# sile/libflate

Hardware: AMD Instinct MI355X
Metric: gzip encode+decode throughput on 256 MiB synthetic text per GPU (uncompressed bytes through the round trip) (higher is better)
Workload: dtype u8; 1 GPU; cfg2: gzip::Encoder (DefaultLz77Encoder, default options, mtime=0) + gzip::Decoder on TEXT(268435456 B) per GPU, write schedule S8K (8192-byte writes); bytes_per_gpu=268435456, schedule=S8K, compressed_bytes=129579521, parallelism=1 rank

## Files before the change

include/lfx.h:

```cpp
#ifndef LFX_H
#define LFX_H
#include <stddef.h>
#include <stdint.h>

#ifdef __cplusplus
extern "C" {
#endif

#define LFX_VERSION 0x000100

enum { LFX_DEFLATE = 0, LFX_ZLIB = 1, LFX_GZIP = 2 };

enum {
    LFX_OK = 0,
    LFX_E_INVALID_DATA = 1,
    LFX_E_UNEXPECTED_EOF = 2,
    LFX_E_IO = 3,
    LFX_E_OOM = 4,
    LFX_E_DEVICE = 5,
    LFX_E_ARG = 6,
    LFX_E_NOSPACE = 7,
    LFX_E_UNSUPPORTED = 8,
    LFX_E_WOULD_BLOCK = 9
};
// ... 104 lines not shown
int lfx_index_read_device(lfx_ctx *c, const lfx_index *idx, const void *d_in, uint64_t in_base, uint64_t n,
                          uint32_t count, const uint64_t *off, const uint64_t *len, void *d_out,
                          const uint64_t *out_off, uint64_t *out_len_r, int32_t *status);
int lfx_index_span(const lfx_index *idx, uint64_t off, uint64_t len, uint64_t *in_lo, uint64_t *in_hi);
int lfx_index_get_info(const lfx_index *idx, lfx_index_info *info);
int lfx_index_get_point(const lfx_index *idx, uint32_t i, lfx_index_point *p);
int lfx_index_export(lfx_ctx *c, const lfx_index *idx, void *buf, uint64_t cap, uint64_t *len);
lfx_index *lfx_index_import(lfx_ctx *c, const void *buf, uint64_t len, int *status);
int lfx_index_check(const void *buf, uint64_t len, lfx_index_info *info);
void lfx_index_free(lfx_index *idx);

typedef struct lfx_shard_info {
    uint64_t total_bits;
    uint64_t n_bytes;
    uint32_t crc32;
    uint32_t adler32;
} lfx_shard_info;
int lfx_encode_shard_prepare(lfx_ctx *c, int format, const lfx_encode_opts *o,
                             const lfx_schedule *s, const void *d_in, uint64_t n, int is_first,
                             int is_last, lfx_shard_info *info);
int lfx_encode_shard_emit(lfx_ctx *c, uint64_t start_bit, uint32_t combined_check,
                          uint64_t total_n, void *d_out, uint64_t cap, uint64_t *out_len);
int lfx_encode_shard_prezero(lfx_ctx *c, void *d_out, uint64_t cap);
int lfx_decode_shard_device(lfx_ctx *c, const void *d_in, uint64_t n, uint64_t start_bit,
                            uint64_t total_bits, int is_last, void *d_out, uint64_t cap,
                            uint64_t *out_len);
typedef struct lfx_blk_tuple {
    uint64_t start_bit, end_bit;
    uint64_t n_out;
    uint64_t data_bit;
    uint32_t n_codes, nlanes;
    uint8_t btype, bfinal, status , _pad;
    uint16_t rank;
    uint16_t _pad2;
    uint32_t slot;
    uint32_t _pad3;
} lfx_blk_tuple;
int lfx_decode_range_scan(lfx_ctx *c, const void *d_part, uint64_t n_part, uint64_t lo_byte, uint64_t hi_byte,
                          uint64_t first_bit, uint64_t final_from_bit, uint32_t rank, lfx_blk_tuple *tuples, uint32_t cap,
                          uint32_t *count);
int lfx_decode_chain(const lfx_blk_tuple *all, uint32_t n_all, uint64_t first_bit, uint32_t *chain, uint32_t cap,
                     uint32_t *n_chain, uint64_t *total_out);
int lfx_decode_range_emit(lfx_ctx *c, const void *d_part, uint64_t n_part, uint64_t lo_byte, const lfx_blk_tuple *all,
                          const uint32_t *chain, uint32_t n_chain, uint32_t rank, void *d_out, uint64_t cap,
                          uint64_t *out_len, uint64_t *out_base, uint32_t *state);
int lfx_decode_range_map(lfx_ctx *c, void *d_map);
int lfx_decode_range_finish(lfx_ctx *c, const void *d_maps, uint32_t rank, uint32_t *crc32, uint32_t *adler32);
int lfx_shard_place_device(lfx_ctx *c, void *d_member, uint64_t cap, const void *d_part, uint64_t part_len,
                           uint64_t start_bit, int is_first);
typedef struct lfx_comm {
    void *user;
    uint32_t rank, world;
    int (*allgather)(void *user, const void *send, void *recv, uint64_t bytes);
    int (*isend)(void *user, const void *d_buf, uint64_t bytes, uint32_t to_rank);
    int (*irecv)(void *user, void *d_buf, uint64_t bytes, uint32_t from_rank);
    int (*wait)(void *user);
    int (*start)(void *user);
} lfx_comm;
int lfx_comm_rccl(void *nccl_comm, void *hip_stream, uint32_t rank, uint32_t world, lfx_comm *out);
void lfx_comm_rccl_free(lfx_comm *cm);

typedef struct lfx_sharded_enc lfx_sharded_enc;
typedef struct lfx_sharded_part {
    uint64_t start_bit;
    uint64_t end_bit;
    uint64_t part_len;
    uint64_t member_len;
    uint64_t total_n;
    uint32_t check;
    uint32_t _pad;
} lfx_sharded_part;
int lfx_sharded_encode_begin(lfx_ctx *c, const lfx_comm *cm, int format, const lfx_encode_opts *o, const lfx_schedule *s,
                             const void *d_in, uint64_t n, void *d_part, uint64_t part_cap, void *d_member ,
                             uint64_t member_cap, void *d_staging , uint64_t staging_cap, lfx_sharded_enc **state,
                             lfx_sharded_part *out);
int lfx_sharded_encode_finish(lfx_ctx *c, const lfx_comm *cm, lfx_sharded_enc *state, uint64_t *member_len );

typedef struct lfx_sharded_slice {
    uint64_t out_len, out_base;
    uint64_t total_out;
    uint32_t crc32, adler32;
} lfx_sharded_slice;
void lfx_sharded_byte_range(uint64_t first_byte, uint64_t member_len, uint32_t rank, uint32_t world, uint64_t *lo_byte,
                            uint64_t *hi_byte, uint64_t *hold_hi);
int lfx_sharded_decode(lfx_ctx *c, const lfx_comm *cm, const void *d_part, uint64_t n_part, uint64_t lo_byte, uint64_t hi_byte,
                       uint64_t first_bit, uint64_t member_len, void *d_out, uint64_t cap, lfx_sharded_slice *out);
int lfx_sharded_layout(const lfx_comm *cm, const lfx_shard_info *mine, uint64_t header_len, int format,
                       uint64_t *start_bits , uint32_t *check, uint64_t *total_n);
int lfx_sharded_gather_tuples(const lfx_comm *cm, const lfx_blk_tuple *mine, uint32_t count, int status, lfx_blk_tuple **all,
                              uint32_t *n_all, uint32_t *failed_rank);
int lfx_sharded_fold(const lfx_comm *cm, int status, uint32_t state, uint64_t len, uint32_t crc32, uint32_t adler32,
                     uint32_t *any_state, uint32_t *crc_all, uint32_t *adler_all, uint64_t *total, uint32_t *failed_rank);
void lfx_sharded_free(void *p);
uint32_t lfx_crc32_combine(uint32_t crc1, uint32_t crc2, uint64_t len2);
uint32_t lfx_adler32_combine(uint32_t ad1, uint32_t ad2, uint64_t len2);
uint64_t lfx_container_header_len(int format, const lfx_encode_opts *o);

typedef int64_t (*lfx_write_cb)(void *user, const uint8_t *p, size_t n);
typedef int (*lfx_flush_cb)(void *user);
typedef int64_t (*lfx_read_cb)(void *user, uint8_t *p, size_t cap);

typedef struct lfx_encoder lfx_encoder;
lfx_encoder *lfx_encoder_new(lfx_ctx *c, int format, const lfx_encode_opts *o, lfx_write_cb w,
                             lfx_flush_cb f, void *user, int *status);
int64_t lfx_encoder_write(lfx_encoder *e, const uint8_t *p, size_t n);
int lfx_encoder_write_codes(lfx_encoder *e, const uint32_t *codes, size_t n_codes, const uint8_t *raw, size_t n_raw,
                            int end_block);
int lfx_encoder_flush(lfx_encoder *e);
int lfx_encoder_finish(lfx_encoder *e);
const char *lfx_encoder_last_error(const lfx_encoder *e);
void lfx_encoder_free(lfx_encoder *e);

typedef struct lfx_decoder lfx_decoder;
#define LFX_DEC_NONBLOCKING 2u
lfx_decoder *lfx_decoder_new(lfx_ctx *c, int format, uint32_t flags, lfx_read_cb r, void *user,
                             int *status);
int64_t lfx_decoder_read(lfx_decoder *d, uint8_t *out, size_t cap);
int lfx_decoder_unread(lfx_decoder *d, const uint8_t **p, size_t *n);
uint64_t lfx_decoder_consumed(const lfx_decoder *d);
uint64_t lfx_decoder_buffered(const lfx_decoder *d);
int lfx_decoder_surplus(lfx_decoder *d, const uint8_t **p, size_t *n);
typedef struct lfx_header {
    int32_t format;
    uint32_t mtime;
    uint8_t xfl, os, is_text, is_verified, has_extra;
    uint8_t _pad[3];
    const uint8_t *extra;
    uint32_t extra_len;
    const char *filename;
    const char *comment;
    uint32_t zlib_window_size;
    uint32_t zlib_level;
} lfx_header;
int lfx_decoder_header(lfx_decoder *d, lfx_header *h);
const char *lfx_decoder_last_error(const lfx_decoder *d);
void lfx_decoder_free(lfx_decoder *d);

typedef void (*lfx_sink_cb)(void *user, const uint32_t *codes, size_t n);
typedef struct lfx_lz77 lfx_lz77;
lfx_lz77 *lfx_lz77_new(lfx_ctx *c, uint32_t window_size, uint32_t max_length, int *status);
int lfx_lz77_encode(lfx_lz77 *z, const uint8_t *buf, size_t len, lfx_sink_cb sink, void *user);
int lfx_lz77_flush(lfx_lz77 *z, lfx_sink_cb sink, void *user);
uint32_t lfx_lz77_window_size(const lfx_lz77 *z);
int lfx_lz77_compression_level(const lfx_lz77 *z);
void lfx_lz77_free(lfx_lz77 *z);

typedef struct lfx_timing {
    float total_ms;
    float phase_ms[16];
    char phase_name[16][24];
    int n_phases;
} lfx_timing;
uint64_t lfx_ctx_match_fallbacks(const lfx_ctx *c);
int lfx_ctx_last_timing(lfx_ctx *c, lfx_timing *t);
void lfx_ctx_enable_timing(lfx_ctx *c, int on);
uint32_t lfx_version(void);

#ifdef __cplusplus
}
#endif
#endif
```

libflate_amd/_ffi.py:

```python
import ctypes as C
import os

_HERE = os.path.dirname(os.path.abspath(__file__))
SO_PATH = os.environ.get("LFX_SO") or os.path.join(_HERE, "liblfx.so")

DEFLATE, ZLIB, GZIP = 0, 1, 2
OK, E_INVALID_DATA, E_UNEXPECTED_EOF, E_IO, E_OOM, E_DEVICE, E_ARG, E_NOSPACE, E_UNSUPPORTED, E_WOULD_BLOCK = range(10)
LZ77_DEFAULT, LZ77_NOCOMPRESSION = 0, 1
FLUSH_NONE, FLUSH_SYNC = 0, 2
SCHED_SINGLE, SCHED_FIXED, SCHED_LIST = 0, 1, 2
SCHED_FLUSH = (1 << 64) - 1
DEC_MULTI = 1
DEC_NONBLOCKING = 2
MEMBERS_BGZF = 1
BGZF_MEMBER_SIZE = 65280

EXPORTS = [
    "lfx_encode_opts_default", "lfx_ctx_new", "lfx_ctx_free", "lfx_ctx_last_error", "lfx_ctx_set_stream",
    "lfx_device_count", "lfx_encode_bound", "lfx_encode_device", "lfx_encode_batch_device", "lfx_encode_host", "lfx_decode_device",
    "lfx_decode_host", "lfx_decode_batch_device", "lfx_encode_shard_prepare", "lfx_encode_shard_emit", "lfx_encode_shard_prezero", "lfx_decode_shard_device", "lfx_shard_place_device", "lfx_decode_range_scan", "lfx_decode_chain", "lfx_decode_range_emit", "lfx_decode_range_map", "lfx_decode_range_finish",
    "lfx_crc32_combine", "lfx_adler32_combine", "lfx_container_header_len", "lfx_encoder_new",
    "lfx_encoder_write", "lfx_encoder_write_codes", "lfx_encoder_flush", "lfx_encoder_finish", "lfx_encoder_last_error",
    "lfx_encoder_free", "lfx_decoder_new", "lfx_decoder_read", "lfx_decoder_unread",
    "lfx_decoder_consumed", "lfx_decoder_buffered", "lfx_decoder_surplus", "lfx_decoder_header", "lfx_decoder_last_error", "lfx_decoder_free", "lfx_lz77_new",
    "lfx_lz77_encode", "lfx_lz77_flush", "lfx_lz77_window_size", "lfx_lz77_compression_level",
    "lfx_lz77_free", "lfx_ctx_last_timing", "lfx_ctx_enable_timing", "lfx_version",
    "lfx_comm_rccl", "lfx_comm_rccl_free", "lfx_sharded_encode_begin", "lfx_sharded_encode_finish", "lfx_sharded_byte_range",
    "lfx_sharded_decode", "lfx_sharded_layout", "lfx_sharded_gather_tuples", "lfx_sharded_fold", "lfx_sharded_free",
    "lfx_host_alloc", "lfx_host_free", "lfx_ctx_match_fallbacks", "lfx_decode_members_device", "lfx_decode_members_host",
    "lfx_decode_index_device", "lfx_index_read_device", "lfx_index_span", "lfx_index_get_info", "lfx_index_get_point",
    "lfx_index_export", "lfx_index_import", "lfx_index_check", "lfx_index_free", "lfx_encode_index_device",
    "lfx_encode_members_bound", "lfx_encode_members_device", "lfx_encode_members_host", "lfx_members_gzi",
]


class EncodeOpts(C.Structure):
    _fields_ = [
        ("block_size", C.c_uint64), ("dynamic_huffman", C.c_int32), ("no_compression", C.c_int32),
        ("lz77_kind", C.c_int32), ("window_size", C.c_uint32), ("max_length", C.c_uint32),
        ("zlib_flush_mode", C.c_int32), ("mtime", C.c_uint32), ("os", C.c_uint8), ("is_text", C.c_uint8),
        ("hcrc", C.c_uint8), ("lz77_level", C.c_uint8), ("extra", C.c_char_p), ("extra_len", C.c_uint32),
        ("filename", C.c_char_p), ("comment", C.c_char_p),
    ]


class Schedule(C.Structure):
    _fields_ = [("kind", C.c_int32), ("fixed_write", C.c_uint64), ("writes", C.POINTER(C.c_uint64)),
                ("n_writes", C.c_size_t)]


class BlkTuple(C.Structure):
    _fields_ = [("start_bit", C.c_uint64), ("end_bit", C.c_uint64), ("n_out", C.c_uint64), ("data_bit", C.c_uint64),
                ("n_codes", C.c_uint32), ("nlanes", C.c_uint32), ("btype", C.c_uint8), ("bfinal", C.c_uint8),
                ("status", C.c_uint8), ("_pad", C.c_uint8), ("rank", C.c_uint16), ("_pad2", C.c_uint16),
                ("slot", C.c_uint32), ("_pad3", C.c_uint32)]


class Member(C.Structure):
    _fields_ = [("in_off", C.c_uint64), ("in_len", C.c_uint64), ("out_off", C.c_uint64), ("out_len", C.c_uint64)]


class IndexPoint(C.Structure):
    _fields_ = [("in_bit", C.c_uint64), ("hdr_bit", C.c_uint64), ("out_off", C.c_uint64), ("member", C.c_uint32),
                ("win_len", C.c_uint32), ("in_crc", C.c_uint32), ("btype", C.c_uint8), ("_pad", C.c_uint8 * 3)]


class IndexInfo(C.Structure):
    _fields_ = [("in_len", C.c_uint64), ("out_len", C.c_uint64), ("spacing", C.c_uint64), ("max_gap", C.c_uint64),
                ("export_bytes", C.c_uint64), ("format", C.c_uint32), ("flags", C.c_uint32), ("n_points", C.c_uint32),
                ("n_members", C.c_uint32)]


class ShardInfo(C.Structure):
    _fields_ = [("total_bits", C.c_uint64), ("n_bytes", C.c_uint64), ("crc32", C.c_uint32),
                ("adler32", C.c_uint32)]


COMM_ALLGATHER = C.CFUNCTYPE(C.c_int, C.c_void_p, C.c_void_p, C.c_void_p, C.c_uint64)
COMM_P2P = C.CFUNCTYPE(C.c_int, C.c_void_p, C.c_void_p, C.c_uint64, C.c_uint32)
COMM_WAIT = C.CFUNCTYPE(C.c_int, C.c_void_p)


class Comm(C.Structure):
    _fields_ = [("user", C.c_void_p), ("rank", C.c_uint32), ("world", C.c_uint32), ("allgather", COMM_ALLGATHER),
                ("isend", COMM_P2P), ("irecv", COMM_P2P), ("wait", COMM_WAIT), ("start", COMM_WAIT)]


class ShardedPart(C.Structure):
    _fields_ = [("start_bit", C.c_uint64), ("end_bit", C.c_uint64), ("part_len", C.c_uint64), ("member_len", C.c_uint64), ("total_n", C.c_uint64),
                ("check", C.c_uint32), ("_pad", C.c_uint32)]


class ShardedSlice(C.Structure):
    _fields_ = [("out_len", C.c_uint64), ("out_base", C.c_uint64), ("total_out", C.c_uint64), ("crc32", C.c_uint32),
                ("adler32", C.c_uint32)]


class Header(C.Structure):
    _fields_ = [("format", C.c_int32), ("mtime", C.c_uint32), ("xfl", C.c_uint8), ("os", C.c_uint8),
                ("is_text", C.c_uint8), ("is_verified", C.c_uint8), ("has_extra", C.c_uint8), ("_pad", C.c_uint8 * 3),
                ("extra", C.POINTER(C.c_uint8)), ("extra_len", C.c_uint32), ("filename", C.c_char_p),
                ("comment", C.c_char_p), ("zlib_window_size", C.c_uint32), ("zlib_level", C.c_uint32)]


class Timing(C.Structure):
    _fields_ = [("total_ms", C.c_float), ("phase_ms", C.c_float * 16), ("phase_name", (C.c_char * 24) * 16),
                ("n_phases", C.c_int)]


WRITE_CB = C.CFUNCTYPE(C.c_int64, C.c_void_p, C.POINTER(C.c_uint8), C.c_size_t)
FLUSH_CB = C.CFUNCTYPE(C.c_int, C.c_void_p)
READ_CB = C.CFUNCTYPE(C.c_int64, C.c_void_p, C.POINTER(C.c_uint8), C.c_size_t)
SINK_CB = C.CFUNCTYPE(None, C.c_void_p, C.POINTER(C.c_uint32), C.c_size_t)


class LfxError(Exception):
    def __init__(self, status, message=""):
        super().__init__("lfx status %d: %s" % (status, message))
        self.status = status
        self.message = message


class DeviceError(LfxError):
    pass


_lib = None


def lib():
    global _lib
    if _lib is not None:
        return _lib
    if not os.path.exists(SO_PATH):
        raise ImportError(
            "libflate_amd: native library %s is missing — run `python -c 'import __graft_entry__ as g; "
            "g.build()'` (hipcc, gfx950). There is no CPU fallback." % SO_PATH)
    try:
        import torch
    except ImportError:
        pass
    L = C.CDLL(SO_PATH)
    u64, u32, vp, i32 = C.c_uint64, C.c_uint32, C.c_void_p, C.c_int
    L.lfx_encode_opts_default.argtypes = [C.POINTER(EncodeOpts)]
    L.lfx_ctx_new.restype = vp
    L.lfx_ctx_new.argtypes = [i32, C.POINTER(i32)]
    L.lfx_ctx_free.argtypes = [vp]
    L.lfx_ctx_last_error.restype = C.c_char_p
    L.lfx_ctx_last_error.argtypes = [vp]
    L.lfx_ctx_set_stream.argtypes = [vp, vp]
    L.lfx_encode_bound.restype = u64
    L.lfx_encode_bound.argtypes = [u64, C.POINTER(EncodeOpts), C.POINTER(Schedule)]
    L.lfx_encode_device.argtypes = [vp, i32, C.POINTER(EncodeOpts), C.POINTER(Schedule), vp, u64, vp, u64,
                                    C.POINTER(u64)]
    L.lfx_encode_host.argtypes = [vp, i32, C.POINTER(EncodeOpts), C.POINTER(Schedule), vp, u64, vp,
                                  u64, C.POINTER(u64)]
    L.lfx_host_alloc.restype = vp
    L.lfx_host_alloc.argtypes = [C.c_size_t]
    L.lfx_host_free.argtypes = [vp]
    L.lfx_ctx_match_fallbacks.restype = u64
    L.lfx_ctx_match_fallbacks.argtypes = [vp]
    L.lfx_decode_device.argtypes = [vp, i32, u32, vp, u64, vp, u64, C.POINTER(u64), C.POINTER(u64)]
    L.lfx_decode_host.argtypes = [vp, i32, u32, vp, u64, vp, u64, C.POINTER(u64), C.POINTER(u64)]
    L.lfx_decode_batch_device.argtypes = [vp, i32, u32, vp, vp, vp, vp, vp, vp, vp, vp]
    L.lfx_decode_members_device.argtypes = [vp, vp, u64, vp, u64, C.POINTER(u64), C.POINTER(u64), C.POINTER(Member), u32,
                                            C.POINTER(u32)]
    L.lfx_decode_members_host.argtypes = [vp, vp, u64, vp, u64, C.POINTER(u64), C.POINTER(u64), C.POINTER(Member), u32,
                                          C.POINTER(u32)]
    L.lfx_encode_members_bound.restype = u64
    L.lfx_encode_members_bound.argtypes = [u64, u64, u32, C.POINTER(EncodeOpts), C.POINTER(Schedule)]
    for f in (L.lfx_encode_members_device, L.lfx_encode_members_host):
        f.argtypes = [vp, C.POINTER(EncodeOpts), C.POINTER(Schedule), u64, u32, vp, u64, vp, u64, C.POINTER(u64),
                      C.POINTER(Member), u32, C.POINTER(u32)]
    L.lfx_members_gzi.argtypes = [C.POINTER(Member), u32, vp, u64, C.POINTER(u64)]
    L.lfx_decode_index_device.argtypes = [vp, i32, u32, vp, u64, vp, u64, C.POINTER(u64), C.POINTER(u64), u64, C.POINTER(vp)]
    L.lfx_encode_index_device.argtypes = [vp, i32, C.POINTER(EncodeOpts), C.POINTER(Schedule), vp, u64, vp, u64, C.POINTER(u64), u64,
                                          C.POINTER(vp)]
    L.lfx_index_read_device.argtypes = [vp, vp, vp, u64, u64, u32, vp, vp, vp, vp, vp, vp]
    L.lfx_index_span.argtypes = [vp, u64, u64, C.POINTER(u64), C.POINTER(u64)]
    L.lfx_index_get_info.argtypes = [vp, C.POINTER(IndexInfo)]
    L.lfx_index_get_point.argtypes = [vp, u32, C.POINTER(IndexPoint)]
    L.lfx_index_export.argtypes = [vp, vp, vp, u64, C.POINTER(u64)]
    L.lfx_index_import.argtypes = [vp, vp, u64, C.POINTER(i32)]
    L.lfx_index_import.restype = vp
    L.lfx_index_check.argtypes = [vp, u64, C.POINTER(IndexInfo)]
    L.lfx_index_free.argtypes = [vp]
    L.lfx_index_free.restype = None
    L.lfx_encode_batch_device.argtypes = [vp, i32, C.POINTER(EncodeOpts), C.POINTER(Schedule), u32, vp, vp, vp, vp, vp, vp, vp, vp]
    L.lfx_encode_shard_prepare.argtypes = [vp, i32, C.POINTER(EncodeOpts), C.POINTER(Schedule), vp, u64, i32,
                                           i32, C.POINTER(ShardInfo)]
    L.lfx_encode_shard_emit.argtypes = [vp, u64, u32, u64, vp, u64, C.POINTER(u64)]
    L.lfx_encode_shard_prezero.argtypes = [vp, vp, u64]
    L.lfx_decode_shard_device.argtypes = [vp, vp, u64, u64, u64, i32, vp, u64, C.POINTER(u64)]
    L.lfx_shard_place_device.argtypes = [vp, vp, u64, vp, u64, u64, i32]
    L.lfx_decode_range_scan.argtypes = [vp, vp, u64, u64, u64, u64, u64, u32, C.POINTER(BlkTuple), u32, C.POINTER(u32)]
    L.lfx_decode_chain.argtypes = [C.POINTER(BlkTuple), u32, u64, C.POINTER(u32), u32, C.POINTER(u32), C.POINTER(u64)]
    L.lfx_decode_range_emit.argtypes = [vp, vp, u64, u64, C.POINTER(BlkTuple), C.POINTER(u32), u32, u32, vp, u64,
                                        C.POINTER(u64), C.POINTER(u64), C.POINTER(u32)]
    L.lfx_decode_range_map.argtypes = [vp, vp]
    L.lfx_decode_range_finish.argtypes = [vp, vp, u32, C.POINTER(u32), C.POINTER(u32)]
    L.lfx_crc32_combine.restype = u32
    L.lfx_crc32_combine.argtypes = [u32, u32, u64]
    L.lfx_adler32_combine.restype = u32
    L.lfx_adler32_combine.argtypes = [u32, u32, u64]
    L.lfx_container_header_len.restype = u64
    L.lfx_container_header_len.argtypes = [i32, C.POINTER(EncodeOpts)]
    L.lfx_encoder_new.restype = vp
    L.lfx_encoder_new.argtypes = [vp, i32, C.POINTER(EncodeOpts), WRITE_CB, FLUSH_CB, vp, C.POINTER(i32)]
    L.lfx_encoder_write.restype = C.c_int64
    L.lfx_encoder_write.argtypes = [vp, C.c_char_p, C.c_size_t]
    L.lfx_encoder_write_codes.argtypes = [vp, C.POINTER(u32), C.c_size_t, C.c_char_p, C.c_size_t, i32]
    L.lfx_encoder_flush.argtypes = [vp]
    L.lfx_encoder_finish.argtypes = [vp]
    L.lfx_encoder_last_error.restype = C.c_char_p
    L.lfx_encoder_last_error.argtypes = [vp]
    L.lfx_encoder_free.argtypes = [vp]
    L.lfx_decoder_new.restype = vp
    L.lfx_decoder_new.argtypes = [vp, i32, u32, READ_CB, vp, C.POINTER(i32)]
    L.lfx_decoder_read.restype = C.c_int64
    L.lfx_decoder_read.argtypes = [vp, vp, C.c_size_t]
    L.lfx_decoder_unread.argtypes = [vp, C.POINTER(C.POINTER(C.c_uint8)), C.POINTER(C.c_size_t)]
    L.lfx_decoder_consumed.restype = u64
    L.lfx_decoder_consumed.argtypes = [vp]
    L.lfx_decoder_buffered.restype = u64
    L.lfx_decoder_buffered.argtypes = [vp]
    L.lfx_decoder_surplus.argtypes = [vp, C.POINTER(C.POINTER(C.c_uint8)), C.POINTER(C.c_size_t)]
    L.lfx_decoder_header.argtypes = [vp, C.POINTER(Header)]
    L.lfx_decoder_last_error.restype = C.c_char_p
    L.lfx_decoder_last_error.argtypes = [vp]
    L.lfx_decoder_free.argtypes = [vp]
    L.lfx_lz77_new.restype = vp
    L.lfx_lz77_new.argtypes = [vp, u32, u32, C.POINTER(i32)]
    L.lfx_lz77_encode.argtypes = [vp, C.c_char_p, C.c_size_t, SINK_CB, vp]
    L.lfx_lz77_flush.argtypes = [vp, SINK_CB, vp]
    L.lfx_lz77_window_size.restype = u32
    L.lfx_lz77_window_size.argtypes = [vp]
    L.lfx_lz77_compression_level.argtypes = [vp]
    L.lfx_lz77_free.argtypes = [vp]
    L.lfx_ctx_last_timing.argtypes = [vp, C.POINTER(Timing)]
    L.lfx_ctx_enable_timing.argtypes = [vp, i32]
    L.lfx_version.restype = u32
    L.lfx_comm_rccl.argtypes = [vp, vp, u32, u32, C.POINTER(Comm)]
    L.lfx_comm_rccl_free.argtypes = [C.POINTER(Comm)]
    L.lfx_comm_rccl_free.restype = None
    L.lfx_sharded_encode_begin.argtypes = [vp, C.POINTER(Comm), i32, C.POINTER(EncodeOpts), C.POINTER(Schedule), vp, u64, vp, u64,
                                           vp, u64, vp, u64, C.POINTER(vp), C.POINTER(ShardedPart)]
    L.lfx_sharded_encode_finish.argtypes = [vp, C.POINTER(Comm), vp, C.POINTER(u64)]
    L.lfx_sharded_byte_range.argtypes = [u64, u64, u32, u32, C.POINTER(u64), C.POINTER(u64), C.POINTER(u64)]
    L.lfx_sharded_byte_range.restype = None
    L.lfx_sharded_decode.argtypes = [vp, C.POINTER(Comm), vp, u64, u64, u64, u64, u64, vp, u64, C.POINTER(ShardedSlice)]
    L.lfx_sharded_layout.argtypes = [C.POINTER(Comm), C.POINTER(ShardInfo), u64, i32, C.POINTER(u64), C.POINTER(u32), C.POINTER(u64)]
    L.lfx_sharded_gather_tuples.argtypes = [C.POINTER(Comm), C.POINTER(BlkTuple), u32, i32, C.POINTER(C.POINTER(BlkTuple)),
                                            C.POINTER(u32), C.POINTER(u32)]
    L.lfx_sharded_fold.argtypes = [C.POINTER(Comm), i32, u32, u64, u32, u32, C.POINTER(u32), C.POINTER(u32), C.POINTER(u32),
                                   C.POINTER(u64), C.POINTER(u32)]
    L.lfx_sharded_free.argtypes = [vp]
    L.lfx_sharded_free.restype = None
    L.lfx_debug_huff_block.argtypes = [vp, u32, vp, vp, vp, C.POINTER(u32), C.POINTER(u64)]
    L.lfx_debug_plan.argtypes = [i32, C.POINTER(EncodeOpts), C.POINTER(Schedule), u64, vp, C.c_size_t,
                                 C.POINTER(C.c_size_t), vp, C.c_size_t, C.POINTER(C.c_size_t)]
    L.lfx_debug_plan_incremental.argtypes = [i32, C.POINTER(EncodeOpts), C.POINTER(Schedule), u64, u32, vp, C.c_size_t,
                                             C.POINTER(C.c_size_t), vp, C.c_size_t, C.POINTER(C.c_size_t)]
    L.lfx_debug_symbols.argtypes = [u32, u32, vp]
    _lib = L
    return L


def make_opts(**kw):
    o = EncodeOpts()
    lib().lfx_encode_opts_default(C.byref(o))
    keep = []
    for k, v in kw.items():
        if k == "extra":
            v = bytes(v)
            keep.append(v)
            o.extra, o.extra_len = v, len(v)
        elif k in ("filename", "comment"):
            v = bytes(v)
            keep.append(v)
            setattr(o, k, v)
        else:
            setattr(o, k, v)
    o._keep = keep
    return o


def members_to_gzi(members):
    members = list(members)
    table = (Member * max(len(members), 1))()
    for i, m in enumerate(members):
        table[i].in_off, table[i].in_len, table[i].out_off, table[i].out_len = m
    need = C.c_uint64(0)
    lib().lfx_members_gzi(table, len(members), None, 0, C.byref(need))
    buf = C.create_string_buffer(need.value)
    rc = lib().lfx_members_gzi(table, len(members), buf, need.value, C.byref(need))
    if rc:
        raise LfxError(rc, "lfx_members_gzi")
    return buf.raw[:need.value]


def make_schedule(write_size=0, writes=None):
    s = Schedule()
    if writes is not None:
        arr = (C.c_uint64 * len(writes))(*[SCHED_FLUSH if w is None else int(w) for w in writes])
        s.kind, s.writes, s.n_writes = SCHED_LIST, arr, len(writes)
        s._keep = arr
    elif write_size:
        s.kind, s.fixed_write = SCHED_FIXED, write_size
    else:
        s.kind = SCHED_SINGLE
    return s
```

libflate_amd/context.py:

```python
import ctypes as C

from . import _ffi


class Context:
    def __init__(self, device=0):
        st = C.c_int(0)
        self._h = _ffi.lib().lfx_ctx_new(device, C.byref(st))
        if not self._h:
            raise _ffi.DeviceError(st.value, "no usable MI355X device %d (there is no CPU fallback)" % device)
        self.device = device
        self._users = 0
        self._closing = False

    def _retain(self):
        self._users += 1

    def _release(self):
        self._users -= 1
        if self._users <= 0 and self._closing:
            self._free_now()

    def _free_now(self):
        if self._h:
            _ffi.lib().lfx_ctx_free(self._h)
            self._h = None

    def close(self):
        self._closing = True
        if self._users <= 0:
            self._free_now()

    def __del__(self):
        try:
            self.close()
        except Exception:
            pass

    @property
    def handle(self):
        return self._h

    def last_error(self):
        return (_ffi.lib().lfx_ctx_last_error(self._h) or b"").decode("utf-8", "replace")

    def set_stream(self, hip_stream_ptr):
        _ffi.lib().lfx_ctx_set_stream(self._h, hip_stream_ptr)

    def enable_timing(self, on=True):
        _ffi.lib().lfx_ctx_enable_timing(self._h, int(on) if on is not True and on is not False and 2 <= int(on) <= 6 else (1 if on else 0))

    def last_timing(self):
        t = _ffi.Timing()
        if _ffi.lib().lfx_ctx_last_timing(self._h, C.byref(t)) != 0:
            return None
        return {"total_ms": t.total_ms,
                "phases": [(bytes(t.phase_name[i]).split(b"\0")[0].decode(), t.phase_ms[i])
                           for i in range(t.n_phases)]}

    def match_fallbacks(self):
        return int(_ffi.lib().lfx_ctx_match_fallbacks(self._h))

    def encode_host_ptr(self, fmt, in_ptr, n, out_ptr, cap, opts=None, schedule=None):
        out_len = C.c_uint64(0)
        rc = _ffi.lib().lfx_encode_host(self._h, fmt, C.byref(opts) if opts is not None else None,
                                        C.byref(schedule) if schedule is not None else None, in_ptr, n, out_ptr, cap, C.byref(out_len))
        if rc:
            raise (_ffi.DeviceError if rc == _ffi.E_DEVICE else _ffi.LfxError)(rc, self.last_error())
        return out_len.value

    def decode_host_ptr(self, fmt, in_ptr, n, out_ptr, cap, flags=0):
        out_len, consumed = C.c_uint64(0), C.c_uint64(0)
        rc = _ffi.lib().lfx_decode_host(self._h, fmt, flags, in_ptr, n, out_ptr, cap, C.byref(out_len), C.byref(consumed))
        if rc in (_ffi.E_DEVICE, _ffi.E_OOM, _ffi.E_ARG):
            raise (_ffi.DeviceError if rc == _ffi.E_DEVICE else _ffi.LfxError)(rc, self.last_error())
        return rc, out_len.value, consumed.value, self.last_error() if rc else ""

    def encode_device(self, fmt, d_in, n, d_out, cap, opts=None, schedule=None):
        out_len = C.c_uint64(0)
        rc = _ffi.lib().lfx_encode_device(self._h, fmt, C.byref(opts) if opts is not None else None,
                                          C.byref(schedule) if schedule is not None else None,
                                          d_in, n, d_out, cap, C.byref(out_len))
        if rc:
            raise (_ffi.DeviceError if rc == _ffi.E_DEVICE else _ffi.LfxError)(rc, self.last_error())
        return out_len.value

    def encode_index_device(self, fmt, d_in, n, d_out, cap, opts=None, schedule=None, spacing=1 << 20):
        out_len, h = C.c_uint64(0), C.c_void_p(None)
        rc = _ffi.lib().lfx_encode_index_device(self._h, fmt, C.byref(opts) if opts is not None else None,
                                                C.byref(schedule) if schedule is not None else None,
                                                d_in, n, d_out, cap, C.byref(out_len), spacing, C.byref(h))
        if rc:
            raise (_ffi.DeviceError if rc == _ffi.E_DEVICE else _ffi.LfxError)(rc, self.last_error())
        return out_len.value, h.value

    def decode_device(self, fmt, d_in, n, d_out, cap, flags=0):
        out_len, consumed = C.c_uint64(0), C.c_uint64(0)
        rc = _ffi.lib().lfx_decode_device(self._h, fmt, flags, d_in, n, d_out, cap, C.byref(out_len),
                                          C.byref(consumed))
        if rc in (_ffi.E_DEVICE, _ffi.E_OOM, _ffi.E_ARG):
            raise (_ffi.DeviceError if rc == _ffi.E_DEVICE else _ffi.LfxError)(rc, self.last_error())
        return rc, out_len.value, consumed.value, self.last_error() if rc else ""

    def decode_members_device(self, d_in, n, d_out, cap, max_members=None):
        return self._members(_ffi.lib().lfx_decode_members_device, d_in, n, d_out, cap, max_members)

    def decode_index_device(self, fmt, d_in, n, d_out, cap, spacing=1 << 20, flags=0):
        out_len, consumed, h = C.c_uint64(0), C.c_uint64(0), C.c_void_p(None)
        rc = _ffi.lib().lfx_decode_index_device(self._h, fmt, flags, d_in, n, d_out, cap, C.byref(out_len), C.byref(consumed),
                                                spacing, C.byref(h))
        if rc in (_ffi.E_DEVICE, _ffi.E_OOM, _ffi.E_ARG):
            raise (_ffi.DeviceError if rc == _ffi.E_DEVICE else _ffi.LfxError)(rc, self.last_error())
        return rc, out_len.value, consumed.value, h.value, self.last_error() if rc else ""

    def index_read_device(self, index_handle, d_in, in_base, n, offs, lens, d_out, out_offs):
        k = len(offs)
        a = lambda v: (C.c_uint64 * max(k, 1))(*v)
        o, ln, oo = a(offs), a(lens), a(out_offs)
        out_len, st = (C.c_uint64 * max(k, 1))(), (C.c_int32 * max(k, 1))()
        rc = _ffi.lib().lfx_index_read_device(self._h, index_handle, d_in, in_base, n, k, o, ln, d_out, oo, out_len, st)
        if rc in (_ffi.E_DEVICE, _ffi.E_OOM) or (rc == _ffi.E_ARG and not any(st[i] == _ffi.E_ARG for i in range(k))):
            raise (_ffi.DeviceError if rc == _ffi.E_DEVICE else _ffi.LfxError)(rc, self.last_error())
        return rc, list(out_len[:k]), list(st[:k]), self.last_error() if rc else ""

    def _members(self, fn, src, n, dst, cap, max_members):
        if max_members is None:
            max_members = n // 20 + 1
        table = (_ffi.Member * max(int(max_members), 1))()
        out_len, consumed, count = C.c_uint64(0), C.c_uint64(0), C.c_uint32(0)
        rc = fn(self._h, src, n, dst, cap, C.byref(out_len), C.byref(consumed), table, int(max_members), C.byref(count))
        if rc in (_ffi.E_DEVICE, _ffi.E_OOM, _ffi.E_ARG):
            raise (_ffi.DeviceError if rc == _ffi.E_DEVICE else _ffi.LfxError)(rc, self.last_error())
        members = [(m.in_off, m.in_len, m.out_off, m.out_len) for m in table[:min(count.value, int(max_members))]]
        return rc, out_len.value, consumed.value, members, self.last_error() if rc else ""

    def decode_members_host(self, data, cap=None, max_members=None):
        data = bytes(data)
        grow = cap is None
        cap = cap if cap is not None else max(1 << 16, len(data) * 16)
        while True:
            out = C.create_string_buffer(cap)
            rc, ol, used, members, msg = self._members(_ffi.lib().lfx_decode_members_host, data, len(data), out, cap, max_members)
            if grow and rc == _ffi.E_NOSPACE and cap < len(data) * 1040 + (1 << 20):
                cap *= 8
                continue
            return rc, out.raw[:ol], used, members, msg

    def _encode_members(self, fn, src, n, dst, cap, member_size, flags, opts, schedule, max_members):
        count = 0 if (flags & _ffi.MEMBERS_BGZF and n == 0) else max(1, -(-n // member_size)) if member_size else 0
        if max_members is None:
            max_members = count
        table = (_ffi.Member * max(int(max_members), 1))()
        out_len, got = C.c_uint64(0), C.c_uint32(0)
        rc = fn(self._h, C.byref(opts) if opts is not None else None, C.byref(schedule) if schedule is not None else None,
                member_size, flags, src, n, dst, cap, C.byref(out_len), table, int(max_members), C.byref(got))
        if rc in (_ffi.E_DEVICE, _ffi.E_OOM, _ffi.E_ARG, _ffi.E_UNSUPPORTED):
            raise (_ffi.DeviceError if rc == _ffi.E_DEVICE else _ffi.LfxError)(rc, self.last_error())
        members = [(m.in_off, m.in_len, m.out_off, m.out_len) for m in table[:min(got.value, int(max_members))]]
        return rc, out_len.value, got.value, members, self.last_error() if rc else ""

    def encode_members_device(self, d_in, n, d_out, cap, member_size=1 << 20, flags=0, opts=None, schedule=None, max_members=None):
        return self._encode_members(_ffi.lib().lfx_encode_members_device, d_in, n, d_out, cap, member_size, flags, opts, schedule,
                                    max_members)

    def encode_members_host(self, data, member_size=1 << 20, flags=0, opts=None, schedule=None, cap=None, max_members=None):
        data = bytes(data)
        if cap is None:
            cap = _ffi.lib().lfx_encode_members_bound(len(data), member_size, flags, C.byref(opts) if opts is not None else None,
                                                      C.byref(schedule) if schedule is not None else None)
        out = C.create_string_buffer(max(cap, 1))
        rc, ol, count, members, msg = self._encode_members(_ffi.lib().lfx_encode_members_host, data, len(data), out, cap, member_size,
                                                           flags, opts, schedule, max_members)
        return rc, out.raw[:ol], count, members, msg

    def encode_host(self, fmt, data, opts=None, schedule=None):
        data = bytes(data)
        bound = _ffi.lib().lfx_encode_bound(len(data), C.byref(opts) if opts is not None else None,
                                            C.byref(schedule) if schedule is not None else None)
        if bound == 0:
            raise _ffi.LfxError(_ffi.E_ARG, "option outside the reference's domain")
        out = C.create_string_buffer(bound)
        out_len = C.c_uint64(0)
        rc = _ffi.lib().lfx_encode_host(self._h, fmt, C.byref(opts) if opts is not None else None,
                                        C.byref(schedule) if schedule is not None else None,
                                        data, len(data), out, bound, C.byref(out_len))
        if rc:
            raise (_ffi.DeviceError if rc == _ffi.E_DEVICE else _ffi.LfxError)(rc, self.last_error())
        return out.raw[:out_len.value]

    def decode_host(self, fmt, data, cap=None, flags=0):
        data = bytes(data)
        cap = cap if cap is not None else max(1 << 16, len(data) * 16)
        while True:
            out = C.create_string_buffer(cap)
            out_len, consumed = C.c_uint64(0), C.c_uint64(0)
            rc = _ffi.lib().lfx_decode_host(self._h, fmt, flags, data, len(data), out, cap,
                                            C.byref(out_len), C.byref(consumed))
            if rc in (_ffi.E_DEVICE, _ffi.E_OOM, _ffi.E_ARG):
                raise (_ffi.DeviceError if rc == _ffi.E_DEVICE else _ffi.LfxError)(rc, self.last_error())
            if rc == _ffi.E_NOSPACE and cap < len(data) * 1040 + (1 << 20):
                cap *= 8
                continue
            return rc, out.raw[:out_len.value], consumed.value, self.last_error() if rc else ""


_default = {}


def default_context(device=0):
    if device not in _default:
        _default[device] = Context(device)
    return _default[device]
```

libflate_amd/csrc/lfx_api.cpp:

```cpp
#include "../../include/lfx.h"
#include "../../include/lfx_testhooks.h"

#include <hip/hip_runtime.h>

#include <algorithm>
#include <cstddef>
#include <cstdio>
#include <cstdlib>
#include <cstring>
#include <mutex>
#include <string>
#include <vector>

#include "lfx_ctx.h"
#include "lfx_device.h"
#include "lfx_huff.h"
#include "lfx_index.h"
#include "lfx_plan.h"
#include "lfx_abi_guard.h"

using namespace lfx;

static uint32_t host_crc32(const uint8_t *p, size_t n) {
    static uint32_t tab[256];
// ... 58 lines not shown
    return d;
}
static int check_opts(const lfx_encode_opts &o) {
    if (o.block_size == 0) return LFX_E_ARG;
    if (o.max_length < 3) return LFX_E_ARG;
    return LFX_OK;
}
static PlanOpts plan_opts(int format, const lfx_encode_opts &o) {
    PlanOpts p;
    p.block_size = o.block_size;
    p.dynamic_huffman = o.dynamic_huffman != 0;
    p.no_compression = o.no_compression != 0;
    p.lz77_kind = o.lz77_kind;
    p.window_size = o.window_size;
    p.max_length = o.max_length;
    p.zlib_sync = format == LFX_ZLIB && o.zlib_flush_mode == LFX_FLUSH_SYNC;
    return p;
}

static void gzip_header(const lfx_encode_opts &o, bool with_hcrc, std::vector<uint8_t> &b) {
    uint8_t flg = (uint8_t)((o.is_text ? 1 : 0) | (with_hcrc ? 2 : 0) | (o.extra ? 4 : 0) |
                            (o.filename ? 8 : 0) | (o.comment ? 16 : 0));
    const uint8_t xfl = o.lz77_level == 1 + LFX_LEVEL_FAST ? 4 : o.lz77_level == 1 + LFX_LEVEL_BEST ? 2 : 0;
    const uint8_t h[10] = {31, 139, 8, flg, (uint8_t)o.mtime, (uint8_t)(o.mtime >> 8),
                           (uint8_t)(o.mtime >> 16), (uint8_t)(o.mtime >> 24), xfl, o.os};
    b.insert(b.end(), h, h + 10);
    if (o.extra) {
        b.push_back((uint8_t)o.extra_len);
        b.push_back((uint8_t)(o.extra_len >> 8));
        b.insert(b.end(), o.extra, o.extra + o.extra_len);
    }
    if (o.filename) b.insert(b.end(), o.filename, o.filename + strlen(o.filename) + 1);
    if (o.comment) b.insert(b.end(), o.comment, o.comment + strlen(o.comment) + 1);
    if (with_hcrc) {
        std::vector<uint8_t> t;
        gzip_header(o, false, t);
        uint32_t c = host_crc32(t.data(), t.size());
        b.push_back((uint8_t)c);
        b.push_back((uint8_t)(c >> 8));
    }
}
static int container_header(int format, const lfx_encode_opts &o, std::vector<uint8_t> &b) {
    if (format == LFX_GZIP) {
        if (o.extra && o.extra_len > 0xFFFF) return LFX_E_INVALID_DATA;
        gzip_header(o, o.hcrc != 0, b);
    } else if (format == LFX_ZLIB) {
        uint32_t ws = o.window_size;
        uint8_t cinfo = ws > 16384 ? 7 : ws > 8192 ? 6 : ws > 4096 ? 5 : ws > 2048 ? 4 : ws > 1024 ? 3
                        : ws > 512 ? 2 : ws > 256 ? 1 : 0;
        uint8_t level = (o.no_compression || o.lz77_kind == LFX_LZ77_NOCOMPRESSION) ? 0 : 2;
        if (o.lz77_level && !o.no_compression) level = (uint8_t)((o.lz77_level - 1) & 3);
        uint8_t cmf = (uint8_t)((cinfo << 4) | 8), flg = (uint8_t)(level << 6);
        uint32_t check = ((uint32_t)cmf << 8) + flg;
        if (check % 31 != 0) flg = (uint8_t)(flg + (31 - check % 31));
        b.push_back(cmf);
        b.push_back(flg);
    } else if (format != LFX_DEFLATE) {
        return LFX_E_ARG;
    }
    return LFX_OK;
}
extern "C" uint64_t lfx_container_header_len(int format, const lfx_encode_opts *o) {
    std::vector<uint8_t> b;
    lfx_encode_opts d = norm_opts(o);
    container_header(format, d, b);
    return b.size();
}

static void apply_schedule(Planner &pl, const lfx_schedule *s, uint64_t n) {
    if (!s || s->kind == LFX_SCHED_SINGLE) {
        pl.write(n);
    } else if (s->kind == LFX_SCHED_FIXED) {
        uint64_t w = s->fixed_write ? s->fixed_write : n;
        if (w) {
            pl.write_repeat(w, n / w);
            if (n % w) pl.write(n % w);
        }
    } else {
        uint64_t used = 0;
        for (size_t i = 0; i < s->n_writes; i++) {
            if (s->writes[i] == LFX_SCHED_FLUSH) { pl.flush(); continue; }
            uint64_t w = std::min(s->writes[i], n - used);
            pl.write(w);
            used += w;
        }
        if (used < n) pl.write(n - used);
    }
}

extern "C" uint64_t lfx_encode_bound(uint64_t n, const lfx_encode_opts *o, const lfx_schedule *s) {
    lfx_encode_opts d = norm_opts(o);
    if (check_opts(d)) return 0;
    Planner pl(plan_opts(LFX_ZLIB, d));
    apply_schedule(pl, s, n);
    Plan &p = pl.finish();
    uint64_t hdr = 64 + (d.extra ? d.extra_len + 2 : 0) + (d.filename ? strlen(d.filename) + 1 : 0) +
                   (d.comment ? strlen(d.comment) + 1 : 0);
    return n + n / 4 + 1024 * (uint64_t)p.blocks.size() + hdr + 64;
}

namespace lfx {

#define HIP_TRY(expr)                                                                 \
    do {                                                                              \
        hipError_t e_ = (expr);                                                       \
        if (e_ != hipSuccess) {                                                       \
            c->set_error(std::string(#expr) + ": " + hipGetErrorString(e_));          \
            return LFX_E_DEVICE;                                                      \
        }                                                                             \
    } while (0)

int DevBuf::reserve(size_t bytes) {
    if (bytes <= cap) return 0;
    if (p) (void)hipFree(p);
    p = nullptr;
    cap = 0;
    gen++;
    size_t want = bytes + bytes / 8 + 4096;
    if (hipMalloc(&p, want) != hipSuccess) {
        if (hipMalloc(&p, bytes) != hipSuccess) { p = nullptr; return LFX_E_OOM; }
        want = bytes;
    }
    cap = want;
    return 0;
}
void DevBuf::release() {
    if (p) (void)hipFree(p);
    p = nullptr;
    cap = 0;
}

void Diag::read() {
    auto on = [](const char *k) { return getenv(k) != nullptr; };
    debug = on("LFX_DEBUG");
    match_v1 = on("LFX_MATCH_V1");
    match_v5 = on("LFX_MATCH_V5");
    if (const char *mp = getenv("LFX_MATCH_PARTS")) match_parts = atoi(mp);
    if (const char *rc7 = getenv("LFX_R7_CAP")) r7_cap = atoi(rc7);
    no_serial = on("LFX_NO_SERIAL");
    batch_serial = on("LFX_BATCH_SERIAL");
    no_markers = on("LFX_NO_MARKERS");
    no_pieces = on("LFX_NO_PIECES");
    no_final_cand = on("LFX_NO_FINAL_CAND");
    window_chain = on("LFX_WINDOW_CHAIN");
    if (const char *fs = getenv("LFX_FREE_SHIFT")) free_shift = atoi(fs);
    if (const char *pm = getenv("LFX_POCR_MAX")) pocr_max = atoi(pm);
    if (const char *eb = getenv("LFX_ENC_BATCH_MB")) enc_batch_mb = atoi(eb);
    two_pass = on("LFX_TWO_PASS");
    hist_separate = on("LFX_HIST_SEPARATE");
    find2_exp = getenv("LFX_FIND2_EXP") ? atoi(getenv("LFX_FIND2_EXP")) : 0;
    no_pin_slots = on("LFX_NO_PIN_SLOTS");
    no_small_scan = on("LFX_NO_SMALL_SCAN");
    store_tight = on("LFX_STORE_TIGHT");
}

void Ctx::phase(const char *name) {
    if (!timing_on) return;
    if (timing_on >= 2 && timing_on <= 5) {
        static const char *const pair[4][2] = {{"lz77_resolve", "lz77_walk"}, {"find2", "blk_scan"}, {"upload", "lz77_cand"}, {"blk_emit", "lz77_copy"}};
        const char *const *pr = pair[timing_on - 2];
        if (strcmp(name, pr[0]) != 0 && strcmp(name, pr[1]) != 0) return;
    }
    if (n_ev >= 17) return;
    if (!ev[n_ev]) (void)hipEventCreate(&ev[n_ev]);
    (void)hipEventRecord(ev[n_ev], stream);
    snprintf(ev_name[n_ev], sizeof ev_name[n_ev], "%s", name);
    n_ev++;
}

}

extern "C" int lfx_device_count(void) {
    int n = 0;
    if (hipGetDeviceCount(&n) != hipSuccess) return 0;
    return n;
}

extern "C" lfx_ctx *lfx_ctx_new(int device, int *status) try {
    int st = LFX_OK;
    int n = 0;
    if (hipGetDeviceCount(&n) != hipSuccess || n <= 0 || device < 0 || device >= n) {
        if (status) *status = LFX_E_DEVICE;
        return nullptr;
    }
    Ctx *c = new Ctx();
    c->device = device;
    if (hipSetDevice(device) != hipSuccess || hipStreamCreate(&c->own_stream) != hipSuccess) {
        delete c;
        if (status) *status = LFX_E_DEVICE;
        return nullptr;
    }
    c->stream = c->own_stream;
    c->diag.read();
    (void)hipDeviceGetAttribute(&c->n_cu, hipDeviceAttributeMultiprocessorCount, device);
    if (hipStreamCreateWithFlags(&c->side_stream, hipStreamNonBlocking) != hipSuccess ||
        hipEventCreateWithFlags(&c->ev_fork, hipEventDisableTiming) != hipSuccess ||
        hipEventCreateWithFlags(&c->ev_join, hipEventDisableTiming) != hipSuccess ||
        hipEventCreateWithFlags(&c->ev_zero, hipEventDisableTiming) != hipSuccess ||
        hipEventCreateWithFlags(&c->ev_res, hipEventDisableTiming) != hipSuccess ||
        hipEventCreateWithFlags(&c->ev_part[0], hipEventDisableTiming) != hipSuccess ||
        hipEventCreateWithFlags(&c->ev_part[1], hipEventDisableTiming) != hipSuccess ||
        hipEventCreateWithFlags(&c->ev_part[2], hipEventDisableTiming) != hipSuccess ||
        hipEventCreateWithFlags(&c->ev_part[3], hipEventDisableTiming) != hipSuccess) {
        (void)hipStreamDestroy(c->own_stream);
        delete c;
        if (status) *status = LFX_E_DEVICE;
        return nullptr;
    }
    if (hipHostMalloc((void **)&c->h_res, 4096 + Ctx::PIN_ARENA, hipHostMallocDefault) != hipSuccess) {
        (void)hipStreamDestroy(c->own_stream);
        delete c;
        if (status) *status = LFX_E_OOM;
        return nullptr;
    }
    if (status) *status = st;
    return reinterpret_cast<lfx_ctx *>(c);
} LFX_ABI_CATCH_NEW
extern "C" void lfx_ctx_free(lfx_ctx *cc) {
    if (!cc) return;
    Ctx *c = reinterpret_cast<Ctx *>(cc);
    (void)hipSetDevice(c->device);
    (void)hipStreamSynchronize(c->stream);
    for (DevBuf *b : c->all_bufs()) b->release();
    for (DevBuf &b : c->dev_pool) b.release();
    c->dev_pool.clear();
    c->pin_pool.clear();
    for (auto &e : c->ev) if (e) (void)hipEventDestroy(e);
    if (c->h_res) (void)hipHostFree(c->h_res);
    c->hostio.release();
    if (c->ev_fork) (void)hipEventDestroy(c->ev_fork);
    if (c->ev_join) (void)hipEventDestroy(c->ev_join);
    if (c->ev_zero) (void)hipEventDestroy(c->ev_zero);
    if (c->ev_res) (void)hipEventDestroy(c->ev_res);
    for (hipEvent_t e : c->ev_part) if (e) (void)hipEventDestroy(e);
    if (c->side_stream) (void)hipStreamDestroy(c->side_stream);
    if (c->own_stream) (void)hipStreamDestroy(c->own_stream);
    delete c;
}
extern "C" const char *lfx_ctx_last_error(const lfx_ctx *cc) {
    return cc ? reinterpret_cast<const Ctx *>(cc)->err.c_str() : "no context";
}
extern "C" void lfx_ctx_set_stream(lfx_ctx *cc, void *s) {
    Ctx *c = reinterpret_cast<Ctx *>(cc);
    c->stream = s ? (hipStream_t)s : c->own_stream;
}
extern "C" uint64_t lfx_ctx_match_fallbacks(const lfx_ctx *cc) {
    return cc ? reinterpret_cast<const Ctx *>(cc)->match_fallbacks : 0;
}
extern "C" void lfx_ctx_enable_timing(lfx_ctx *cc, int on) { reinterpret_cast<Ctx *>(cc)->timing_on = on >= 2 && on <= 6 ? on : on != 0; }
extern "C" int lfx_ctx_last_timing(lfx_ctx *cc, lfx_timing *t) try {
    Ctx *c = reinterpret_cast<Ctx *>(cc);
    std::lock_guard<std::recursive_mutex> lock(c->mu);
    memset(t, 0, sizeof *t);
    if (c->n_ev < 2) return LFX_E_ARG;
    (void)hipEventSynchronize(c->ev[c->n_ev - 1]);
    (void)hipEventElapsedTime(&t->total_ms, c->ev[0], c->ev[c->n_ev - 1]);
    t->n_phases = c->n_ev - 1;
    for (int i = 0; i + 1 < c->n_ev && i < 16; i++) {
        (void)hipEventElapsedTime(&t->phase_ms[i], c->ev[i], c->ev[i + 1]);
        snprintf(t->phase_name[i], sizeof t->phase_name[i], "%s", c->ev_name[i + 1]);
    }
    return LFX_OK;
} LFX_ABI_CATCH

namespace lfx {

int encode_prepare(Ctx *c, const Plan &plan, const PlanOpts &po, const uint8_t *d_in, uint64_t n,
                   int ck_mode, const HostCodes *hc) {
    const bool want_checksum = ck_mode != 0;
    (void)hipSetDevice(c->device);
    hipStream_t st = c->stream;
    c->n_ev = 0;
    c->phase("start");
    for (const ChunkDesc &ch : plan.chunks)
        if (ch.len >= (1ull << 32) - 4) {
            c->set_error("an LZ77 chunk of 4 GiB or more is outside the reference's domain (u32 positions, default.rs:78)");
            return LFX_E_ARG;
        }
    const uint32_t nchunks = (uint32_t)plan.chunks.size(), nblocks = (uint32_t)plan.blocks.size();
    const bool match_v1 = c->force_match_v1 || c->diag.match_v1;
    if (c->force_match_v1 && !hc) c->match_fallbacks++;
    std::vector<SegDesc> segs;
    if (!hc) {
        uint64_t seg_len = SEG_POSITIONS;
        for (;;) {
            uint64_t cnt = 0;
            for (const ChunkDesc &ch : plan.chunks)
                if (!(ch.flags & CH_LITERALS) && ch.len > 3) cnt += div_up(ch.len - 3, seg_len);
            if (cnt >= 512 || seg_len <= 32768) break;
            seg_len /= 2;
        }
        for (uint32_t ci = 0; ci < nchunks; ci++) {
            const ChunkDesc &ch = plan.chunks[ci];
            if (ch.flags & CH_LITERALS) continue;
            for (uint64_t s = 0; s + 3 < ch.len; s += seg_len)
                segs.push_back(SegDesc{ci, (uint32_t)s, (uint32_t)std::min<uint64_t>(seg_len, ch.len - s), 0});
        }
    }
    uint64_t lnk_units = 0;
    for (SegDesc &sg : segs) {
        if (lnk_units > 0xFFFFFFFFull) { c->set_error("input too large for the link scratch"); return LFX_E_ARG; }
        sg.lnk_base = (uint32_t)lnk_units;
        lnk_units += div_up((uint64_t)sg.len + std::min<uint64_t>(sg.start, MAX_WINDOW) + 4, 64);
        lnk_units = (lnk_units + 1) & ~1ull;
    }
    std::vector<ParseWg> pwgs;
    for (uint32_t ci = 0; ci < nchunks && !hc; ci++) {
        const ChunkDesc &ch = plan.chunks[ci];
        if (ch.flags & CH_LITERALS) continue;
        for (uint32_t s = 0; s < ch.n_seg; s += PARSE_WG_SEGS) pwgs.push_back(ParseWg{ci, s});
    }
    if (pwgs.size() > 8) {
        const size_t nl = pwgs.size(), per = (nl + 7) / 8;
        std::vector<ParseWg> phys(per * 8);
        for (size_t i = 0; i < phys.size(); i++) {
            const size_t l = (i % 8) * per + i / 8;
            phys[i] = (i / 8 < per && l < nl && l / per == i % 8) ? pwgs[l] : ParseWg{0xFFFFFFFFu, 0u};
        }
        pwgs.swap(phys);
    }
    c->cur_nchunks = nchunks;
    c->cur_nblocks = nblocks;
    c->cur_ntiles = plan.n_tiles;
    c->cur_n = n;
    c->cur_in = d_in;
    int rc;
    if ((rc = c->d_chunks.reserve(sizeof(ChunkDesc) * std::max<size_t>(nchunks, 1)))) return rc;
    if ((rc = c->d_blocks.reserve(sizeof(BlockDesc) * std::max<size_t>(nblocks, 1)))) return rc;
    if ((rc = c->d_segs.reserve(sizeof(SegDesc) * std::max<size_t>(segs.size(), 1)))) return rc;
    if ((rc = c->d_pwgs.reserve(sizeof(ParseWg) * std::max<size_t>(pwgs.size(), 1)))) return rc;
    if (!hc && (rc = c->d_cd.reserve(2 * n + 64))) return rc;
    if (!hc && !match_v1 && (rc = c->d_glnk.reserve(264 * std::max<uint64_t>(lnk_units, 1)))) return rc;
    if (!hc && !match_v1 && (rc = c->d_ucount.reserve(4 * std::max<size_t>(segs.size(), 1)))) return rc;
    if (!hc && match_v1 && (rc = c->d_md.reserve(4 * std::max<uint64_t>(n, 1)))) return rc;
    if ((rc = c->d_codes.reserve(4 * std::max<uint64_t>(plan.n_codes_cap, 1)))) return rc;
    if ((rc = c->d_ncodes.reserve(4 * std::max<size_t>(nchunks, 1)))) return rc;
    if ((rc = c->d_vis.reserve(8 * std::max<uint64_t>(plan.n_vis, 1)))) return rc;
    if ((rc = c->d_segtmp.reserve(24ull * std::max<uint32_t>(plan.n_segs, 1)))) return rc;
    if (!hc && (rc = c->d_stage.reserve(4ull * (n + 64)))) return rc;
    if ((rc = c->d_chunkmap.reserve(4ull * (plan.n_tiles + plan.n_segs + 2)))) return rc;
    if ((rc = c->d_hist.reserve(4ull * 320 * std::max<size_t>(nblocks, 1)))) return rc;
    if ((rc = c->d_bc.reserve(sizeof(BlockCodes) * std::max<size_t>(nblocks, 1)))) return rc;
    if ((rc = c->d_block_start.reserve(8 * std::max<size_t>(nblocks, 1)))) return rc;
    if ((rc = c->d_tile_bits.reserve(4 * std::max<uint64_t>(plan.n_tiles, 1)))) return rc;
    if ((rc = c->d_tile_start.reserve(8 * std::max<uint64_t>(plan.n_tiles, 1)))) return rc;
    const uint64_t nspans = ck_nspans(n);
    if ((rc = c->d_ck.reserve(12 * nspans))) return rc;
    if ((rc = c->d_res.reserve(256))) return rc;
    if ((rc = c->d_small.reserve(70000))) return rc;

    auto upload = [&](int slot, DevBuf &b, const void *src, size_t bytes) -> hipError_t {
        std::vector<uint8_t> &sh = c->up_shadow[slot];
        const uint64_t tag = (uint64_t)(uintptr_t)b.p ^ ((uint64_t)b.gen << 48) ^ (1ull << 63);
        if (c->up_dev[slot] == tag && sh.size() == bytes && (bytes == 0 || memcmp(sh.data(), src, bytes) == 0)) return hipSuccess;
        sh.assign((const uint8_t *)src, (const uint8_t *)src + bytes);
        c->up_dev[slot] = tag;
        return bytes ? hipMemcpyAsync(b.p, sh.data(), bytes, hipMemcpyHostToDevice, st) : hipSuccess;
    };
    HIP_TRY(upload(0, c->d_chunks, plan.chunks.data(), sizeof(ChunkDesc) * nchunks));
    HIP_TRY(upload(1, c->d_blocks, plan.blocks.data(), sizeof(BlockDesc) * nblocks));
    HIP_TRY(upload(2, c->d_segs, segs.data(), sizeof(SegDesc) * segs.size()));
    HIP_TRY(upload(3, c->d_pwgs, pwgs.data(), sizeof(ParseWg) * pwgs.size()));
    const bool ucount_here = !hc && !match_v1 && !c->diag.match_v5;
    const ZeroSpan z_hist{(uint32_t *)c->d_hist.p, (uint32_t)(320 * std::max<size_t>(nblocks, 1))}, z_res{(uint32_t *)c->d_res.p, 64u},
        z_ucount{ucount_here ? (uint32_t *)c->d_ucount.p : nullptr, ucount_here ? (uint32_t)std::max<size_t>(segs.size(), 1) : 0u};
    c->phase("upload");
    uint32_t *tile_map = (uint32_t *)c->d_chunkmap.p, *seg_map = tile_map + plan.n_tiles;
    c->cur_tile_map = tile_map;
    if (int e_ = launch_chunk_maps(st, (const ChunkDesc *)c->d_chunks.p, nchunks, plan.n_tiles, plan.n_segs, tile_map, seg_map, z_hist,
                                   z_res, z_ucount)) {
        c->set_error(hipGetErrorString((hipError_t)e_));
        return LFX_E_DEVICE;
    }

#define LAUNCH_TRY(call)                                                              \
    do {                                                                              \
        int e_ = (call);                                                              \
        if (e_) {                                                                     \
            c->set_error(std::string(#call) + ": " + hipGetErrorString((hipError_t)e_)); \
            return LFX_E_DEVICE;                                                      \
        }                                                                             \
    } while (0)

    uint64_t *mdbg = nullptr;
    if (c->diag.debug) mdbg = (uint64_t *)((uint8_t *)c->d_small.p + 32768);
    bool fused_hist = false;
    bool forked = false;
    uint32_t emit_per = 0, emit_parts = 0;
    if (hc) {
        if (hc->n_codes) HIP_TRY(hipMemcpyAsync(c->d_codes.p, hc->codes, 4ull * hc->n_codes, hipMemcpyHostToDevice, st));
        if (nchunks) HIP_TRY(hipMemcpyAsync(c->d_ncodes.p, hc->chunk_codes, 4ull * nchunks, hipMemcpyHostToDevice, st));
        c->phase("codes_upload");
    } else {
    uint32_t *d_match_flags = (uint32_t *)((uint8_t *)c->d_res.p + offsetof(EncodeResult, match_flags));
    uint16_t *d_cd = (uint16_t *)c->d_cd.p;
    if (match_v1) {
        LAUNCH_TRY(launch_match(st, d_in, n, (const ChunkDesc *)c->d_chunks.p, (const SegDesc *)c->d_segs.p,
                                (uint32_t)segs.size(), po.window_size, po.max_length, (uint32_t *)c->d_md.p, mdbg));
        LAUNCH_TRY(launch_md_to_cd(st, (const uint32_t *)c->d_md.p, n, d_cd));
    } else {
        if (!c->diag.match_v5) {
            const uint32_t ns = (uint32_t)segs.size();
            const uint32_t ncu = (uint32_t)std::max(c->n_cu, 1);
            const uint32_t want_parts = (uint32_t)std::max(c->diag.match_parts, 1);
            const uint32_t parts = ns >= 2 * ncu ? std::min<uint32_t>(std::min<uint32_t>(4, want_parts), ns / ncu) : 1;
            const SegDesc *dsegs = (const SegDesc *)c->d_segs.p;
            uint32_t *d_glnk = (uint32_t *)c->d_glnk.p;
            uint64_t *d_umask = (uint64_t *)((uint8_t *)c->d_glnk.p + 256 * std::max<uint64_t>(lnk_units, 1));
            uint32_t *d_ucount = (uint32_t *)c->d_ucount.p;
            for (uint32_t k = 0; k < parts; k++) {
                const uint32_t s0 = (uint32_t)((uint64_t)ns * k / parts), s1 = (uint32_t)((uint64_t)ns * (k + 1) / parts);
                LAUNCH_TRY(launch_match7(st, d_in, n, (const ChunkDesc *)c->d_chunks.p, dsegs + s0, s1 - s0, po.window_size, d_cd,
                                         d_glnk, d_umask, d_match_flags, k == 0 ? mdbg : nullptr));
                if (parts == 1 && c->timing_fine()) c->phase("lz77_cand");
                hipStream_t rs = parts > 1 ? c->side_stream : st;
                if (parts > 1) {
                    HIP_TRY(hipEventRecord(c->ev_part[k], st));
                    HIP_TRY(hipStreamWaitEvent(rs, c->ev_part[k], 0));
                }
                LAUNCH_TRY(launch_resolve7(rs, (const ChunkDesc *)c->d_chunks.p, dsegs + s0, s1 - s0, po.window_size, d_cd,
                                           d_glnk, d_umask, (uint32_t *)c->d_stage.p, d_ucount + s0, (uint32_t)std::max(c->diag.r7_cap, 0)));
            }
            if (parts > 1) {
                HIP_TRY(hipEventRecord(c->ev_res, c->side_stream));
                HIP_TRY(hipStreamWaitEvent(st, c->ev_res, 0));
            }
        }
        else
            LAUNCH_TRY(launch_match5(st, d_in, n, (const ChunkDesc *)c->d_chunks.p, (const SegDesc *)c->d_segs.p,
                                     (uint32_t)segs.size(), po.window_size, d_cd, (uint16_t *)c->d_glnk.p, d_match_flags, mdbg));
    }
    if (mdbg) {
        uint64_t hv[256];
        (void)hipMemcpy(hv, mdbg, sizeof hv, hipMemcpyDeviceToHost);
        const bool v5 = !match_v1 && c->diag.match_v5, v7 = !match_v1 && !c->diag.match_v5;
        if (v7) {
            for (int w = 0; w < 16; w++)
                fprintf(stderr, "[lfx] match7 wave%d: work=%llu barrier-wait=%llu tiles=%llu\n", w, (unsigned long long)hv[w * 8],
                        (unsigned long long)hv[w * 8 + 1], (unsigned long long)hv[w * 8 + 5]);
        } else {
            for (int w = 0; w < 16; w++)
                fprintf(stderr, "[lfx] match%s wave%d: %s=%llu %s=%llu wait=%llu tiles=%llu\n", match_v1 ? "1" : "5", w,
                        match_v1 ? "load" : "phaseA", (unsigned long long)hv[w * 8], match_v1 ? "work" : "phaseB",
                        (unsigned long long)hv[w * 8 + 1], (unsigned long long)hv[w * 8 + 2], (unsigned long long)hv[w * 8 + 5]);
        }
        if (v5) {
            uint64_t handed = 0;
            for (int w = 1; w < 16; w++) handed += hv[128 + w * 8 + 5];
            fprintf(stderr, "[lfx] match5 workgroup 0: %llu walks handed over to wave 0 of %llu positions; wave 0 waited %llu cycles for their loads\n",
                    (unsigned long long)handed, (unsigned long long)hv[5] * 960ull, (unsigned long long)hv[6]);
            for (int w = 1; w < 16; w++)
                fprintf(stderr, "[lfx] match5 wave%d loop trips: sum=%u max=%u tiles>4=%u tiles>8=%u\n", w, (unsigned)hv[w * 8 + 3],
                        (unsigned)(hv[w * 8 + 3] >> 32), (unsigned)hv[w * 8 + 4], (unsigned)(hv[w * 8 + 4] >> 32));
        }
    }
    c->phase(c->timing_fine() ? "lz77_resolve" : "lz77_match");
    if (c->diag.debug && getenv("LFX_DUMP_SEG")) {
        const uint32_t sg = (uint32_t)atoi(getenv("LFX_DUMP_SEG"));
        for (int stage_no = 1; stage_no <= 3 && sg < plan.n_segs; stage_no++) {
            LAUNCH_TRY(launch_parse(st, d_in, n, (const ChunkDesc *)c->d_chunks.p, nchunks, plan.n_segs, (const ParseWg *)c->d_pwgs.p,
                                    (uint32_t)pwgs.size(), d_cd, po.max_length, (uint64_t *)c->d_vis.p, (uint32_t *)c->d_segtmp.p,
                                    (uint32_t *)c->d_codes.p, (uint32_t *)c->d_ncodes.p, (uint32_t *)c->d_stage.p, seg_map, stage_no % 3));
            (void)hipStreamSynchronize(st);
            uint64_t v[4];
            uint32_t t[6];
            uint16_t cdv[64];
            (void)hipMemcpy(v, (uint64_t *)c->d_vis.p + (uint64_t)sg * 64, sizeof v, hipMemcpyDeviceToHost);
            for (int q = 0; q < 6; q++) (void)hipMemcpy(&t[q], (uint32_t *)c->d_segtmp.p + (size_t)q * plan.n_segs + sg, 4, hipMemcpyDeviceToHost);
            (void)hipMemcpy(cdv, d_cd + (uint64_t)sg * PARSE_SEG, sizeof cdv, hipMemcpyDeviceToHost);
            fprintf(stderr, "[lfx] seg %u stage %d: vis %016llx %016llx %016llx %016llx exit=%u count=%u off=%u exit2=%u mpos=%u kspec=%u\n", sg,
                    stage_no, (unsigned long long)v[0], (unsigned long long)v[1], (unsigned long long)v[2], (unsigned long long)v[3], t[0],
                    t[1], t[2], t[3], t[4], t[5]);
            if (stage_no == 1) { fprintf(stderr, "[lfx]  cd:"); for (int q = 0; q < 64; q++) fprintf(stderr, " %u", cdv[q]); fprintf(stderr, "\n"); }
        }
    }
    {
        const uint32_t target = PARSE_EMIT_WG_PER_CU * (uint32_t)std::max(c->n_cu, 1);
        uint32_t per = (uint32_t)div_up(std::max<uint32_t>(plan.n_segs, 1), target);
        per = (per + PARSE_EMIT_WAVES - 1) / PARSE_EMIT_WAVES * PARSE_EMIT_WAVES;
        uint32_t max_segs = 0;
        uint64_t useful = 0;
        for (uint32_t ci = 0; ci < nchunks; ci++) {
            max_segs = std::max(max_segs, plan.chunks[ci].n_seg);
            useful += div_up(plan.chunks[ci].n_seg, per);
        }
        const uint64_t parts = div_up(max_segs, per);
        fused_hist = !c->diag.hist_separate && parts <= 65535 && (uint64_t)nchunks * parts <= 4 * useful + 4096;
        emit_per = per;
        emit_parts = (uint32_t)parts;
    }
    for (int part = c->timing_fine() ? 1 : 0; part <= (c->timing_fine() ? 2 : 0); part++) {
        LAUNCH_TRY(launch_parse(st, d_in, n, (const ChunkDesc *)c->d_chunks.p, nchunks, plan.n_segs, (const ParseWg *)c->d_pwgs.p,
                                (uint32_t)pwgs.size(), d_cd, po.max_length, (uint64_t *)c->d_vis.p, (uint32_t *)c->d_segtmp.p,
                                (uint32_t *)c->d_codes.p, (uint32_t *)c->d_ncodes.p, (uint32_t *)c->d_stage.p, seg_map, part == 1 ? 1 : 0,
                                mdbg ? mdbg + 256 : nullptr, fused_hist ? (uint32_t *)c->d_hist.p : nullptr, emit_per, emit_parts,
                                want_checksum ? c->ev_fork : nullptr, d_match_flags, part == 2 ? 1 : 0));
        if (part == 1) c->phase("lz77_walk");
    }
    if (want_checksum) {
        uint32_t *ck = (uint32_t *)c->d_ck.p;
        HIP_TRY(hipStreamWaitEvent(c->side_stream, c->ev_fork, 0));
        LAUNCH_TRY(launch_checksum_part(c->side_stream, d_in, n, ck, ck + nspans, ck + 2 * nspans, (EncodeResult *)c->d_res.p, ck_mode, 0, 2));
        forked = true;
    }
    if (mdbg) {
        uint64_t hv[32];
        (void)hipMemcpy(hv, mdbg + 256, sizeof hv, hipMemcpyDeviceToHost);
        for (int w = 0; w < 4; w++)
            fprintf(stderr, "[lfx] walk wave%d: fill=%llu spec=%llu resolve+chain=%llu emit=%llu cycles\n", w, (unsigned long long)hv[w * 8],
                    (unsigned long long)hv[w * 8 + 1], (unsigned long long)hv[w * 8 + 2], (unsigned long long)hv[w * 8 + 3]);
    }
    c->phase(c->timing_fine() ? "lz77_chain" : "lz77_parse");
    }
    if (want_checksum) {
        uint32_t *ck = (uint32_t *)c->d_ck.p;
        HIP_TRY(hipEventRecord(c->ev_fork, st));
        HIP_TRY(hipStreamWaitEvent(c->side_stream, c->ev_fork, 0));
        if (forked) LAUNCH_TRY(launch_checksum_part(c->side_stream, d_in, n, ck, ck + nspans, ck + 2 * nspans, (EncodeResult *)c->d_res.p, ck_mode, 1, 2));
        else LAUNCH_TRY(launch_checksum(c->side_stream, d_in, n, ck, ck + nspans, ck + 2 * nspans, (EncodeResult *)c->d_res.p, ck_mode));
        HIP_TRY(hipEventRecord(c->ev_join, c->side_stream));
    }
    uint32_t split = nchunks && nchunks < 1024 ? std::min<uint32_t>(1024, 2048 / nchunks + 1) : 1;
    if (!fused_hist)
        LAUNCH_TRY(launch_histogram(st, (const ChunkDesc *)c->d_chunks.p, nchunks, split, (const uint32_t *)c->d_codes.p,
                                    (const uint32_t *)c->d_ncodes.p, (uint32_t *)c->d_hist.p));
    c->phase("histogram");
    LAUNCH_TRY(launch_huffman(st, (const BlockDesc *)c->d_blocks.p, nblocks, (const uint32_t *)c->d_hist.p,
                              (BlockCodes *)c->d_bc.p, mdbg ? mdbg + 512 : nullptr));
    c->phase("huffman");
    if (mdbg) {
        uint64_t hv[24];
        (void)hipMemcpy(hv, mdbg + 512, sizeof hv, hipMemcpyDeviceToHost);
        static const char *nm[10] = {"lit: rank sort", "lit: depth", "lit: package-merge", "lit: widths", "lit: codes", "dist tree", "run lengths",
                                     "code-length tree", "header bits", "body size"};
        fprintf(stderr, "[lfx] huffman block 0 (cycles):");
        for (int k = 0; k < 10; k++) fprintf(stderr, " %s=%llu", nm[k], (unsigned long long)(hv[k + 1] - hv[k]));
        fprintf(stderr, "\n");
    }
    if (want_checksum) {
        HIP_TRY(hipStreamWaitEvent(st, c->ev_join, 0));
        c->phase("checksum");
    }
    return LFX_OK;
}

int encode_emit(Ctx *c, int format, bool with_trailer, uint32_t trailer_check, bool use_device_check, uint64_t total_n,
                const uint8_t *prefix, uint32_t prefix_len, uint64_t start_bit, uint8_t *d_out, uint64_t cap,
                EncodeResult *host_res, EncodeResult *async_slot = nullptr);
int encode_emit(Ctx *c, int format, bool with_trailer, uint32_t trailer_check, bool use_device_check,
                uint64_t total_n, const uint8_t *prefix, uint32_t prefix_len, uint64_t start_bit,
                uint8_t *d_out, uint64_t cap, EncodeResult *host_res, EncodeResult *async_slot) {
    (void)hipSetDevice(c->device);
    hipStream_t st = c->stream;
    if (((uintptr_t)d_out & 3) != 0) { c->set_error("output buffer must be 4-byte aligned"); return LFX_E_ARG; }
    const uint64_t trailer = with_trailer ? (format == LFX_GZIP ? 8 : format == LFX_ZLIB ? 4 : 0) : 0;
    if (cap < prefix_len + trailer + 8) { c->set_error("output capacity too small"); return LFX_E_NOSPACE; }
    const uint64_t cap_words = cap / 4;
    const uint64_t cap_bits = (cap_words * 4 - trailer) * 8;
    if (c->prezero_ptr == d_out && c->prezero_bytes == cap_words * 4) {
        HIP_TRY(hipStreamWaitEvent(st, c->ev_zero, 0));
    } else {
        HIP_TRY(hipMemsetAsync(d_out, 0, cap_words * 4, st));
    }
    c->prezero_ptr = nullptr;
    c->phase("memset_out");
    EncodeResult *dres = (EncodeResult *)c->d_res.p;
    LAUNCH_TRY(launch_offsets(st, (const BlockDesc *)c->d_blocks.p, c->cur_nblocks, (const BlockCodes *)c->d_bc.p,
                              start_bit, cap_bits, (uint64_t *)c->d_block_start.p, dres));
    LAUNCH_TRY(launch_pack(st, c->cur_in, c->cur_n, (const ChunkDesc *)c->d_chunks.p, c->cur_nchunks,
                           (const BlockDesc *)c->d_blocks.p, c->cur_nblocks, c->cur_ntiles,
                           (const uint32_t *)c->d_codes.p, (const uint32_t *)c->d_ncodes.p,
                           (const BlockCodes *)c->d_bc.p, (const uint64_t *)c->d_block_start.p,
                           (uint32_t *)c->d_tile_bits.p, (uint64_t *)c->d_tile_start.p, dres, 0,
                           (uint32_t *)d_out, c->cur_tile_map));
    c->phase("pack");
    if (prefix_len) {
        int rcp = c->d_hdr.reserve(prefix_len);
        if (rcp) return rcp;
        HIP_TRY(hipMemcpyAsync(c->d_hdr.p, prefix, prefix_len, hipMemcpyHostToDevice, st));
        LAUNCH_TRY(launch_put_bytes(st, (const uint8_t *)c->d_hdr.p, prefix_len, 0, (uint32_t *)d_out));
    }
    if (!use_device_check) {
        HIP_TRY(hipMemcpyAsync((uint8_t *)dres + offsetof(EncodeResult, crc32), &trailer_check, 4, hipMemcpyHostToDevice, st));
        HIP_TRY(hipMemcpyAsync((uint8_t *)dres + offsetof(EncodeResult, adler32), &trailer_check, 4, hipMemcpyHostToDevice, st));
    }
    LAUNCH_TRY(launch_trailer(st, with_trailer ? format : LFX_DEFLATE, (uint32_t)total_n, 0, dres, (uint32_t *)d_out));
    HIP_TRY(hipMemcpyAsync(async_slot ? (void *)async_slot : c->h_res, dres, sizeof(EncodeResult), hipMemcpyDeviceToHost, st));
    c->phase("frame");
    if (async_slot) return LFX_OK;
    HIP_TRY(hipStreamSynchronize(st));
    *host_res = *(EncodeResult *)c->h_res;
    if (host_res->status != 0) { c->set_error("output capacity too small"); return LFX_E_NOSPACE; }
    return LFX_OK;
}

}

static bool match_violation(Ctx *c, const EncodeResult &res) {
    if (!(res.match_flags & 1) || c->force_match_v1) return false;
    c->force_match_v1 = true;
    return true;
}

extern "C" int lfx_encode_device(lfx_ctx *cc, int format, const lfx_encode_opts *o, const lfx_schedule *s,
                                 const void *d_in, uint64_t n, void *d_out, uint64_t cap, uint64_t *out_len) try {
    if (!cc) return LFX_E_DEVICE;
    Ctx *c = reinterpret_cast<Ctx *>(cc);
    std::lock_guard<std::recursive_mutex> lock(c->mu);
    lfx_encode_opts d = norm_opts(o);
    int rc = check_opts(d);
    if (rc) { c->set_error("option outside the reference's domain"); return rc; }
    std::vector<uint8_t> hdr;
    if ((rc = container_header(format, d, hdr))) { c->set_error("bad container options"); return rc; }
    PlanOpts po = plan_opts(format, d);
    Planner pl(po);
    apply_schedule(pl, s, n);
    Plan &plan = pl.finish();
    EncodeResult res{};
    c->prezero_ptr = nullptr;
    if (((uintptr_t)d_out & 3) == 0 && cap >= 16) {
        (void)hipSetDevice(c->device);
        const uint64_t bytes = cap / 4 * 4;
        if (hipEventRecord(c->ev_fork, c->stream) == hipSuccess && hipStreamWaitEvent(c->side_stream, c->ev_fork, 0) == hipSuccess &&
            hipMemsetAsync(d_out, 0, bytes, c->side_stream) == hipSuccess && hipEventRecord(c->ev_zero, c->side_stream) == hipSuccess) {
            c->prezero_ptr = d_out;
            c->prezero_bytes = bytes;
        }
    }
    for (;;) {
        if ((rc = encode_prepare(c, plan, po, (const uint8_t *)d_in, n, format == LFX_GZIP ? 1 : format == LFX_ZLIB ? 2 : 0))) {
            if (c->prezero_ptr) (void)hipEventSynchronize(c->ev_zero);
            c->prezero_ptr = nullptr;
            return rc;
        }
        rc = encode_emit(c, format, true, 0, true, n, hdr.data(), (uint32_t)hdr.size(), 8 * (uint64_t)hdr.size(),
                         (uint8_t *)d_out, cap, &res);
        if (match_violation(c, res)) continue;
        break;
    }
    if (c->prezero_ptr) (void)hipEventSynchronize(c->ev_zero);
    c->prezero_ptr = nullptr;
    if (rc) return rc;
    if (out_len) *out_len = res.out_bytes;
    if (c->idx_enc) return idx_encode_cand(c, plan);
    return LFX_OK;
} LFX_ABI_CATCH

extern "C" int lfx_encode_batch_device(lfx_ctx *cc, int format, const lfx_encode_opts *o, const lfx_schedule *s, uint32_t count,
                                       const void *d_in, const uint64_t *in_off, const uint64_t *in_len, void *d_out,
                                       const uint64_t *out_off, const uint64_t *out_cap, uint64_t *out_len, int32_t *status) try {
    if (!cc) return LFX_E_DEVICE;
    Ctx *c = reinterpret_cast<Ctx *>(cc);
    std::lock_guard<std::recursive_mutex> lock(c->mu);
    if (format < 0 || format > 2 || (count && (!in_off || !in_len || !out_off || !out_cap))) return LFX_E_ARG;
    lfx_encode_opts d = norm_opts(o);
    int rc = check_opts(d);
    if (rc) { c->set_error("option outside the reference's domain"); return rc; }
    std::vector<uint8_t> hdr;
    if ((rc = container_header(format, d, hdr))) { c->set_error("bad container options"); return rc; }
    if (!count) return LFX_OK;
    (void)hipSetDevice(c->device);
    hipStream_t st = c->stream;
    const PlanOpts po = plan_opts(format, d);
    const uint32_t trailer = format == LFX_GZIP ? 8 : format == LFX_ZLIB ? 4 : 0;
    Plan plan;
    std::vector<BatchStream> streams(count);
    uint64_t in_extent = 0, out_lo = ~0ull, out_hi = 0;
    for (uint32_t i = 0; i < count; i++) {
        if (out_off[i] & 3) { c->set_error("output offsets must be 4-byte aligned"); return LFX_E_ARG; }
        Planner pl(po);
        apply_schedule(pl, s, in_len[i]);
        Plan &p = pl.finish();
        const uint32_t c0 = (uint32_t)plan.chunks.size(), b0 = (uint32_t)plan.blocks.size();
        for (ChunkDesc ch : p.chunks) {
            ch.in_off += in_off[i]; ch.code_off += plan.n_codes_cap; ch.block += b0; ch.tile_base += plan.n_tiles;
            ch.vis_base += plan.n_vis; ch.seg_base += plan.n_segs;
            plan.chunks.push_back(ch);
        }
        for (BlockDesc b : p.blocks) { b.in_off += in_off[i]; b.first_chunk += c0; plan.blocks.push_back(b); }
        plan.n_codes_cap += p.n_codes_cap; plan.n_tiles += p.n_tiles; plan.n_vis += p.n_vis; plan.n_segs += p.n_segs;
        streams[i] = BatchStream{in_off[i], in_len[i], out_off[i], out_cap[i], b0, (uint32_t)p.blocks.size()};
        in_extent = std::max(in_extent, in_off[i] + in_len[i]);
        out_lo = std::min(out_lo, out_off[i]);
        out_hi = std::max(out_hi, out_off[i] + out_cap[i]);
    }
    {
        std::vector<uint32_t> order(count);
        for (uint32_t i = 0; i < count; i++) order[i] = i;
        std::sort(order.begin(), order.end(), [&](uint32_t a, uint32_t b) { return out_off[a] < out_off[b]; });
        for (uint32_t k = 0; k + 1 < count; k++)
            if (out_off[order[k]] + out_cap[order[k]] > out_off[order[k + 1]]) {
                c->set_error("the output ranges of two streams overlap");
                return LFX_E_ARG;
            }
    }
    const uint32_t nblocks = (uint32_t)plan.blocks.size();
    const size_t sz_streams = sizeof(BatchStream) * count;
    DevBuf &sb = c->d_dec_streams;
    if ((rc = sb.reserve(sz_streams + (4 + 4 + 8 + 4 + 8) * (size_t)count + hdr.size() + 64))) return rc;
    BatchStream *d_streams = (BatchStream *)sb.p;
    uint64_t *d_end = (uint64_t *)((uint8_t *)sb.p + sz_streams);
    uint64_t *d_len = d_end + count;
    uint32_t *d_crc = (uint32_t *)(d_len + count), *d_adler = d_crc + count;
    int32_t *d_status = (int32_t *)(d_adler + count);
    uint8_t *d_hdr = (uint8_t *)(d_status + count);
    std::vector<uint64_t> h_len(count);
    std::vector<int32_t> h_status(count);
    EncodeResult res{};
    for (;;) {
        if ((rc = encode_prepare(c, plan, po, (const uint8_t *)d_in, in_extent, 0))) return rc;
        HIP_TRY(hipMemcpyAsync(d_streams, streams.data(), sz_streams, hipMemcpyHostToDevice, st));
        if (!hdr.empty()) HIP_TRY(hipMemcpyAsync(d_hdr, hdr.data(), hdr.size(), hipMemcpyHostToDevice, st));
        if (trailer)
            LAUNCH_TRY(launch_checksum_ranges(st, (const uint8_t *)d_in, count, (const uint64_t *)d_streams, sizeof(BatchStream) / 8,
                                              (const uint64_t *)d_streams + 1, sizeof(BatchStream) / 8, d_crc, d_adler));
        c->phase("checksum");
        HIP_TRY(hipMemsetAsync((uint8_t *)d_out + out_lo, 0, out_hi - out_lo, st));
        EncodeResult *dres = (EncodeResult *)c->d_res.p;
        LAUNCH_TRY(launch_offsets_batch(st, d_streams, count, (const BlockDesc *)c->d_blocks.p, (const BlockCodes *)c->d_bc.p,
                                        (uint32_t)hdr.size(), trailer, (uint64_t *)c->d_block_start.p, d_end, d_status, dres));
        LAUNCH_TRY(launch_pack(st, (const uint8_t *)d_in, in_extent, (const ChunkDesc *)c->d_chunks.p, c->cur_nchunks,
                               (const BlockDesc *)c->d_blocks.p, nblocks, c->cur_ntiles, (const uint32_t *)c->d_codes.p,
                               (const uint32_t *)c->d_ncodes.p, (const BlockCodes *)c->d_bc.p, (const uint64_t *)c->d_block_start.p,
                               (uint32_t *)c->d_tile_bits.p, (uint64_t *)c->d_tile_start.p, dres, 0, (uint32_t *)d_out, c->cur_tile_map));
        c->phase("pack");
        LAUNCH_TRY(launch_frame_batch(st, format, d_streams, count, d_hdr, (uint32_t)hdr.size(), d_end, d_crc, d_adler, dres,
                                      (uint32_t *)d_out, d_len));
        HIP_TRY(hipMemcpyAsync(c->h_res, dres, sizeof(EncodeResult), hipMemcpyDeviceToHost, st));
        HIP_TRY(hipMemcpyAsync(h_len.data(), d_len, 8ull * count, hipMemcpyDeviceToHost, st));
        HIP_TRY(hipMemcpyAsync(h_status.data(), d_status, 4ull * count, hipMemcpyDeviceToHost, st));
        c->phase("frame");
        HIP_TRY(hipStreamSynchronize(st));
        res = *(EncodeResult *)c->h_res;
        if (match_violation(c, res)) continue;
        break;
    }
    for (uint32_t i = 0; i < count; i++) {
        if (status) status[i] = res.status ? h_status[i] : LFX_OK;
        if (out_len) out_len[i] = res.status ? 0 : h_len[i];
    }
    if (res.status) {
        c->set_error("output capacity of a stream too small (status[] says which): the call is void, the output span holds no stream");
        return LFX_E_NOSPACE;
    }
    return LFX_OK;
} LFX_ABI_CATCH

extern "C" int lfx_encode_host(lfx_ctx *cc, int format, const lfx_encode_opts *o, const lfx_schedule *s,
                               const void *in, uint64_t n, void *out, uint64_t cap, uint64_t *out_len) try {
    if (!cc) return LFX_E_DEVICE;
    Ctx *c = reinterpret_cast<Ctx *>(cc);
    std::lock_guard<std::recursive_mutex> lock(c->mu);
    (void)hipSetDevice(c->device);
    uint64_t bound = lfx_encode_bound(n, o, s);
    if (bound == 0) { c->set_error("option outside the reference's domain"); return LFX_E_ARG; }
    int rc;
    if ((rc = c->d_io_in.reserve(std::max<uint64_t>(n, 4)))) return rc;
    if ((rc = c->d_io_out.reserve(bound))) return rc;
    if ((rc = host_to_device(c, c->d_io_in.p, in, n, c->stream))) { c->set_error("host to device copy failed"); return rc; }
    uint64_t len = 0;
    rc = lfx_encode_device(cc, format, o, s, c->d_io_in.p, n, c->d_io_out.p, bound & ~3ull, &len);
    if (rc) { (void)hipStreamSynchronize(c->stream); return rc; }
    if (len > cap) { c->set_error("output capacity too small"); return LFX_E_NOSPACE; }
    if ((rc = device_to_host(c, out, c->d_io_out.p, len, c->stream))) { c->set_error("device to host copy failed"); return rc; }
    if (out_len) *out_len = len;
    return LFX_OK;
} LFX_ABI_CATCH

static const uint8_t BGZF_EXTRA[6] = {0x42, 0x43, 0x02, 0x00, 0x00, 0x00};
static const uint32_t BGZF_MAX_MEMBER = 65536, BGZF_EOF_LEN = 28;
static const uint64_t BGZF_MAX_SLICE = 65505;
static int members_check(uint64_t member_size, uint32_t flags, const lfx_encode_opts *o, const lfx_schedule *s, lfx_encode_opts *d,
                         const char **why) {
    *d = norm_opts(o);
    if (flags & ~(uint32_t)LFX_MEMBERS_BGZF) { *why = "flags: unknown bit"; return LFX_E_ARG; }
    if (member_size == 0) { *why = "member_size: must not be 0"; return LFX_E_ARG; }
    if (check_opts(*d)) { *why = "block_size / max_length: outside the reference's domain"; return LFX_E_ARG; }
    if (!(flags & LFX_MEMBERS_BGZF)) return LFX_OK;
    if (member_size > BGZF_MAX_SLICE) { *why = "member_size: a BGZF member holds at most 65505 bytes"; return LFX_E_ARG; }
    if (d->extra) { *why = "extra: BGZF carries its own BC subfield"; return LFX_E_ARG; }
    if (d->filename) { *why = "filename: a BGZF header is 18 bytes"; return LFX_E_ARG; }
    if (d->comment) { *why = "comment: a BGZF header is 18 bytes"; return LFX_E_ARG; }
    if (d->hcrc) { *why = "hcrc: a BGZF header is 18 bytes"; return LFX_E_ARG; }
    if (s && s->kind != LFX_SCHED_SINGLE) { *why = "schedule: BGZF needs LFX_SCHED_SINGLE"; return LFX_E_ARG; }
    if (d->block_size <= member_size && member_size + 36 > BGZF_MAX_MEMBER) {
        *why = "block_size: with block_size <= member_size a BGZF member holds at most 65500 bytes";
        return LFX_E_ARG;
    }
    d->extra = BGZF_EXTRA;
    d->extra_len = sizeof BGZF_EXTRA;
    return LFX_OK;
}
struct MemberSlices { uint64_t full, last; bool have_last; uint64_t count() const { return full + (have_last ? 1 : 0); } };
static MemberSlices member_slices(uint64_t n, uint64_t member_size, uint32_t flags) {
    MemberSlices m{n / member_size, n % member_size, n % member_size != 0};
    if (n == 0 && !(flags & LFX_MEMBERS_BGZF)) m.have_last = true;
    return m;
}

extern "C" uint64_t lfx_encode_members_bound(uint64_t n, uint64_t member_size, uint32_t flags, const lfx_encode_opts *o,
                                             const lfx_schedule *s) try {
    lfx_encode_opts d;
    const char *why = nullptr;
    if (members_check(member_size, flags, o, s, &d, &why)) return 0;
    const bool bgzf = (flags & LFX_MEMBERS_BGZF) != 0;
    const MemberSlices ms = member_slices(n, member_size, flags);
    auto term = [&](uint64_t len) { const uint64_t b = lfx_encode_bound(len, o, s); return bgzf ? std::min<uint64_t>(b, BGZF_MAX_MEMBER) : b; };
    return (ms.full ? ms.full * term(member_size) : 0) + (ms.have_last ? term(ms.last) : 0) + (bgzf ? BGZF_EOF_LEN : 0);
} catch (...) { return 0; }

extern "C" int lfx_encode_members_device(lfx_ctx *cc, const lfx_encode_opts *o, const lfx_schedule *s, uint64_t member_size,
                                         uint32_t flags, const void *d_in, uint64_t n, void *d_out, uint64_t cap, uint64_t *out_len,
                                         lfx_member *members, uint32_t max_members, uint32_t *n_members) try {
    if (!cc) return LFX_E_DEVICE;
    Ctx *c = reinterpret_cast<Ctx *>(cc);
    std::lock_guard<std::recursive_mutex> lock(c->mu);
    if (out_len) *out_len = 0;
    if (n_members) *n_members = 0;
    lfx_encode_opts d;
    const char *why = nullptr;
    int rc = members_check(member_size, flags, o, s, &d, &why);
    if (rc) { c->set_error(why); return rc; }
    if (((uintptr_t)d_out & 3) != 0) { c->set_error("output buffer must be 4-byte aligned"); return LFX_E_ARG; }
    const bool bgzf = (flags & LFX_MEMBERS_BGZF) != 0;
    std::vector<uint8_t> hdr;
    if ((rc = container_header(LFX_GZIP, d, hdr))) { c->set_error("extra: longer than 65535 bytes"); return rc; }
    const MemberSlices ms = member_slices(n, member_size, flags);
    if (ms.count() >= 0xFFFFFFFFull) { c->set_error("member_size: more than 2^32 - 2 members"); return LFX_E_ARG; }
    const uint32_t count = (uint32_t)ms.count();
    (void)hipSetDevice(c->device);
    hipStream_t st = c->stream;
    if (!count) {
        static const uint8_t eof[BGZF_EOF_LEN] = {0x1f, 0x8b, 0x08, 0x04, 0, 0, 0, 0, 0, 0xff, 0x06, 0, 0x42, 0x43,
                                                  0x02, 0,    0x1b, 0,    3, 0, 0, 0, 0, 0,    0,    0, 0,    0};
        if (cap < BGZF_EOF_LEN) { c->set_error("output capacity too small"); return LFX_E_NOSPACE; }
        HIP_TRY(hipMemcpyAsync(d_out, eof, BGZF_EOF_LEN, hipMemcpyHostToDevice, st));
        HIP_TRY(hipStreamSynchronize(st));
        if (out_len) *out_len = BGZF_EOF_LEN;
        return LFX_OK;
    }
    const PlanOpts po = plan_opts(LFX_GZIP, d);
    Plan pfull, plast;
    if (ms.full) { Planner pl(po); apply_schedule(pl, s, member_size); pfull = std::move(pl.finish()); }
    if (ms.have_last) { Planner pl(po); apply_schedule(pl, s, ms.last); plast = std::move(pl.finish()); }
    if (bgzf) {
        PlanOpts ps = po;
        ps.no_compression = true;
        for (int k = 0; k < 2; k++) {
            if (k == 0 ? !ms.full : !ms.have_last) continue;
            const Plan &pc = k == 0 ? pfull : plast;
            Planner pl(ps);
            apply_schedule(pl, s, k == 0 ? member_size : ms.last);
            const Plan &pr = pl.finish();
            bool same = pr.blocks.size() == pc.blocks.size();
            for (size_t b = 0; same && b < pr.blocks.size(); b++)
                same = pr.blocks[b].in_off == pc.blocks[b].in_off && pr.blocks[b].in_len == pc.blocks[b].in_len &&
                       pr.blocks[b].final == pc.blocks[b].final && pr.blocks[b].align_after == pc.blocks[b].align_after;
            if (!same) { c->set_error("block_size: the stored form of a member has other blocks than the compressed form"); return LFX_E_UNSUPPORTED; }
        }
    }
    if ((uint64_t)ms.full * pfull.chunks.size() + plast.chunks.size() > 0xFFFFFFF0ull ||
        (uint64_t)ms.full * pfull.blocks.size() + plast.blocks.size() > 0xFFFFFFF0ull ||
        (uint64_t)ms.full * pfull.n_segs + plast.n_segs > 0xFFFFFFF0ull) {
        c->set_error("member_size: too many blocks for one call");
        return LFX_E_ARG;
    }
    Plan plan;
    plan.chunks.reserve(ms.full * pfull.chunks.size() + plast.chunks.size());
    plan.blocks.reserve(ms.full * pfull.blocks.size() + plast.blocks.size());
    auto append = [&](const Plan &p, uint64_t in_off) {
        const uint32_t c0 = (uint32_t)plan.chunks.size(), b0 = (uint32_t)plan.blocks.size();
        for (ChunkDesc ch : p.chunks) {
            ch.in_off += in_off; ch.code_off += plan.n_codes_cap; ch.block += b0; ch.tile_base += plan.n_tiles;
            ch.vis_base += plan.n_vis; ch.seg_base += plan.n_segs;
            plan.chunks.push_back(ch);
        }
        for (BlockDesc b : p.blocks) { b.in_off += in_off; b.first_chunk += c0; plan.blocks.push_back(b); }
        plan.n_codes_cap += p.n_codes_cap; plan.n_tiles += p.n_tiles; plan.n_vis += p.n_vis; plan.n_segs += p.n_segs;
    };
    for (uint64_t m = 0; m < ms.full; m++) append(pfull, m * member_size);
    if (ms.have_last) append(plast, ms.full * member_size);
    MembersGeom g{};
    g.n = n; g.member_size = member_size; g.count = count;
    g.bpm = (uint32_t)(ms.full ? pfull.blocks.size() : plast.blocks.size());
    g.bpm_last = (uint32_t)(ms.have_last ? plast.blocks.size() : pfull.blocks.size());
    g.hdr_len = (uint32_t)hdr.size(); g.bgzf = bgzf ? 1u : 0u;
    const uint32_t nblocks = (uint32_t)plan.blocks.size();
    const uint32_t nwg = (count + 255) / 256;
    const size_t cnt = std::max<uint32_t>(count, 1);
    DevBuf &sb = c->d_dec_streams;
    if ((rc = sb.reserve((sizeof(lfx_member) + 8 + 8 + 4 + 4) * cnt + 8 * (size_t)std::max<uint32_t>(nwg, 1) + hdr.size() + 64))) return rc;
    lfx_member *d_members = (lfx_member *)sb.p;
    uint64_t *d_local = (uint64_t *)(d_members + cnt), *d_mlen = d_local + cnt, *d_wg = d_mlen + cnt;
    uint32_t *d_crc = (uint32_t *)(d_wg + std::max<uint32_t>(nwg, 1)), *d_adler = d_crc + cnt;
    uint8_t *d_hdr = (uint8_t *)(d_adler + cnt);
    const uint64_t bound = lfx_encode_members_bound(n, member_size, flags, o, s);
    const uint64_t fill = std::min(cap, bound);
    bool prezero = fill && hipEventRecord(c->ev_fork, st) == hipSuccess && hipStreamWaitEvent(c->side_stream, c->ev_fork, 0) == hipSuccess &&
                   hipMemsetAsync(d_out, 0, fill, c->side_stream) == hipSuccess && hipEventRecord(c->ev_zero, c->side_stream) == hipSuccess;
    c->prezero_ptr = nullptr;
    EncodeResult res{};
    const uint32_t n_rec = members ? std::min(count, max_members) : 0;
    auto body = [&]() -> int {
        for (;;) {
            int rc2;
            if ((rc2 = encode_prepare(c, plan, po, (const uint8_t *)d_in, n, 0))) return rc2;
            HIP_TRY(hipMemcpyAsync(d_hdr, hdr.data(), hdr.size(), hipMemcpyHostToDevice, st));
            EncodeResult *dres = (EncodeResult *)c->d_res.p;
            LAUNCH_TRY(launch_members_layout(st, g, (BlockDesc *)c->d_blocks.p, (const BlockCodes *)c->d_bc.p, d_local, d_mlen, d_wg, cap,
                                             (uint64_t *)c->d_block_start.p, d_members, dres));
            if (bgzf) c->up_dev[1] = 0;
            c->phase("members_layout");
            LAUNCH_TRY(launch_checksum_ranges(st, (const uint8_t *)d_in, count, (const uint64_t *)d_members, sizeof(lfx_member) / 8,
                                              (const uint64_t *)d_members + 1, sizeof(lfx_member) / 8, d_crc, d_adler));
            c->phase("checksum");
            if (prezero) HIP_TRY(hipStreamWaitEvent(st, c->ev_zero, 0));
            else if (fill) HIP_TRY(hipMemsetAsync(d_out, 0, fill, st));
            prezero = false;
            LAUNCH_TRY(launch_pack(st, (const uint8_t *)d_in, n, (const ChunkDesc *)c->d_chunks.p, c->cur_nchunks,
                                   (const BlockDesc *)c->d_blocks.p, nblocks, c->cur_ntiles, (const uint32_t *)c->d_codes.p,
                                   (const uint32_t *)c->d_ncodes.p, (const BlockCodes *)c->d_bc.p, (const uint64_t *)c->d_block_start.p,
                                   (uint32_t *)c->d_tile_bits.p, (uint64_t *)c->d_tile_start.p, dres, 0, (uint32_t *)d_out, c->cur_tile_map));
            c->phase("pack");
            LAUNCH_TRY(launch_members_frame(st, g, d_hdr, d_members, d_crc, dres, (uint32_t *)d_out));
            HIP_TRY(hipMemcpyAsync(c->h_res, dres, sizeof(EncodeResult), hipMemcpyDeviceToHost, st));
            if (n_rec) HIP_TRY(hipMemcpyAsync(members, d_members, sizeof(lfx_member) * (size_t)n_rec, hipMemcpyDeviceToHost, st));
            c->phase("frame");
            HIP_TRY(hipStreamSynchronize(st));
            res = *(EncodeResult *)c->h_res;
            if (match_violation(c, res)) continue;
            return LFX_OK;
        }
    };
    rc = body();
    if (prezero) (void)hipEventSynchronize(c->ev_zero);
    if (rc) return rc;
    if (n_members) *n_members = count;
    if (res.status) { c->set_error("output capacity too small"); return LFX_E_NOSPACE; }
    if (out_len) *out_len = res.out_bytes;
    return LFX_OK;
} LFX_ABI_CATCH

extern "C" int lfx_encode_members_host(lfx_ctx *cc, const lfx_encode_opts *o, const lfx_schedule *s, uint64_t member_size,
                                       uint32_t flags, const void *in, uint64_t n, void *out, uint64_t cap, uint64_t *out_len,
                                       lfx_member *members, uint32_t max_members, uint32_t *n_members) try {
    if (!cc) return LFX_E_DEVICE;
    Ctx *c = reinterpret_cast<Ctx *>(cc);
    std::lock_guard<std::recursive_mutex> lock(c->mu);
    (void)hipSetDevice(c->device);
    if (out_len) *out_len = 0;
    if (n_members) *n_members = 0;
    lfx_encode_opts d;
    const char *why = nullptr;
    int rc = members_check(member_size, flags, o, s, &d, &why);
    if (rc) { c->set_error(why); return rc; }
    const uint64_t bound = lfx_encode_members_bound(n, member_size, flags, o, s);
    if ((rc = c->d_io_in.reserve(std::max<uint64_t>(n, 4)))) return rc;
    if ((rc = c->d_io_out.reserve(std::max<uint64_t>(bound, 4)))) return rc;
    if ((rc = host_to_device(c, c->d_io_in.p, in, n, c->stream))) { c->set_error("host to device copy failed"); return rc; }
    uint64_t len = 0;
    rc = lfx_encode_members_device(cc, o, s, member_size, flags, c->d_io_in.p, n, c->d_io_out.p, std::min(cap, bound), &len, members,
                                   max_members, n_members);
    if (rc) { (void)hipStreamSynchronize(c->stream); return rc; }
    if ((rc = device_to_host(c, out, c->d_io_out.p, len, c->stream))) { c->set_error("device to host copy failed"); return rc; }
    if (out_len) *out_len = len;
    return LFX_OK;
} LFX_ABI_CATCH

extern "C" int lfx_members_gzi(const lfx_member *members, uint32_t n_members, void *buf, uint64_t cap, uint64_t *len) {
    if (n_members && !members) return LFX_E_ARG;
    const uint64_t pairs = n_members ? n_members - 1 : 0, need = 8 + 16 * pairs;
    if (len) *len = need;
    if (cap < need || !buf) return cap < need ? LFX_E_NOSPACE : LFX_E_ARG;
    uint8_t *p = (uint8_t *)buf;
    auto put64 = [&](uint64_t v) { for (int i = 0; i < 8; i++) *p++ = (uint8_t)(v >> (8 * i)); };
    put64(pairs);
    for (uint32_t i = 1; i < n_members; i++) { put64(members[i].out_off); put64(members[i].in_off); }
    return LFX_OK;
}

extern "C" int lfx_encode_shard_prezero(lfx_ctx *cc, void *d_out, uint64_t cap) try {
    if (!cc) return LFX_E_DEVICE;
    Ctx *c = reinterpret_cast<Ctx *>(cc);
    std::lock_guard<std::recursive_mutex> lock(c->mu);
    if (c->prezero_ptr) (void)hipEventSynchronize(c->ev_zero);
    c->prezero_ptr = nullptr;
    if (!d_out || ((uintptr_t)d_out & 3) != 0 || cap < 16) return LFX_OK;
    (void)hipSetDevice(c->device);
    const uint64_t bytes = cap / 4 * 4;
    if (hipEventRecord(c->ev_fork, c->stream) == hipSuccess && hipStreamWaitEvent(c->side_stream, c->ev_fork, 0) == hipSuccess &&
        hipMemsetAsync(d_out, 0, bytes, c->side_stream) == hipSuccess && hipEventRecord(c->ev_zero, c->side_stream) == hipSuccess) {
        c->prezero_ptr = d_out;
        c->prezero_bytes = bytes;
    }
    return LFX_OK;
} LFX_ABI_CATCH

extern "C" int lfx_encode_shard_prepare(lfx_ctx *cc, int format, const lfx_encode_opts *o, const lfx_schedule *s,
                                        const void *d_in, uint64_t n, int is_first, int is_last,
                                        lfx_shard_info *info) try {
    if (!cc) return LFX_E_DEVICE;
    Ctx *c = reinterpret_cast<Ctx *>(cc);
    std::lock_guard<std::recursive_mutex> lock(c->mu);
    lfx_encode_opts d = norm_opts(o);
    int rc = check_opts(d);
    if (rc) return rc;
    if (d.no_compression) { c->set_error("sharded encode of stored blocks is not supported (their size depends on the bit phase)"); return LFX_E_UNSUPPORTED; }
    PlanOpts po = plan_opts(format, d);
    Planner pl(po);
    apply_schedule(pl, s, n);
    Plan *plan;
    if (is_last) {
        plan = &pl.finish();
    } else {
        plan = &pl.plan();
        Planner probe = pl;
        Plan &fin = probe.finish();
        if (fin.blocks.size() != plan->blocks.size() + 1 || fin.blocks.back().in_len != 0) {
            c->set_error("shard boundary is not a block boundary under this write schedule");
            return LFX_E_ARG;
        }
        plan->n_codes_cap = fin.n_codes_cap;
        plan->n_tiles = plan->chunks.empty() ? 0 : plan->chunks.back().tile_base + div_up(plan->chunks.back().len + 1, PACK_TILE);
    }
    c->shard_hdr.clear();
    if (is_first && (rc = container_header(format, d, c->shard_hdr))) return rc;
    c->shard_format = format;
    c->shard_last = is_last != 0;
    hipStream_t st = c->stream;
    EncodeResult r{};
    for (;;) {
        if ((rc = encode_prepare(c, *plan, po, (const uint8_t *)d_in, n, 3))) return rc;
        LAUNCH_TRY(launch_offsets(st, (const BlockDesc *)c->d_blocks.p, c->cur_nblocks, (const BlockCodes *)c->d_bc.p,
                                  0, ~0ull, (uint64_t *)c->d_block_start.p, (EncodeResult *)c->d_res.p));
        HIP_TRY(hipMemcpyAsync(c->h_res, c->d_res.p, sizeof(EncodeResult), hipMemcpyDeviceToHost, st));
        HIP_TRY(hipStreamSynchronize(st));
        r = *(EncodeResult *)c->h_res;
        if (match_violation(c, r)) continue;
        break;
    }
    info->total_bits = r.end_bit;
    info->n_bytes = n;
    info->crc32 = r.crc32;
    info->adler32 = r.adler32;
    return LFX_OK;
} LFX_ABI_CATCH

extern "C" int lfx_encode_shard_emit(lfx_ctx *cc, uint64_t start_bit, uint32_t combined_check, uint64_t total_n,
                                     void *d_out, uint64_t cap, uint64_t *out_len) try {
    if (!cc) return LFX_E_DEVICE;
    Ctx *c = reinterpret_cast<Ctx *>(cc);
    std::lock_guard<std::recursive_mutex> lock(c->mu);
    const uint64_t rel_start = c->shard_hdr.empty() ? (start_bit & 7) : start_bit;
    EncodeResult res;
    int rc = encode_emit(c, c->shard_format, c->shard_last, combined_check, false, total_n,
                         c->shard_hdr.data(), (uint32_t)c->shard_hdr.size(), rel_start, (uint8_t *)d_out, cap, &res);
    if (rc) return rc;
    if (out_len) *out_len = c->shard_last ? res.out_bytes : (res.end_bit + 7) / 8;
    return LFX_OK;
} LFX_ABI_CATCH

extern "C" int lfx_shard_place_device(lfx_ctx *cc, void *d_member, uint64_t cap, const void *d_part, uint64_t part_len,
                                      uint64_t start_bit, int is_first) try {
    if (!cc) return LFX_E_DEVICE;
    Ctx *c = reinterpret_cast<Ctx *>(cc);
    std::lock_guard<std::recursive_mutex> lock(c->mu);
    (void)hipSetDevice(c->device);
    const uint64_t at = is_first ? 0 : start_bit / 8;
    if (at + part_len > cap) { c->set_error("member buffer too small"); return LFX_E_NOSPACE; }
    if (part_len == 0) return LFX_OK;
    uint8_t *dst = (uint8_t *)d_member + at;
    const uint8_t *src = (const uint8_t *)d_part;
    const bool shared = !is_first && (start_bit & 7) != 0;
    if (shared) {
        LAUNCH_TRY(launch_or_byte(c->stream, dst, src));
        if (part_len > 1) HIP_TRY(hipMemcpyAsync(dst + 1, src + 1, part_len - 1, hipMemcpyDeviceToDevice, c->stream));
    } else {
        HIP_TRY(hipMemcpyAsync(dst, src, part_len, hipMemcpyDeviceToDevice, c->stream));
    }
    HIP_TRY(hipStreamSynchronize(c->stream));
    return LFX_OK;
} LFX_ABI_CATCH

struct lfx_encoder {
    Ctx *c;
    int format;
    lfx_encode_opts o;
    std::string filename, comment;
    std::vector<uint8_t> extra;
    PlanOpts po;
    lfx_write_cb w;
    lfx_flush_cb f;
    void *user;
    PinVec pending;
    PinVec h_out;
    PinVec inflight_buf, h_res;
    bool inflight = false, inflight_final = false;
    uint64_t inflight_n = 0, inflight_bound = 0;
    Plan inflight_plan;
    hipEvent_t ev_out = nullptr, ev_small = nullptr;
    Planner *pl = nullptr;
    uint64_t total_in = 0, encoded_in = 0;
    uint32_t crc = 0, adler = 1;
    uint8_t carry = 0;
    uint32_t carry_bits = 0;
    bool finished = false, failed = false;
    std::string err;
    DevBuf d_in, d_out;
    int mode = 0;
    struct CodeBlock { uint64_t n_codes; uint32_t type, final; };
    std::vector<uint32_t> codes;
    std::vector<CodeBlock> cblocks;
    uint64_t closed_codes = 0, open_codes = 0;
    bool final_closed = false;
};

static int enc_emit_bytes(lfx_encoder *e, const uint8_t *p, size_t n) {
    if (!n) return LFX_OK;
    int64_t r = e->w(e->user, p, n);
    if (r != (int64_t)n) { e->err = "write callback failed"; e->failed = true; return LFX_E_IO; }
    return LFX_OK;
}

struct EncCollected { uint64_t whole = 0; bool have = false; };

static int enc_launch(lfx_encoder *e, Plan &&plan, uint64_t n, bool final) {
    Ctx *c = e->c;
    int rc;
    if ((rc = e->d_in.reserve(std::max<uint64_t>(n, 4)))) return rc;
    const uint64_t bound = n + n / 4 + 1024 * (uint64_t)plan.blocks.size() + 128;
    if ((rc = e->d_out.reserve(bound))) return rc;
    if (e->h_res.size() < 256) e->h_res.resize(256);
    e->inflight_buf.assign(e->pending.begin() + (std::ptrdiff_t)n, e->pending.end());
    e->inflight_buf.swap(e->pending);
    if (n && hipMemcpyAsync(e->d_in.p, e->inflight_buf.data(), n, hipMemcpyHostToDevice, c->stream) != hipSuccess) return LFX_E_DEVICE;
    const uint8_t prefix[1] = {e->carry};
    if ((rc = encode_prepare(c, plan, e->po, (const uint8_t *)e->d_in.p, n, e->format == LFX_GZIP ? 1 : e->format == LFX_ZLIB ? 2 : 0))) { e->err = c->err; return rc; }
    rc = encode_emit(c, LFX_DEFLATE, false, 0, true, 0, prefix, e->carry_bits ? 1 : 0, e->carry_bits, (uint8_t *)e->d_out.p,
                     bound & ~3ull, nullptr, (EncodeResult *)e->h_res.data());
    if (rc) { e->err = c->err; return rc; }
    e->inflight = true;
    e->inflight_final = final;
    e->inflight_n = n;
    e->inflight_bound = bound;
    e->inflight_plan = std::move(plan);
    return LFX_OK;
}

static int enc_collect(lfx_encoder *e, EncCollected *out) {
    Ctx *c = e->c;
    out->have = false;
    if (!e->inflight) return LFX_OK;
    e->inflight = false;
    if (hipStreamSynchronize(c->stream) != hipSuccess) return LFX_E_DEVICE;
    EncodeResult res = *(const EncodeResult *)e->h_res.data();
    const uint64_t n = e->inflight_n;
    int rc = LFX_OK;
    if (match_violation(c, res)) {
        const uint8_t prefix[1] = {e->carry};
        if ((rc = encode_prepare(c, e->inflight_plan, e->po, (const uint8_t *)e->d_in.p, n, e->format == LFX_GZIP ? 1 : e->format == LFX_ZLIB ? 2 : 0))) { e->err = c->err; return rc; }
        rc = encode_emit(c, LFX_DEFLATE, false, 0, true, 0, prefix, e->carry_bits ? 1 : 0, e->carry_bits, (uint8_t *)e->d_out.p,
                         e->inflight_bound & ~3ull, &res);
        if (rc) { e->err = c->err; return rc; }
    }
    if (res.status != 0) { c->set_error("output capacity too small"); e->err = c->err; return LFX_E_NOSPACE; }
    if (e->format == LFX_GZIP) e->crc = e->encoded_in == 0 ? res.crc32 : lfx_crc32_combine(e->crc, res.crc32, n);
    if (e->format == LFX_ZLIB) e->adler = e->encoded_in == 0 ? res.adler32 : lfx_adler32_combine(e->adler, res.adler32, n);
    e->encoded_in += n;
    const uint64_t whole = e->inflight_final ? (res.end_bit + 7) / 8 : res.end_bit / 8;
    e->h_out.resize(whole + 1);
    uint8_t *slot = e->h_res.data() + 128;
    if (hipMemcpyAsync(slot, (const uint8_t *)e->d_out.p + whole, 1, hipMemcpyDeviceToHost, c->stream) != hipSuccess ||
        hipEventRecord(e->ev_small, c->stream) != hipSuccess ||
        (whole && hipMemcpyAsync(e->h_out.data(), e->d_out.p, whole, hipMemcpyDeviceToHost, c->stream) != hipSuccess) ||
        hipEventRecord(e->ev_out, c->stream) != hipSuccess || hipEventSynchronize(e->ev_small) != hipSuccess) return LFX_E_DEVICE;
    e->carry_bits = e->inflight_final ? 0 : (uint32_t)(res.end_bit & 7);
    e->carry = e->carry_bits ? *slot : 0;
    out->whole = whole;
    out->have = true;
    return LFX_OK;
}

static int enc_run(lfx_encoder *e, bool final, bool drain = true) {
    Ctx *c = e->c;
    std::lock_guard<std::recursive_mutex> lock(c->mu);
    (void)hipSetDevice(c->device);
    if (!e->ev_out && (hipEventCreateWithFlags(&e->ev_out, hipEventDisableTiming) != hipSuccess ||
                       hipEventCreateWithFlags(&e->ev_small, hipEventDisableTiming) != hipSuccess)) return LFX_E_DEVICE;
    if (final) e->pl->finish();
    const uint64_t n = final ? e->pending.size() : e->pl->closed_bytes();
    Plan plan = final ? std::move(e->pl->plan()) : e->pl->take_closed();
    int rc;
    EncCollected prev;
    if ((rc = enc_collect(e, &prev))) return rc;
    const bool launched = !plan.blocks.empty();
    if (launched && (rc = enc_launch(e, std::move(plan), n, final))) return rc;
    if (prev.have) {
        if (hipEventSynchronize(e->ev_out) != hipSuccess) return LFX_E_DEVICE;
        if ((rc = enc_emit_bytes(e, e->h_out.data(), prev.whole))) return rc;
    }
    if (drain && launched) {
        EncCollected cur;
        if ((rc = enc_collect(e, &cur))) return rc;
        if (cur.have) {
            if (hipEventSynchronize(e->ev_out) != hipSuccess) return LFX_E_DEVICE;
            if ((rc = enc_emit_bytes(e, e->h_out.data(), cur.whole))) return rc;
        }
    }
    return LFX_OK;
}

static int enc_run_codes(lfx_encoder *e) {
    Ctx *c = e->c;
    std::lock_guard<std::recursive_mutex> lock(c->mu);
    (void)hipSetDevice(c->device);
    if (e->cblocks.empty()) return LFX_OK;
    Plan plan;
    std::vector<uint32_t> chunk_codes;
    uint64_t code_cursor = 0, tile_cursor = 0;
    for (const lfx_encoder::CodeBlock &cb : e->cblocks) {
        BlockDesc b{};
        b.type = cb.type;
        b.final = cb.final;
        b.first_chunk = (uint32_t)plan.chunks.size();
        if (cb.type != BT_RAW) {
            ChunkDesc ch{};
            ch.len = cb.n_codes - 1;
            ch.code_off = code_cursor;
            ch.block = (uint32_t)plan.blocks.size();
            ch.flags = CH_LAST_IN_BLOCK;
            ch.tile_base = tile_cursor;
            code_cursor += cb.n_codes;
            tile_cursor += div_up(cb.n_codes, PACK_TILE);
            plan.chunks.push_back(ch);
            chunk_codes.push_back((uint32_t)cb.n_codes);
            b.n_chunks = 1;
        }
        plan.blocks.push_back(b);
    }
    if (e->final_closed) plan.blocks.back().align_after = 1;
    plan.n_codes_cap = code_cursor;
    plan.n_tiles = tile_cursor;
    const uint64_t n = e->pending.size();
    int rc;
    if ((rc = e->d_in.reserve(std::max<uint64_t>(n, 4)))) return rc;
    const uint64_t bound = 6 * code_cursor + 1024 * (uint64_t)plan.blocks.size() + 128;
    if ((rc = e->d_out.reserve(bound))) return rc;
    if (n && hipMemcpyAsync(e->d_in.p, e->pending.data(), n, hipMemcpyHostToDevice, c->stream) != hipSuccess) return LFX_E_DEVICE;
    EncodeResult res{};
    uint8_t prefix[1] = {e->carry};
    const HostCodes hc{e->codes.data(), code_cursor, chunk_codes.data()};
    if ((rc = encode_prepare(c, plan, e->po, (const uint8_t *)e->d_in.p, n, e->format == LFX_GZIP ? 1 : e->format == LFX_ZLIB ? 2 : 0, &hc))) { e->err = c->err; return rc; }
    rc = encode_emit(c, LFX_DEFLATE, false, 0, true, 0, prefix, e->carry_bits ? 1 : 0, e->carry_bits, (uint8_t *)e->d_out.p, bound & ~3ull, &res);
    if (rc) { e->err = c->err; return rc; }
    if (n) {
        if (e->format == LFX_GZIP) e->crc = e->encoded_in == 0 ? res.crc32 : lfx_crc32_combine(e->crc, res.crc32, n);
        if (e->format == LFX_ZLIB) e->adler = e->encoded_in == 0 ? res.adler32 : lfx_adler32_combine(e->adler, res.adler32, n);
        e->encoded_in += n;
    }
    const uint64_t whole = e->final_closed ? (res.end_bit + 7) / 8 : res.end_bit / 8;
    e->h_out.resize(whole + 1);
    if (hipMemcpyAsync(e->h_out.data(), e->d_out.p, whole + 1, hipMemcpyDeviceToHost, c->stream) != hipSuccess ||
        hipStreamSynchronize(c->stream) != hipSuccess) return LFX_E_DEVICE;
    e->carry_bits = e->final_closed ? 0 : (uint32_t)(res.end_bit & 7);
    e->carry = e->carry_bits ? e->h_out[whole] : 0;
    e->pending.clear();
    e->codes.erase(e->codes.begin(), e->codes.begin() + (std::ptrdiff_t)e->closed_codes);
    e->closed_codes = 0;
    e->cblocks.clear();
    return enc_emit_bytes(e, e->h_out.data(), whole);
}

static const uint64_t ENC_BATCH_CODES = 2ull << 20;
static const uint64_t ENC_BATCH_BYTES_DEFAULT = 8ull << 20;
static uint64_t enc_batch_bytes(const lfx_encoder *e) { return e->c->diag.enc_batch_mb > 0 ? (uint64_t)e->c->diag.enc_batch_mb << 20 : ENC_BATCH_BYTES_DEFAULT; }

extern "C" int lfx_encoder_write_codes(lfx_encoder *e, const uint32_t *codes, size_t n_codes, const uint8_t *raw, size_t n_raw,
                                       int end_block) try {
    if (!e || e->finished || e->final_closed || end_block < 0 || end_block > 2 || (n_codes && !codes) || (n_raw && !raw)) return LFX_E_ARG;
    if (e->failed) return LFX_E_IO;
    if (e->mode == 1 || e->po.no_compression) { e->err = "lfx_encoder_write_codes on an encoder that takes bytes"; return LFX_E_ARG; }
    for (size_t i = 0; i < n_codes; i++) {
        const uint32_t dist = codes[i] & 0xFFFFu, val = codes[i] >> 16;
        if (dist == 0 ? val > 255 : (val < 3 || val > MAX_LENGTH || dist > MAX_WINDOW)) { e->err = "code word outside Code's domain"; return LFX_E_ARG; }
    }
    e->mode = 2;
    e->codes.insert(e->codes.end(), codes, codes + n_codes);
    e->open_codes += n_codes;
    e->pending.insert(e->pending.end(), raw, raw + n_raw);
    e->total_in += n_raw;
    if (end_block) {
        e->codes.push_back(CODE_EOB);
        e->cblocks.push_back(lfx_encoder::CodeBlock{e->open_codes + 1, e->po.dynamic_huffman ? (uint32_t)BT_DYNAMIC : (uint32_t)BT_FIXED,
                                                    end_block == 2 ? 1u : 0u});
        e->closed_codes += e->open_codes + 1;
        e->open_codes = 0;
        if (end_block == 2) e->final_closed = true;
        else if (e->closed_codes >= ENC_BATCH_CODES || e->pending.size() >= enc_batch_bytes(e)) {
            int rc = enc_run_codes(e);
            if (rc) { e->failed = true; return rc; }
        }
    }
    return LFX_OK;
} LFX_ABI_CATCH

extern "C" void lfx_encoder_free(lfx_encoder *e);
extern "C" lfx_encoder *lfx_encoder_new(lfx_ctx *cc, int format, const lfx_encode_opts *o, lfx_write_cb w,
                                        lfx_flush_cb f, void *user, int *status) try {
    if (!cc || !w) { if (status) *status = cc ? LFX_E_ARG : LFX_E_DEVICE; return nullptr; }
    lfx_encode_opts d = norm_opts(o);
    int rc = check_opts(d);
// ... 253 lines not shown
```

libflate_amd/csrc/lfx_ctx.h:

```cpp
#pragma once
#include <hip/hip_runtime.h>

#include <mutex>
#include <string>
#include <vector>

#include "lfx_common.h"
#include "lfx_device.h"
#include <string.h>

#include "lfx_hostio.h"

namespace lfx {

struct DevBuf {
    void *p = nullptr;
    size_t cap = 0;
    uint32_t gen = 0;
    int reserve(size_t bytes);
    void release();
};

struct Diag {
    bool debug = false;
    bool match_v1 = false;
    bool match_v5 = false;
    int r7_cap = 0;
    int match_parts = 1;
    bool no_serial = false;
    bool batch_serial = false;
    bool no_markers = false;
    bool no_pieces = false;
    bool no_final_cand = false;
    bool window_chain = false;
    int free_shift = -1;
    bool no_small_scan = false;
    bool two_pass = false;
    bool no_pin_slots = false;
    int find2_exp = 0;
    bool hist_separate = false;
    bool store_tight = false;
    int enc_batch_mb = 0;
    int pocr_max = 100;
    void read();
};

struct RangeState {
    int state = -1;
    uint64_t total = 0, before = 0, max_len = 0;
    uint8_t *d_out = nullptr;
    uint32_t nsu = 0;
};

struct Ctx {
    int device = 0;
    RangeState range;
    std::vector<uint8_t> range_stored;
    std::vector<uint64_t> range_temp_off;
    std::vector<uint32_t> range_cap;
    Diag diag;
    int n_cu = 0;
    hipStream_t own_stream = nullptr, stream = nullptr;
    hipStream_t side_stream = nullptr;
    hipEvent_t ev_fork = nullptr, ev_join = nullptr, ev_zero = nullptr;
    hipEvent_t ev_part[4] = {}, ev_res = nullptr;
    const void *prezero_ptr = nullptr;
    uint64_t prezero_bytes = 0;
    std::recursive_mutex mu;
    std::string err;
    void set_error(const std::string &e) { err = e; }

    DevBuf d_chunks, d_blocks, d_segs, d_pwgs, d_cd, d_md, d_codes, d_ncodes, d_hist, d_bc, d_block_start, d_tile_bits,
        d_tile_start, d_ck, d_res, d_small, d_hdr, d_io_in, d_io_out, d_vis, d_segtmp, d_stage, d_chunkmap, d_glnk, d_ucount;
    std::vector<uint8_t> up_shadow[4];
    uint64_t up_dev[4] = {0, 0, 0, 0};
    DevBuf d_dec_streams, d_dec_state, d_dec_tmp, d_dec_cand, d_dec_blocks, d_dec_tabs, d_dec_sym, d_dec_win, d_dec_maps,
        d_dec_temp, d_dec_lanesx;
    DevBuf d_idx_tasks, d_idx_probe, d_idx_stage;
    DevBuf d_idx_enc;
    struct IdxCollect *idx = nullptr;
    struct IdxCollect *idx_enc = nullptr;
    std::vector<DevBuf *> all_bufs() {
        return {&d_chunks, &d_blocks, &d_segs, &d_pwgs, &d_cd, &d_md, &d_codes, &d_ncodes, &d_hist, &d_bc, &d_block_start,
                &d_tile_bits, &d_tile_start, &d_ck, &d_res, &d_small, &d_hdr, &d_io_in, &d_io_out, &d_vis, &d_segtmp, &d_stage, &d_chunkmap, &d_glnk, &d_ucount,
                &d_dec_streams, &d_dec_state, &d_dec_tmp, &d_dec_cand, &d_dec_blocks, &d_dec_tabs, &d_dec_sym, &d_dec_win, &d_dec_maps,
                &d_dec_temp, &d_dec_lanesx, &d_idx_tasks, &d_idx_probe, &d_idx_stage, &d_idx_enc};
    }
    void *h_res = nullptr;
    static constexpr size_t PIN_ARENA = 1u << 20;
    size_t pin_used = 0;
    struct PinDown { void *slot, *dst; size_t n; };
    std::vector<PinDown> pin_pending;
    void pin_reset() { pin_used = 0; pin_pending.clear(); }
    void *pin_take(size_t n) {
        const size_t at = (pin_used + 63) & ~(size_t)63;
        if (!h_res || diag.no_pin_slots || at + n > PIN_ARENA) return nullptr;
        pin_used = at + n;
        return (uint8_t *)h_res + 4096 + at;
    }
    hipError_t small_up(void *dev, const void *host, size_t n, hipStream_t st) {
        if (!n) return hipSuccess;
        void *slot = pin_take(n);
        if (!slot) return hipMemcpyAsync(dev, host, n, hipMemcpyHostToDevice, st);
        memcpy(slot, host, n);
        return hipMemcpyAsync(dev, slot, n, hipMemcpyHostToDevice, st);
    }
    hipError_t small_down(void *host, const void *dev, size_t n, hipStream_t st) {
        if (!n) return hipSuccess;
        void *slot = pin_take(n);
        if (!slot) return hipMemcpyAsync(host, dev, n, hipMemcpyDeviceToHost, st);
        pin_pending.push_back({slot, host, n});
        return hipMemcpyAsync(slot, dev, n, hipMemcpyDeviceToHost, st);
    }
    hipError_t small_sync(hipStream_t st) {
        const hipError_t e = hipStreamSynchronize(st);
        for (const PinDown &d : pin_pending) memcpy(d.dst, d.slot, d.n);
        pin_pending.clear();
        return e;
    }

    uint32_t cur_nchunks = 0, cur_nblocks = 0;
    uint64_t cur_ntiles = 0, cur_n = 0;
    const uint32_t *cur_tile_map = nullptr;
    const uint8_t *cur_in = nullptr;
    bool force_match_v1 = false;
    uint64_t match_fallbacks = 0;
    HostIo hostio;
    static constexpr size_t POOL_MAX = 8;
    std::vector<PinVec> pin_pool;
    std::vector<DevBuf> dev_pool;
    PinVec take_pin() {
        std::lock_guard<std::recursive_mutex> lock(mu);
        if (pin_pool.empty()) return PinVec();
        size_t best = 0;
        for (size_t i = 1; i < pin_pool.size(); i++)
            if (pin_pool[i].capacity() > pin_pool[best].capacity()) best = i;
        PinVec v = std::move(pin_pool[best]);
        pin_pool.erase(pin_pool.begin() + (std::ptrdiff_t)best);
        v.clear();
        return v;
    }
    void give_pin(PinVec &&v) {
        std::lock_guard<std::recursive_mutex> lock(mu);
        if (v.capacity() && pin_pool.size() < POOL_MAX) { v.clear(); pin_pool.push_back(std::move(v)); }
    }
    DevBuf take_dev() {
        std::lock_guard<std::recursive_mutex> lock(mu);
        if (dev_pool.empty()) return DevBuf();
        DevBuf b = dev_pool.back();
        dev_pool.pop_back();
        return b;
    }
    void give_dev(DevBuf &b) {
        std::lock_guard<std::recursive_mutex> lock(mu);
        if (b.p && dev_pool.size() < POOL_MAX) dev_pool.push_back(b);
        else b.release();
        b = DevBuf();
    }
    std::vector<uint8_t> shard_hdr;
    int shard_format = 0;
    bool shard_last = false;

    int timing_on = 0;
    bool timing_fine() const { return timing_on >= 2; }
    hipEvent_t ev[17] = {};
    char ev_name[17][24] = {};
    int n_ev = 0;
    void phase(const char *name);
};

struct HostCodes {
    const uint32_t *codes;
    uint64_t n_codes;
    const uint32_t *chunk_codes;
};
int encode_prepare(Ctx *c, const struct Plan &plan, const struct PlanOpts &po, const uint8_t *d_in,
                   uint64_t n, int ck_mode, const HostCodes *hc = nullptr);

}
```

libflate_amd/csrc/lfx_device.h:

```cpp
#pragma once
#include <hip/hip_runtime.h>
#include <stdint.h>

#include "../../include/lfx.h"
#include "lfx_common.h"

namespace lfx {

struct SegDesc {
    uint32_t chunk;
    uint32_t start;
    uint32_t len;
    uint32_t lnk_base;
};
constexpr uint32_t SEG_POSITIONS = 256 * 1024;

struct EncodeResult {
    uint64_t end_bit;
    uint64_t out_bytes;
    uint32_t status;
    uint32_t crc32;
    uint32_t adler32;
    uint32_t match_flags;
};

struct BatchStream {
    uint64_t in_off, in_len;
    uint64_t out_off, out_cap;
    uint32_t first_block, n_blocks;
};

struct ParseWg {
    uint32_t chunk;
    uint32_t seg0;
};

int launch_match(hipStream_t st, const uint8_t *in, uint64_t in_bytes, const ChunkDesc *chunks,
                 const SegDesc *segs, uint32_t nsegs, uint32_t window, uint32_t max_len, uint32_t *md,
                 uint64_t *dbg = nullptr);
int launch_match7(hipStream_t st, const uint8_t *in, uint64_t in_bytes, const ChunkDesc *chunks, const SegDesc *segs,
                  uint32_t nsegs, uint32_t window, uint16_t *cd, uint32_t *glnk ,
                  uint64_t *umask , uint32_t *flags, uint64_t *dbg = nullptr);
int launch_resolve7(hipStream_t st, const ChunkDesc *chunks, const SegDesc *segs, uint32_t nsegs, uint32_t window, uint16_t *cd,
                    const uint32_t *glnk, const uint64_t *umask, uint32_t *ulist ,
                    uint32_t *ucount ,
                    uint32_t hop_cap = 0 );
int launch_match5(hipStream_t st, const uint8_t *in, uint64_t in_bytes, const ChunkDesc *chunks, const SegDesc *segs,
                  uint32_t nsegs, uint32_t window, uint16_t *cd, uint16_t *glnk, uint32_t *flags, uint64_t *dbg = nullptr);
int launch_md_to_cd(hipStream_t st, const uint32_t *md, uint64_t n, uint16_t *cd);
int launch_parse(hipStream_t st, const uint8_t *in, uint64_t in_bytes, const ChunkDesc *chunks, uint32_t nchunks,
                 uint32_t nsegs, const ParseWg *wgs, uint32_t nwgs, const uint16_t *cd, uint32_t max_len, uint64_t *vis,
                 uint32_t *seg_tmp, uint32_t *codes, uint32_t *ncodes, uint32_t *stage ,
                 const uint32_t *seg_map, int stop_after = 0 ,
                 uint64_t *dbg = nullptr ,
                 uint32_t *hist = nullptr ,
                 uint32_t emit_per = 0 ,
                 uint32_t emit_parts = 0 ,
                 hipEvent_t ev_walked = nullptr ,
                 const uint32_t *mflags = nullptr ,
                 int start_at = 0 );
struct ZeroSpan { uint32_t *p; uint32_t n; };
int launch_chunk_maps(hipStream_t st, const ChunkDesc *chunks, uint32_t nchunks, uint64_t ntiles, uint32_t nsegs,
                      uint32_t *tile_map, uint32_t *seg_map, ZeroSpan z0 = ZeroSpan{nullptr, 0}, ZeroSpan z1 = ZeroSpan{nullptr, 0},
                      ZeroSpan z2 = ZeroSpan{nullptr, 0});
int launch_histogram(hipStream_t st, const ChunkDesc *chunks, uint32_t nchunks, uint32_t split,
                     const uint32_t *codes, const uint32_t *ncodes, uint32_t *hist);
int launch_huffman(hipStream_t st, const BlockDesc *blocks, uint32_t nblocks, const uint32_t *hist,
                   BlockCodes *bc, uint64_t *dbg = nullptr);
int launch_offsets(hipStream_t st, const BlockDesc *blocks, uint32_t nblocks, const BlockCodes *bc,
                   uint64_t start_bit, uint64_t cap_bits, uint64_t *block_start, EncodeResult *res);
int launch_offsets_batch(hipStream_t st, const BatchStream *streams, uint32_t count, const BlockDesc *blocks, const BlockCodes *bc,
                         uint32_t hdr_len, uint32_t trailer_len, uint64_t *block_start, uint64_t *stream_end, int32_t *status,
                         EncodeResult *res);
int launch_frame_batch(hipStream_t st, int format, const BatchStream *streams, uint32_t count, const uint8_t *hdr, uint32_t hdr_len,
                       const uint64_t *stream_end, const uint32_t *crc, const uint32_t *adler, const EncodeResult *res, uint32_t *out,
                       uint64_t *out_len);
struct MembersGeom {
    uint64_t n, member_size;
    uint32_t count;
    uint32_t bpm, bpm_last;
    uint32_t hdr_len;
    uint32_t bgzf;
};
int launch_members_layout(hipStream_t st, const MembersGeom &g, BlockDesc *blocks, const BlockCodes *bc, uint64_t *local_off,
                          uint64_t *mlen, uint64_t *wg_sum, uint64_t cap, uint64_t *block_start, lfx_member *members,
                          EncodeResult *res);
int launch_members_frame(hipStream_t st, const MembersGeom &g, const uint8_t *hdr, const lfx_member *members, const uint32_t *crc,
                         const EncodeResult *res, uint32_t *out);
int launch_pack(hipStream_t st, const uint8_t *in, uint64_t in_bytes, const ChunkDesc *chunks,
                uint32_t nchunks, const BlockDesc *blocks, uint32_t nblocks, uint64_t ntiles,
                const uint32_t *codes, const uint32_t *ncodes, const BlockCodes *bc,
                const uint64_t *block_start, uint32_t *tile_bits, uint64_t *tile_start,
                const EncodeResult *res, uint64_t out_base_bit, uint32_t *out, const uint32_t *tile_map);
inline uint32_t ck_span(uint64_t n) { return n <= (64ull << 20) ? 8192u : 65536u; }
inline uint64_t ck_nspans(uint64_t n) { return div_up(n ? n : 1, ck_span(n)); }
int launch_checksum(hipStream_t st, const uint8_t *in, uint64_t n, uint32_t *crc_part,
                    uint32_t *a_part, uint32_t *b_part, EncodeResult *res,
                    int mode = 3)   ;
int launch_checksum_part(hipStream_t st, const uint8_t *in, uint64_t n, uint32_t *crc_part, uint32_t *a_part, uint32_t *b_part,
                         EncodeResult *res, int mode, uint32_t part, uint32_t nparts);
int launch_checksum_ranges(hipStream_t st, const uint8_t *data, uint32_t count, const uint64_t *off,
                           uint32_t off_stride, const uint64_t *len, uint32_t len_stride, uint32_t *crc, uint32_t *adler);
int launch_or_byte(hipStream_t st, uint8_t *dst, const uint8_t *src);
int launch_put_bytes(hipStream_t st, const uint8_t *d_bytes, uint32_t n, uint64_t at_byte, uint32_t *out);
int launch_trailer(hipStream_t st, int format, uint32_t isize, uint64_t out_base_bit,
                   EncodeResult *res, uint32_t *out);

}
```

libflate_amd/csrc/lfx_encode_kernels.hip:

```cpp
#include <hip/hip_runtime.h>
#include <stdint.h>

#include "lfx_common.h"
#include "lfx_device.h"
#include "lfx_huff.h"

namespace lfx {

struct ByteSrc {
    gptr_u32 w;
    uint64_t shift;
    uint64_t nbytes;
    __device__ __forceinline__ uint32_t load4(uint64_t off) const {
        uint64_t a = off + shift;
        uint64_t idx = a >> 2;
        uint32_t sh = (uint32_t)a & 3;
        uint64_t last = (nbytes + shift + 3) >> 2;
        uint32_t w0 = idx < last ? w[idx] : 0;
        uint32_t w1 = (sh != 0 && idx + 1 < last) ? w[idx + 1] : 0;
        return __builtin_amdgcn_alignbyte(w1, w0, sh);
    }
    __device__ __forceinline__ uint32_t load1(uint64_t off) const {
        uint64_t a = off + shift;
        return (w[a >> 2] >> (((uint32_t)a & 3) * 8)) & 0xFF;
// ... 121 lines not shown
        }
        if (need > loaded_to) loaded_to = need;
        if (do_head && t_head + MTILE - swept_at > 16384) {
            for (uint32_t i = tid; i < (1u << HASH_BITS); i += MATCH_THREADS) {
                const uint32_t d = (t_head - head[i]) & 0xFFFFu;
                if (d == 0 || d > MAX_WINDOW) head[i] = (uint16_t)(t_head - HEAD_FAR);
            }
            swept_at = t_head;
        }
        const uint32_t fidx = (wave - 1) * 64 + lane;
        bool fin_valid = false;
        uint32_t fin_e = LK_DONE;
        if (wave > 0 && do_fin) {
            const uint32_t sk = st_k[(fin_idx % 3) * MTILE + fidx];
            if (sk != 0xFFFFFFFFu) {
                fin_valid = true;
                const uint32_t key = sk & 0xFFFFFFu, f = sk >> 24;
                const uint32_t w_p = ring_fwd(wring_off(t_fin), fidx, WRING), s_p = ring_fwd(t_fin % PRING, fidx, PRING);
                uint32_t d = f & 0x3F;
                bool same = (f & 0x40) != 0;
                if (d == 0) {
                    d = (t_fin + fidx - hvs[(fin_idx & 1) * MTILE + fidx]) & 0xFFFFu;
                    if (d > MAX_WINDOW) d = 0;
                    if (d) same = (win_at(win32, ring_back(w_p, d, WRING)) & 0xFFFFFFu) == key;
                }
                uint32_t e = LK_DONE | d;
                if (d && same) {
                    if (d > fidx) {
                        const uint32_t pq = prevd[ring_back(s_p, d, PRING)];
                        e = LK_DONE | (pq ? d + pq : 0);
                    } else e = fidx - d;
                }
                fin_e = e;
                lk[fidx] = e;
                cd[(fin_idx & 1) * MTILE + fidx] = (uint16_t)((d && same) ? d : 0);
            }
        }
        lds_barrier();
        const uint64_t c1 = dbg ? clock64() : 0;
        if (wave == 0) {
            if (do_head) {
                const uint32_t *stl = st_k + (head_idx % 3) * MTILE;
                uint16_t *hv_out = hvs + (head_idx & 1) * MTILE;
                uint32_t hvv[NSUB];
#pragma unroll
                for (uint32_t sub = 0; sub < NSUB; ++sub) {
                    const uint32_t sk = stl[sub * 64 + lane];
                    const uint32_t hh = hash3(sk & 0xFFFFFFu) & ((1u << HASH_BITS) - 1);
                    hvv[sub] = head[hh];
                    if (sk != 0xFFFFFFFFu && ((sk >> 24) & 0x80)) head[hh] = (uint16_t)(t_head + sub * 64 + lane);
                }
#pragma unroll
                for (uint32_t sub = 0; sub < NSUB; ++sub) hv_out[sub * 64 + lane] = (uint16_t)hvv[sub];
            }
        } else {
            if (do_fin) {
                uint32_t e = fin_e;
                while (__ballot(fin_valid && !(e & LK_DONE))) {
                    if (fin_valid && !(e & LK_DONE)) {
                        const uint32_t eq = lk[e];
                        if (eq & LK_DONE) {
                            const uint32_t dq = eq & ~LK_DONE;
                            e = LK_DONE | (dq ? (fidx - e) + dq : 0);
                        } else e = eq;
                        lk[fidx] = e;
                    }
                }
                if (fin_valid) {
                    const uint32_t dist = e & ~LK_DONE;
                    prevd[ring_fwd(t_fin % PRING, fidx, PRING)] = (uint16_t)(dist <= MAX_WINDOW ? dist : 0);
                }
            }
            if (it >= 0) {
            const uint32_t w_res = wring_off(t_res), s_res = t_res % PRING;
            const uint32_t pos = t_res + (wave - 1) * 64 + lane;
            const bool act = pos >= q0 && pos < q1;
            uint32_t dist = 0, l = 0, lim = 0, oa = 0, ob = 0, lit_byte = 0;
            bool found = false;
            if (act) {
                const uint32_t w_pos = ring_fwd(w_res, (wave - 1) * 64 + lane, WRING);
                const uint32_t s_pos = ring_fwd(s_res, (wave - 1) * 64 + lane, PRING);
                const uint32_t key = st_k[((uint32_t)it % 3) * MTILE + (wave - 1) * 64 + lane] & 0xFFFFFFu;
                const uint32_t known = cd[((uint32_t)it & 1) * MTILE + (wave - 1) * 64 + lane];
                lit_byte = key & 0xFFu;
                uint32_t d = prevd[s_pos];
                if (known) { dist = known; found = dist <= window; d = 0; }
                while (d != 0) {
                    dist += d;
                    if (dist > window || dist > pos) break;
                    if ((win_at(win32, ring_back(w_pos, dist, WRING)) & 0xFFFFFFu) == key) { found = true; break; }
                    d = prevd[ring_back(s_pos, dist, PRING)];
                }
                if (found) {
                    lim = n - (pos + 3);
                    if (lim > max_len - 3) lim = max_len - 3;
                    oa = ring_fwd(w_pos, 3, WRING); ob = ring_back(oa, dist, WRING);
                    while (l < lim && l < 16) {
                        const uint32_t x = win_at(win32, oa) ^ win_at(win32, ob);
                        if (x) { l += (uint32_t)__builtin_ctz(x) >> 3; break; }
                        l += 4;
                        oa += 4; if (oa >= WRING) oa -= WRING;
                        ob += 4; if (ob >= WRING) ob -= WRING;
                    }
                }
            }
            uint64_t lm = __ballot(found && l == 16 && l < lim);
            while (lm) {
                const uint32_t sl = (uint32_t)__builtin_ctzll(lm);
                lm &= lm - 1;
                const uint32_t boa = __builtin_amdgcn_readlane(oa, sl), bob = __builtin_amdgcn_readlane(ob, sl);
                const uint32_t blim = __builtin_amdgcn_readlane(lim, sl);
                const uint32_t off = 4 * lane;
                uint32_t x = 0;
                if (16 + off < blim) {
                    uint32_t a = boa + off, b = bob + off;
                    if (a >= WRING) a -= WRING;
                    if (b >= WRING) b -= WRING;
                    x = win_at(win32, a) ^ win_at(win32, b);
                }
                const uint64_t mis = __ballot(x != 0);
                uint32_t res = blim;
                if (mis) {
                    const uint32_t fl = (uint32_t)__builtin_ctzll(mis);
                    const uint32_t cand = 16 + off + ((uint32_t)__builtin_ctz(x | 0x80000000u) >> 3);
                    res = __builtin_amdgcn_readlane(cand, fl);
                }
                if (lane == sl) l = res;
            }
            if (act) {
                uint32_t out = lit_byte << 16;
                if (found) {
                    if (l > lim) l = lim;
                    out = ((3 + l) << 16) | dist;
                }
                md[ch.in_off + pos] = out;
            }
            }
            predigest(pre_idx);
        }
        const uint64_t c2 = dbg ? clock64() : 0;
        lds_barrier();
        const uint64_t c3 = dbg ? clock64() : 0;
        cy_load += c1 - c0; cy_work += c2 - c1; cy_wait += c3 - c2;
    }
    if (dbg && blockIdx.x == 0 && lane == 0) {
        uint64_t *d = dbg + wave * 8;
        d[0] = cy_load; d[1] = cy_work; d[2] = cy_wait; d[3] = 0; d[4] = 0; d[5] = ntiles;
    }
}

__global__ __launch_bounds__(256) void chunk_maps_kernel(const ChunkDesc *__restrict__ chunks, uint32_t nchunks,
                                                         uint64_t ntiles, uint32_t nsegs,
                                                         uint32_t *__restrict__ tile_map, uint32_t *__restrict__ seg_map,
                                                         ZeroSpan z0, ZeroSpan z1, ZeroSpan z2) {
    {
        const uint32_t nthreads = 256u * gridDim.x * gridDim.y, me = (blockIdx.y * gridDim.x + blockIdx.x) * 256u + threadIdx.x;
        for (uint32_t i = me; i < z0.n; i += nthreads) z0.p[i] = 0;
        for (uint32_t i = me; i < z1.n; i += nthreads) z1.p[i] = 0;
        for (uint32_t i = me; i < z2.n; i += nthreads) z2.p[i] = 0;
    }
    const uint32_t c = blockIdx.x;
    const ChunkDesc ch = chunks[c];
    const uint64_t t1 = c + 1 < nchunks ? chunks[c + 1].tile_base : ntiles;
    const uint32_t s1 = c + 1 < nchunks ? chunks[c + 1].seg_base : nsegs;
    for (uint64_t t = ch.tile_base + blockIdx.y * 256 + threadIdx.x; t < t1; t += 256ull * gridDim.y) tile_map[t] = c;
    for (uint32_t q = ch.seg_base + blockIdx.y * 256 + threadIdx.x; q < s1; q += 256u * gridDim.y) seg_map[q] = c;
}

constexpr int HIST_STRIDE = 320;

__global__ __launch_bounds__(256) void histogram_kernel(const ChunkDesc *__restrict__ chunks,
                                                        const uint32_t *__restrict__ codes,
                                                        const uint32_t *__restrict__ ncodes,
                                                        uint32_t *__restrict__ hist) {
    constexpr uint32_t HREP = 4;
    __shared__ uint32_t hh[HREP * HIST_STRIDE];
    uint32_t *h = hh + (threadIdx.x & (HREP - 1)) * HIST_STRIDE;
    const uint32_t c = blockIdx.x;
    const ChunkDesc ch = chunks[c];
    for (uint32_t i = threadIdx.x; i < HREP * HIST_STRIDE; i += 256) hh[i] = 0;
    __syncthreads();
    const uint32_t n = ncodes[c];
    const uint32_t per = (uint32_t)div_up(n, gridDim.y);
    const uint32_t lo = blockIdx.y * per, hi = min(n, lo + per);
    const uint32_t *p = codes + ch.code_off;
    constexpr uint32_t HLOADS = 16;
    for (uint32_t i0 = lo + threadIdx.x; i0 < hi; i0 += HLOADS * 256) {
        uint32_t v[HLOADS];
#pragma unroll
        for (uint32_t q = 0; q < HLOADS; ++q) v[q] = p[min(i0 + 256 * q, hi - 1)];
#pragma unroll
        for (uint32_t q = 0; q < HLOADS; ++q) {
            if (i0 + 256 * q >= hi) break;
            const uint32_t dist = v[q] & 0xFFFFu, val = v[q] >> 16;
            if (dist == 0) {
                atomicAdd(&h[val], 1u);
            } else {
                uint32_t eb, ex;
                atomicAdd(&h[len_symbol(val, eb, ex)], 1u);
                atomicAdd(&h[288 + dist_symbol(dist, eb, ex)], 1u);
            }
        }
    }
    __syncthreads();
    uint32_t *g = hist + (uint64_t)ch.block * HIST_STRIDE;
    for (uint32_t i = threadIdx.x; i < HIST_STRIDE; i += 256) {
        uint32_t v = 0;
#pragma unroll
        for (uint32_t r = 0; r < HREP; ++r) v += hh[r * HIST_STRIDE + i];
        if (v) atomicAdd(&g[i], v);
    }
}

constexpr int HUFF_THREADS = 320;
__global__ __launch_bounds__(HUFF_THREADS) void huffman_kernel(const BlockDesc *__restrict__ blocks,
                                                               const uint32_t *__restrict__ hist,
                                                               BlockCodes *__restrict__ bc, uint64_t *__restrict__ dbg) {
    __shared__ HuffScratch S;
    const uint32_t b = blockIdx.x;
    const uint32_t type = blocks[b].type;
    if (type == BT_RAW) return;
    huff_block_build(hist + (uint64_t)b * HIST_STRIDE, type, &bc[b], S, (int)threadIdx.x, HUFF_THREADS);
    if (dbg && b == 0 && threadIdx.x < 24) dbg[threadIdx.x] = S.stamp[threadIdx.x];
}

__global__ __launch_bounds__(256) void offsets_kernel(const BlockDesc *__restrict__ blocks, uint32_t nblocks,
                                                      const BlockCodes *__restrict__ bc, uint64_t start_bit,
                                                      uint64_t cap_bits, uint64_t *__restrict__ block_start,
                                                      EncodeResult *__restrict__ res) {
    __shared__ uint64_t s_bits[256];
    __shared__ uint32_t s_kind[256];
    __shared__ uint64_t s_bit;
    if (threadIdx.x == 0) s_bit = start_bit;
    for (uint32_t b0 = 0; b0 < nblocks; b0 += 256) {
        const uint32_t b = b0 + threadIdx.x;
        if (b < nblocks) {
            const BlockDesc bd = blocks[b];
            s_kind[threadIdx.x] = (bd.type == BT_RAW ? 1u : 0u) | (bd.align_after ? 2u : 0u);
            s_bits[threadIdx.x] = bd.type == BT_RAW ? 32 + 8 * bd.in_len : bc[b].body_bits;
        }
        const uint32_t cnt = min(256u, nblocks - b0);
        const uint32_t my_kind = b < nblocks ? s_kind[threadIdx.x] : 0u;
        const bool odd = b < nblocks && (my_kind & 1u || ((my_kind & 2u) && threadIdx.x + 1 != cnt));
        const int serial = __syncthreads_or(odd ? 1 : 0);
        if (!serial) {
            const uint32_t lane = threadIdx.x & 63, wave = threadIdx.x >> 6;
            uint64_t x = b < nblocks ? s_bits[threadIdx.x] : 0ull;
            const uint64_t mine = x;
            for (int o = 1; o < 64; o <<= 1) { const uint64_t y = __shfl_up(x, o); if ((int)lane >= o) x += y; }
            __shared__ uint64_t s_wsum[4];
            if (lane == 63) s_wsum[wave] = x;
            __syncthreads();
            uint64_t pre = s_bit;
            for (uint32_t w = 0; w < wave; ++w) pre += s_wsum[w];
            if (b < nblocks) block_start[b] = pre + x - mine;
            __syncthreads();
            if (threadIdx.x == cnt - 1) {
                uint64_t bit = pre + x;
                if (my_kind & 2u) bit = (bit + 7) & ~7ull;
                s_bit = bit;
            }
        } else if (threadIdx.x == 0) {
            uint64_t bit = s_bit;
            for (uint32_t k = 0; k < cnt; ++k) {
                block_start[b0 + k] = bit;
                if (s_kind[k] & 1) { bit += 3; bit = (bit + 7) & ~7ull; }
                bit += s_bits[k];
                if (s_kind[k] & 2) bit = (bit + 7) & ~7ull;
            }
            s_bit = bit;
        }
        __syncthreads();
    }
    if (threadIdx.x == 0) {
        res->end_bit = s_bit;
        res->status = s_bit > cap_bits ? 1u : 0u;
    }
}

__global__ __launch_bounds__(256) void offsets_batch_kernel(const BatchStream *__restrict__ streams, uint32_t count,
                                                            const BlockDesc *__restrict__ blocks, const BlockCodes *__restrict__ bc,
                                                            uint32_t hdr_len, uint32_t trailer_len, uint64_t *__restrict__ block_start,
                                                            uint64_t *__restrict__ stream_end, int32_t *__restrict__ status,
                                                            EncodeResult *__restrict__ res) {
    const uint32_t s = blockIdx.x * 256 + threadIdx.x;
    if (s >= count) return;
    const BatchStream bs = streams[s];
    uint64_t bit = (bs.out_off + hdr_len) * 8;
    for (uint32_t b = bs.first_block; b < bs.first_block + bs.n_blocks; ++b) {
        const BlockDesc bd = blocks[b];
        block_start[b] = bit;
        if (bd.type == BT_RAW) { bit += 3; bit = (bit + 7) & ~7ull; bit += 32 + 8 * bd.in_len; }
        else bit += bc[b].body_bits;
        if (bd.align_after) bit = (bit + 7) & ~7ull;
    }
    stream_end[s] = bit;
    const bool over = bs.out_cap < hdr_len + trailer_len || bit > (bs.out_off + bs.out_cap - trailer_len) * 8;
    status[s] = over ? 7 : 0;
    if (over) atomicOr(&res->status, 1u);
}
__global__ __launch_bounds__(256) void frame_batch_kernel(int format, const BatchStream *__restrict__ streams, uint32_t count,
                                                          const uint8_t *__restrict__ hdr, uint32_t hdr_len,
                                                          const uint64_t *__restrict__ stream_end, const uint32_t *__restrict__ crc,
                                                          const uint32_t *__restrict__ adler, const EncodeResult *__restrict__ res,
                                                          uint32_t *__restrict__ out, uint64_t *__restrict__ out_len) {
    const uint32_t s = blockIdx.x * 256 + threadIdx.x;
    if (s >= count || res->status != 0) return;
    const BatchStream bs = streams[s];
    auto put = [&](uint64_t ob, uint32_t byte) { atomicOr(&out[ob >> 2], byte << (8 * (ob & 3))); };
    for (uint32_t i = 0; i < hdr_len; ++i) put(bs.out_off + i, hdr[i]);
    const uint64_t at = stream_end[s] >> 3;
    uint32_t nt = 0;
    if (format == 2) {
        const uint32_t c = bs.in_len ? crc[s] : 0u, sz = (uint32_t)bs.in_len;
        for (uint32_t i = 0; i < 4; ++i) { put(at + i, (c >> (8 * i)) & 255u); put(at + 4 + i, (sz >> (8 * i)) & 255u); }
        nt = 8;
    } else if (format == 1) {
        const uint32_t a = bs.in_len ? adler[s] : 1u;
// ... 77 lines not shown
        __syncthreads();
        if (threadIdx.x == 0) tile_bits[gt] = red[0] + red[1] + red[2] + red[3];
    }
}

__global__ __launch_bounds__(1024) void tile_scan_kernel(const ChunkDesc *__restrict__ chunks,
                                                        const BlockDesc *__restrict__ blocks,
                                                        const BlockCodes *__restrict__ bc,
                                                        const uint64_t *__restrict__ block_start,
                                                        const uint32_t *__restrict__ tile_bits,
                                                        uint64_t total_tiles,
                                                        uint32_t nchunks,
                                                        uint64_t *__restrict__ tile_start) {
    __shared__ uint64_t wsum[16];
    __shared__ uint64_t carry;
    const uint32_t b = blockIdx.x;
    const BlockDesc bd = blocks[b];
    if (bd.type == BT_RAW || bd.n_chunks == 0) return;
    const uint64_t t0 = chunks[bd.first_chunk].tile_base;
    const uint32_t lastc = bd.first_chunk + bd.n_chunks;
    const uint64_t t1 = lastc < nchunks ? chunks[lastc].tile_base : total_tiles;
    if (threadIdx.x == 0) carry = block_start[b] + 3 + bc[b].hdr_bits;
    __syncthreads();
    const uint32_t lane = threadIdx.x & 63, wave = threadIdx.x >> 6;
    const uint32_t T = blockDim.x;
    for (uint64_t base = t0; base < t1; base += T) {
        const uint64_t i = base + threadIdx.x;
        const uint64_t v = i < t1 ? tile_bits[i] : 0;
        uint64_t x = v;
        for (int o = 1; o < 64; o <<= 1) {
            const uint64_t y = __shfl_up(x, o);
            if ((int)lane >= o) x += y;
        }
        if (lane == 63) wsum[wave] = x;
        __syncthreads();
        uint64_t pre = carry;
        for (uint32_t w = 0; w < wave; ++w) pre += wsum[w];
        if (i < t1) tile_start[i] = pre + x - v;
        __syncthreads();
        if (threadIdx.x == T - 1) carry = pre + x;
        __syncthreads();
    }
}

constexpr int STAGE_WORDS64 = (PACK_TILE * 48) / 64 + 4;

__global__ __launch_bounds__(PACK_THREADS) void pack_kernel(
    const ChunkDesc *__restrict__ chunks, uint32_t nchunks, const BlockDesc *__restrict__ blocks,
    const uint32_t *__restrict__ codes, const uint32_t *__restrict__ ncodes,
    const BlockCodes *__restrict__ bc, const uint64_t *__restrict__ tile_start,
    const EncodeResult *__restrict__ res, uint64_t out_base_bit, uint32_t *__restrict__ out,
    const uint32_t *__restrict__ tile_map, uint64_t ntiles) {
    __shared__ uint32_t lit[288], dst[32];
    __shared__ uint32_t wsum[PACK_THREADS / 64];
    __shared__ unsigned long long stage[STAGE_WORDS64];
    if (res->status != 0) return;
    const uint64_t g0 = (uint64_t)blockIdx.x * PACK_TPW;
    uint32_t cm[PACK_TPW];
    uint64_t ts[PACK_TPW];
#pragma unroll
    for (uint32_t q = 0; q < PACK_TPW; ++q) {
        cm[q] = tile_map[min(g0 + q, ntiles - 1)];
        ts[q] = tile_start[min(g0 + q, ntiles - 1)];
    }
    uint32_t cur_c = 0xFFFFFFFFu, cur_block = 0xFFFFFFFFu, n = 0;
    ChunkDesc ch{};
    bool raw = false;
    uint32_t cv[PACK_PER_THREAD], cvn[PACK_PER_THREAD];
    bool have_next = false;
    const uint32_t lane = threadIdx.x & 63, wave = threadIdx.x >> 6;
#pragma unroll
    for (uint32_t q = 0; q < PACK_TPW; ++q) {
        const uint64_t gt = g0 + q;
        if (gt >= ntiles) break;
        const uint32_t c = cm[q];
        if (c != cur_c) {
            cur_c = c;
            ch = chunks[c];
            n = ncodes[c];
            raw = blocks[ch.block].type == BT_RAW;
            have_next = false;
        }
        const uint32_t lo = (uint32_t)(gt - ch.tile_base) * PACK_TILE;
        if (lo >= n || raw) { have_next = false; continue; }
        const uint32_t hi = min(n, lo + PACK_TILE);
        const uint32_t *p = codes + ch.code_off;
        const uint32_t first = lo + threadIdx.x * PACK_PER_THREAD;
        if (have_next) {
#pragma unroll
            for (int k = 0; k < PACK_PER_THREAD; ++k) cv[k] = cvn[k];
        } else {
#pragma unroll
            for (int k = 0; k < PACK_PER_THREAD; ++k) cv[k] = p[min(first + k, hi - 1)];
        }
        have_next = q + 1 < PACK_TPW && gt + 1 < ntiles && cm[q + 1 < PACK_TPW ? q + 1 : q] == c;
        if (have_next) {
#pragma unroll
            for (int k = 0; k < PACK_PER_THREAD; ++k) cvn[k] = p[min(first + PACK_TILE + k, n - 1)];
        }
        __syncthreads();
        if (ch.block != cur_block) {
            cur_block = ch.block;
            const BlockCodes *B = &bc[ch.block];
            for (uint32_t i = threadIdx.x; i < 288; i += PACK_THREADS) lit[i] = B->lit[i];
            if (threadIdx.x < 32) dst[threadIdx.x] = B->dist[threadIdx.x];
        }
        for (uint32_t i = threadIdx.x; i < STAGE_WORDS64; i += PACK_THREADS) stage[i] = 0;
        __syncthreads();
        uint64_t cb[PACK_PER_THREAD];
        uint32_t cn[PACK_PER_THREAD];
        uint32_t mine = 0;
#pragma unroll
        for (int k = 0; k < PACK_PER_THREAD; ++k) {
            const uint32_t i = first + k;
            const uint32_t nb = code_bits(cv[k], lit, dst, cb[k]);
            cn[k] = i < hi ? nb : 0u;
            cb[k] = i < hi ? cb[k] : 0ull;
            mine += cn[k];
        }
        uint32_t x = mine;
        for (int o = 1; o < 64; o <<= 1) {
            const uint32_t y = __shfl_up(x, o);
            if ((int)lane >= o) x += y;
        }
        if (lane == 63) wsum[wave] = x;
        __syncthreads();
        uint32_t pre = 0;
        for (uint32_t w = 0; w < wave; ++w) pre += wsum[w];
        const uint32_t total = wsum[0] + wsum[1] + wsum[2] + wsum[3];
        const uint64_t start = ts[q] - out_base_bit;
        const uint32_t phase = (uint32_t)start & 31;
        uint32_t bit = phase + pre + x - mine;
#pragma unroll
        for (int k = 0; k < PACK_PER_THREAD; ++k) {
            if (cn[k]) {
                const uint32_t w = bit >> 6, sh = bit & 63;
                atomicOr(&stage[w], cb[k] << sh);
                if (sh + cn[k] > 64) atomicOr(&stage[w + 1], cb[k] >> (64 - sh));
                bit += cn[k];
            }
        }
        __syncthreads();
        const uint32_t nwords = (phase + total + 31) >> 5;
        const uint32_t *s32 = (const uint32_t *)stage;
        uint32_t *o = out + (start >> 5);
        for (uint32_t i = threadIdx.x; i < nwords; i += PACK_THREADS) {
            const uint32_t v = s32[i];
            if (i == 0 || i == nwords - 1) { if (v) atomicOr(&o[i], v); }
            else o[i] = v;
        }
    }
}

__global__ __launch_bounds__(256) void block_header_kernel(
    const uint8_t *__restrict__ in, uint64_t in_bytes, const BlockDesc *__restrict__ blocks,
    const BlockCodes *__restrict__ bc, const uint64_t *__restrict__ block_start,
    const EncodeResult *__restrict__ res, uint64_t out_base_bit, uint32_t *__restrict__ out) {
    if (res->status != 0) return;
    const uint32_t b = blockIdx.x;
    const BlockDesc bd = blocks[b];
    const uint64_t start = block_start[b] - out_base_bit;
    const uint32_t first3 = (bd.final & 1) | (bd.type << 1);
    if (threadIdx.x == 0) {
        const uint32_t sh = (uint32_t)start & 31;
        atomicOr(&out[start >> 5], first3 << sh);
        if (sh > 29) atomicOr(&out[(start >> 5) + 1], first3 >> (32 - sh));
    }
    if (bd.type == BT_DYNAMIC) {
        const BlockCodes *B = &bc[b];
        const uint64_t hb = start + 3;
        const uint32_t nw = (B->hdr_bits + 31) >> 5;
        const uint32_t sh = (uint32_t)hb & 31;
        for (uint32_t i = threadIdx.x; i < nw; i += 256) {
            const uint32_t v = B->hdr[i];
            if (v == 0) continue;
            atomicOr(&out[(hb >> 5) + i], v << sh);
            if (sh) atomicOr(&out[(hb >> 5) + i + 1], v >> (32 - sh));
        }
    } else if (bd.type == BT_RAW) {
        const uint64_t byte0 = ((start + 3 + 7) >> 3);
        const uint32_t len = (uint32_t)bd.in_len;
        const ByteSrc src = make_src(in + bd.in_off, in_bytes - bd.in_off);
        const uint64_t total = 4 + (uint64_t)len;
        const uint64_t wfirst = byte0 >> 2, wlast = (byte0 + total - 1) >> 2;
        for (uint64_t w = wfirst + threadIdx.x; w <= wlast; w += 256) {
            uint32_t v = 0;
            for (int k = 0; k < 4; ++k) {
                const uint64_t ob = w * 4 + k;
                if (ob < byte0 || ob >= byte0 + total) continue;
                const uint64_t r = ob - byte0;
                uint32_t byte;
                if (r == 0) byte = len & 0xFF;
                else if (r == 1) byte = (len >> 8) & 0xFF;
                else if (r == 2) byte = (~len) & 0xFF;
                else if (r == 3) byte = ((~len) >> 8) & 0xFF;
                else byte = src.load1(r - 4);
                v |= byte << (8 * k);
            }
            if (v) atomicOr(&out[w], v);
        }
    }
}

constexpr uint32_t CK_SPAN = 65536;
constexpr uint32_t CRC_POLY = 0xEDB88320u;

__device__ __forceinline__ uint32_t gf2_mulmod(uint32_t a, uint32_t b) {
    uint32_t p = 0;
    for (int i = 0; i < 32; ++i) {
        if (a & 0x80000000u) p ^= b;
        a <<= 1;
        b = (b >> 1) ^ (CRC_POLY & (0u - (b & 1)));
    }
    return p;
}
struct Xp8Table { uint32_t v[48]; };
constexpr uint32_t cx_mulmod(uint32_t a, uint32_t b) {
    uint32_t p = 0;
    for (int i = 0; i < 32; ++i) {
        if (a & 0x80000000u) p ^= b;
        a <<= 1;
        b = (b >> 1) ^ (0xEDB88320u & (0u - (b & 1)));
    }
    return p;
}
constexpr Xp8Table cx_xp8_table() {
    Xp8Table t{};
    uint32_t sq = 0x00800000u;
    for (int k = 0; k < 48; ++k) { t.v[k] = sq; sq = cx_mulmod(sq, sq); }
    return t;
}
__constant__ Xp8Table XP8 = cx_xp8_table();

struct AdvTable { uint32_t t[4][256]; };
constexpr uint32_t cx_xpow8n(uint64_t n) {
    uint32_t r = 0x80000000u, sq = 0x00800000u;
    while (n) { if (n & 1) r = cx_mulmod(r, sq); sq = cx_mulmod(sq, sq); n >>= 1; }
    return r;
}
constexpr AdvTable cx_adv_table() {
    AdvTable a{};
    const uint32_t adv = cx_xpow8n(4096 - 64);
    for (int k = 0; k < 4; ++k)
        for (uint32_t b = 0; b < 256; ++b) a.t[k][b] = cx_mulmod(b << (8 * k), adv);
    return a;
}
__constant__ AdvTable ADV = cx_adv_table();

__device__ __forceinline__ uint32_t gf2_xpow8n(uint64_t nbytes) {
    uint32_t r = 0x80000000u;
    bool first = true;
    for (uint32_t k = 0; nbytes; ++k, nbytes >>= 1)
        if (nbytes & 1) {
            const uint32_t f = XP8.v[k < 47 ? k : 47];
            r = first ? f : gf2_mulmod(r, f);
            first = false;
        }
    return r;
}

__device__ __forceinline__ void ck_tables(uint32_t (*tab)[256], uint32_t (*advt)[256]) {
    {
        uint32_t c = threadIdx.x;
        for (int k = 0; k < 8; ++k) c = (c >> 1) ^ (CRC_POLY & (0u - (c & 1)));
        tab[0][threadIdx.x] = c;
    }
    for (int k = 0; k < 4; ++k) advt[k][threadIdx.x] = ADV.t[k][threadIdx.x];
    __syncthreads();
    for (int t = 1; t < 4; ++t) {
        const uint32_t pv = tab[t - 1][threadIdx.x];
        tab[t][threadIdx.x] = (pv >> 8) ^ tab[0][pv & 0xFF];
        __syncthreads();
    }
}

struct CkPartial { uint32_t crc, a, b; };
template <int MODE = 3>
__device__ __forceinline__ CkPartial ck_span_partial(const uint8_t *p, uint32_t rlen, uint32_t lane,
                                                     const uint32_t (*tab)[256], const uint32_t (*advt)[256]) {
    constexpr bool CRC = (MODE & 1) != 0, ADL = (MODE & 2) != 0;
    const ByteSrc src = make_src(p, rlen);
    uint32_t crc = 0, stand = 0;
    uint32_t s1 = 0, s1_before = 0;
    uint64_t s2 = 0;
    const uint32_t first = 64 * lane;
    const uint32_t shb = (uint32_t)src.shift;
    const bool wide = shb == 0 && ((uint64_t)src.w & 15) == 0;
    auto load_piece = [&](uint32_t (&w)[16], uint32_t o) {
        if (wide) {
            const uint32_t last16 = (rlen - 1) >> 4;
            const uint4 *w16 = (const uint4 *)src.w;
#pragma unroll
            for (uint32_t q = 0; q < 4; ++q) {
                const uint32_t i = min((o >> 4) + q, last16);
                const uint4 v = w16[i];
                w[4 * q] = v.x; w[4 * q + 1] = v.y; w[4 * q + 2] = v.z; w[4 * q + 3] = v.w;
            }
        } else {
            const uint32_t lastd = (rlen + shb - 1) >> 2;
            const uint32_t i0 = (o + shb) >> 2;
            uint32_t raw[17];
#pragma unroll
            for (uint32_t q = 0; q < 17; ++q) raw[q] = src.w[min(i0 + q, lastd)];
#pragma unroll
            for (uint32_t q = 0; q < 16; ++q) w[q] = __builtin_amdgcn_alignbyte(raw[q + 1], raw[q], shb);
        }
// ... 63 lines not shown
                                                            uint32_t *__restrict__ a_part,
                                                            uint32_t *__restrict__ b_part, uint64_t region0) {
    __shared__ uint32_t tab[4][256];
    __shared__ uint32_t advt[4][256];
    ck_tables(tab, advt);
    const uint32_t lane = threadIdx.x & 63;
    const uint64_t region = region0 + (uint64_t)blockIdx.x * 4 + (threadIdx.x >> 6);
    const uint64_t r0 = region * span;
    if (r0 >= n) return;
    const uint32_t rlen = (uint32_t)min((uint64_t)span, n - r0);
    const CkPartial r = ck_span_partial<MODE>(in + r0, rlen, lane, tab, advt);
    if (lane == 0) { crc_part[region] = r.crc; a_part[region] = r.a; b_part[region] = r.b; }
}

__global__ __launch_bounds__(256) void checksum_ranges_kernel(const uint8_t *__restrict__ data, uint32_t count,
                                                              const uint64_t *__restrict__ off, uint32_t off_stride,
                                                              const uint64_t *__restrict__ len, uint32_t len_stride,
                                                              uint32_t *__restrict__ crc_out,
                                                              uint32_t *__restrict__ adler_out) {
    __shared__ uint32_t tab[4][256];
    __shared__ uint32_t advt[4][256];
    ck_tables(tab, advt);
    const uint32_t lane = threadIdx.x & 63;
    const uint32_t i = blockIdx.x * 4 + (threadIdx.x >> 6);
    if (i >= count) return;
    const uint8_t *p = data + off[(uint64_t)i * off_stride];
    const uint64_t n = len[(uint64_t)i * len_stride];
    uint32_t crc = 0, a = 0, b = 0;
    const uint32_t xs = gf2_xpow8n(CK_SPAN);
    for (uint64_t o = 0; o < n; o += CK_SPAN) {
        const uint32_t sl = (uint32_t)min((uint64_t)CK_SPAN, n - o);
        const CkPartial r = ck_span_partial(p + o, sl, lane, tab, advt);
        crc = gf2_mulmod(crc, sl == CK_SPAN ? xs : gf2_xpow8n(sl)) ^ r.crc;
        b = (uint32_t)((b + r.b + (sl % 65521u) * (uint64_t)a) % 65521u);
        a = (a + r.a) % 65521u;
    }
    if (lane == 0) {
        crc_out[i] = crc ^ gf2_mulmod(0xFFFFFFFFu, gf2_xpow8n(n)) ^ 0xFFFFFFFFu;
        const uint32_t A = (1u + a) % 65521u;
        const uint32_t B = (uint32_t)((n % 65521u + b) % 65521u);
        adler_out[i] = (B << 16) | A;
    }
}

__global__ __launch_bounds__(1024) void checksum_combine_kernel(const uint32_t *__restrict__ crc_part,
                                                                const uint32_t *__restrict__ a_part,
                                                                const uint32_t *__restrict__ b_part,
                                                                uint64_t n, uint32_t span,
                                                                EncodeResult *__restrict__ res) {
    __shared__ uint32_t s_crc[16], s_a[16], s_b[16];
    const uint64_t nspans = div_up(n, span);
    const uint64_t per = div_up(nspans ? nspans : 1, 1023);
    const uint32_t t = threadIdx.x;
    uint32_t crc = 0, a = 0, b = 0;
    if (t < 1023) {
        const uint64_t lo = (uint64_t)t * per, hi = min(nspans, lo + per);
        if (lo < hi) {
            uint64_t len = 0;
            const uint32_t xs = gf2_xpow8n(span);
            for (uint64_t s = lo; s < hi; ++s) {
                const uint64_t sl = min((uint64_t)span, n - s * span);
                const uint32_t sh = sl == span ? xs : gf2_xpow8n(sl);
                crc = gf2_mulmod(crc, sh) ^ crc_part[s];
                b = (uint32_t)((b + b_part[s] + (sl % 65521u) * (uint64_t)a) % 65521u);
                a = (a + a_part[s]) % 65521u;
                len += sl;
            }
            const uint64_t after = n - (lo * span + len);
            if (after) crc = gf2_mulmod(crc, gf2_xpow8n(after));
            b = (uint32_t)((b + (after % 65521u) * (uint64_t)a) % 65521u);
        }
    } else {
        crc = gf2_mulmod(0xFFFFFFFFu, gf2_xpow8n(n));
    }
    for (int o = 32; o > 0; o >>= 1) {
        crc ^= __shfl_xor(crc, o);
        a += __shfl_xor(a, o);
        b += __shfl_xor(b, o);
    }
    if ((t & 63) == 0) { s_crc[t >> 6] = crc; s_a[t >> 6] = a; s_b[t >> 6] = b; }
    __syncthreads();
    if (t == 0) {
        uint32_t c = 0;
        uint64_t A = 0, B = 0;
        for (int w = 0; w < 16; ++w) { c ^= s_crc[w]; A += s_a[w]; B += s_b[w]; }
        res->crc32 = c ^ 0xFFFFFFFFu;
        const uint32_t Af = (uint32_t)((1u + A) % 65521u);
        const uint32_t Bv = (uint32_t)((n % 65521u + B) % 65521u);
        res->adler32 = (Bv << 16) | Af;
    }
}

__global__ void put_bytes_kernel(const uint8_t *__restrict__ bytes, uint32_t n, uint64_t at_byte,
                                 uint32_t *__restrict__ out) {
    for (uint32_t i = threadIdx.x; i < n; i += blockDim.x) {
        const uint64_t ob = at_byte + i;
        atomicOr(&out[ob >> 2], (uint32_t)bytes[i] << (8 * (ob & 3)));
    }
}
__global__ void or_byte_kernel(uint8_t *__restrict__ dst, const uint8_t *__restrict__ src) {
    if (threadIdx.x == 0 && blockIdx.x == 0) dst[0] = (uint8_t)(dst[0] | src[0]);
}
int launch_or_byte(hipStream_t st, uint8_t *dst, const uint8_t *src) {
    hipLaunchKernelGGL(or_byte_kernel, dim3(1), dim3(64), 0, st, dst, src);
    const hipError_t e_ = hipGetLastError();
    return e_ != hipSuccess ? (int)e_ : 0;
}
__global__ void trailer_kernel(int format, uint32_t isize, uint64_t out_base_bit,
                               EncodeResult *__restrict__ res, uint32_t *__restrict__ out) {
    if (threadIdx.x != 0 || res->status != 0) return;
    const uint64_t at = (res->end_bit - out_base_bit + 7) >> 3;
    uint8_t t[8];
    uint32_t nt = 0;
    if (format == 2) {
        const uint32_t c = res->crc32;
        t[0] = c; t[1] = c >> 8; t[2] = c >> 16; t[3] = c >> 24;
        t[4] = isize; t[5] = isize >> 8; t[6] = isize >> 16; t[7] = isize >> 24;
        nt = 8;
    } else if (format == 1) {
        const uint32_t a = res->adler32;
        t[0] = a >> 24; t[1] = a >> 16; t[2] = a >> 8; t[3] = a;
        nt = 4;
    }
    for (uint32_t i = 0; i < nt; ++i) {
        const uint64_t ob = at + i;
        atomicOr(&out[ob >> 2], (uint32_t)t[i] << (8 * (ob & 3)));
    }
    res->out_bytes = at + nt;
}

#define LFX_LAUNCH_CHECK()                          \
    do {                                            \
        hipError_t e_ = hipGetLastError();          \
        if (e_ != hipSuccess) return (int)e_;       \
    } while (0)

int launch_match(hipStream_t st, const uint8_t *in, uint64_t in_bytes, const ChunkDesc *chunks,
                 const SegDesc *segs, uint32_t nsegs, uint32_t window, uint32_t max_len, uint32_t *md, uint64_t *dbg) {
    if (nsegs == 0) return 0;
    const size_t lds = MATCH_LDS;
    static bool attr_set[64] = {};
    int dev_ = 0;
    (void)hipGetDevice(&dev_);
    if (!attr_set[dev_ & 63]) {
        (void)hipFuncSetAttribute((const void *)lz77_match_kernel, hipFuncAttributeMaxDynamicSharedMemorySize, (int)lds);
        attr_set[dev_ & 63] = true;
    }
    hipLaunchKernelGGL(lz77_match_kernel, dim3(nsegs), dim3(MATCH_THREADS), lds, st, in, in_bytes,
                       chunks, segs, window, max_len, md, dbg);
    LFX_LAUNCH_CHECK();
    return 0;
}
int launch_chunk_maps(hipStream_t st, const ChunkDesc *chunks, uint32_t nchunks, uint64_t ntiles, uint32_t nsegs,
                      uint32_t *tile_map, uint32_t *seg_map, ZeroSpan z0, ZeroSpan z1, ZeroSpan z2) {
    if (nchunks == 0) {
        for (const ZeroSpan &z : {z0, z1, z2})
            if (z.n && hipMemsetAsync(z.p, 0, 4ull * z.n, st) != hipSuccess) return (int)hipGetLastError();
        return 0;
    }
    uint32_t split = nchunks >= 256 ? 1 : 256 / nchunks + 1;
    if (split > 64) split = 64;
    hipLaunchKernelGGL(chunk_maps_kernel, dim3(nchunks, split), dim3(256), 0, st, chunks, nchunks, ntiles, nsegs, tile_map, seg_map, z0, z1, z2);
    LFX_LAUNCH_CHECK();
    return 0;
}
int launch_histogram(hipStream_t st, const ChunkDesc *chunks, uint32_t nchunks, uint32_t split,
                     const uint32_t *codes, const uint32_t *ncodes, uint32_t *hist) {
    if (nchunks == 0) return 0;
    hipLaunchKernelGGL(histogram_kernel, dim3(nchunks, split), dim3(256), 0, st, chunks, codes, ncodes, hist);
    LFX_LAUNCH_CHECK();
    return 0;
}
int launch_huffman(hipStream_t st, const BlockDesc *blocks, uint32_t nblocks, const uint32_t *hist,
                   BlockCodes *bc, uint64_t *dbg) {
    if (nblocks == 0) return 0;
    hipLaunchKernelGGL(huffman_kernel, dim3(nblocks), dim3(HUFF_THREADS), 0, st, blocks, hist, bc, dbg);
    LFX_LAUNCH_CHECK();
    return 0;
}
int launch_offsets(hipStream_t st, const BlockDesc *blocks, uint32_t nblocks, const BlockCodes *bc,
                   uint64_t start_bit, uint64_t cap_bits, uint64_t *block_start, EncodeResult *res) {
    hipLaunchKernelGGL(offsets_kernel, dim3(1), dim3(256), 0, st, blocks, nblocks, bc, start_bit,
                       cap_bits, block_start, res);
    LFX_LAUNCH_CHECK();
    return 0;
}
int launch_offsets_batch(hipStream_t st, const BatchStream *streams, uint32_t count, const BlockDesc *blocks, const BlockCodes *bc,
                         uint32_t hdr_len, uint32_t trailer_len, uint64_t *block_start, uint64_t *stream_end, int32_t *status,
                         EncodeResult *res) {
    if (!count) return 0;
    hipLaunchKernelGGL(offsets_batch_kernel, dim3((count + 255) / 256), dim3(256), 0, st, streams, count, blocks, bc, hdr_len,
                       trailer_len, block_start, stream_end, status, res);
    LFX_LAUNCH_CHECK();
    return 0;
}
int launch_frame_batch(hipStream_t st, int format, const BatchStream *streams, uint32_t count, const uint8_t *hdr, uint32_t hdr_len,
                       const uint64_t *stream_end, const uint32_t *crc, const uint32_t *adler, const EncodeResult *res, uint32_t *out,
                       uint64_t *out_len) {
    if (!count) return 0;
    hipLaunchKernelGGL(frame_batch_kernel, dim3((count + 255) / 256), dim3(256), 0, st, format, streams, count, hdr, hdr_len,
                       stream_end, crc, adler, res, out, out_len);
    LFX_LAUNCH_CHECK();
    return 0;
}
int launch_pack(hipStream_t st, const uint8_t *in, uint64_t in_bytes, const ChunkDesc *chunks,
                uint32_t nchunks, const BlockDesc *blocks, uint32_t nblocks, uint64_t ntiles,
                const uint32_t *codes, const uint32_t *ncodes, const BlockCodes *bc,
                const uint64_t *block_start, uint32_t *tile_bits, uint64_t *tile_start,
                const EncodeResult *res, uint64_t out_base_bit, uint32_t *out, const uint32_t *tile_map) {
    if (ntiles) {
        const uint32_t ngroups = (uint32_t)div_up(ntiles, PACK_TPW);
        hipLaunchKernelGGL(tile_bits_kernel, dim3(ngroups), dim3(PACK_THREADS), 0, st, chunks,
                           nchunks, blocks, codes, ncodes, bc, tile_bits, tile_map, ntiles);
        LFX_LAUNCH_CHECK();
        hipLaunchKernelGGL(tile_scan_kernel, dim3(nblocks), dim3(ntiles / (nblocks ? nblocks : 1) > 2048 ? 1024 : 256), 0, st, chunks, blocks, bc,
                           block_start, tile_bits, ntiles, nchunks, tile_start);
        LFX_LAUNCH_CHECK();
        hipLaunchKernelGGL(pack_kernel, dim3(ngroups), dim3(PACK_THREADS), 0, st, chunks,
                           nchunks, blocks, codes, ncodes, bc, tile_start, res, out_base_bit, out, tile_map, ntiles);
        LFX_LAUNCH_CHECK();
    }
    if (nblocks) {
        hipLaunchKernelGGL(block_header_kernel, dim3(nblocks), dim3(256), 0, st, in, in_bytes, blocks,
                           bc, block_start, res, out_base_bit, out);
        LFX_LAUNCH_CHECK();
    }
    return 0;
}
int launch_checksum_part(hipStream_t st, const uint8_t *in, uint64_t n, uint32_t *crc_part, uint32_t *a_part, uint32_t *b_part,
                         EncodeResult *res, int mode, uint32_t part, uint32_t nparts) {
    const uint32_t span = ck_span(n);
    const uint64_t nspans = div_up(n, span);
    const uint64_t ngroups = div_up(nspans, 4);
    const uint64_t g0 = ngroups * part / nparts, g1 = ngroups * (part + 1) / nparts;
    if (g1 > g0) {
        const dim3 grid((uint32_t)(g1 - g0));
        if (mode == 1) hipLaunchKernelGGL(checksum_span_kernel<1>, grid, dim3(256), 0, st, in, n, span, crc_part, a_part, b_part, 4 * g0);
        else if (mode == 2) hipLaunchKernelGGL(checksum_span_kernel<2>, grid, dim3(256), 0, st, in, n, span, crc_part, a_part, b_part, 4 * g0);
        else hipLaunchKernelGGL(checksum_span_kernel<3>, grid, dim3(256), 0, st, in, n, span, crc_part, a_part, b_part, 4 * g0);
        LFX_LAUNCH_CHECK();
    }
    if (part + 1 == nparts) {
        hipLaunchKernelGGL(checksum_combine_kernel, dim3(1), dim3(1024), 0, st, crc_part, a_part, b_part, n, span, res);
        LFX_LAUNCH_CHECK();
    }
    return 0;
}
int launch_checksum(hipStream_t st, const uint8_t *in, uint64_t n, uint32_t *crc_part,
                    uint32_t *a_part, uint32_t *b_part, EncodeResult *res, int mode) {
    return launch_checksum_part(st, in, n, crc_part, a_part, b_part, res, mode, 0, 1);
}
int launch_checksum_ranges(hipStream_t st, const uint8_t *data, uint32_t count, const uint64_t *off,
                           uint32_t off_stride, const uint64_t *len, uint32_t len_stride, uint32_t *crc, uint32_t *adler) {
    if (!count) return 0;
    hipLaunchKernelGGL(checksum_ranges_kernel, dim3((count + 3) / 4), dim3(256), 0, st, data, count, off, off_stride, len,
                       len_stride, crc, adler);
    LFX_LAUNCH_CHECK();
    return 0;
}
int launch_put_bytes(hipStream_t st, const uint8_t *d_bytes, uint32_t n, uint64_t at_byte, uint32_t *out) {
    if (n == 0) return 0;
    hipLaunchKernelGGL(put_bytes_kernel, dim3(1), dim3(256), 0, st, d_bytes, n, at_byte, out);
    LFX_LAUNCH_CHECK();
    return 0;
}
int launch_trailer(hipStream_t st, int format, uint32_t isize, uint64_t out_base_bit,
                   EncodeResult *res, uint32_t *out) {
    hipLaunchKernelGGL(trailer_kernel, dim3(1), dim3(64), 0, st, format, isize, out_base_bit, res, out);
    LFX_LAUNCH_CHECK();
    return 0;
}

}
```

Before: 59.08 GB/s.

## Fuse tile bit counting, scan and pack into single-pass decoupled look-back kernel

Replaces the three-kernel pack sequence (tile_bits, tile_scan, pack) with one fused kernel. It hands out tiles through an atomic ticket and computes each tile's bit offset with a decoupled look-back prefix scan over per-tile state words. This removes two kernel launches and the round trips of per-tile bit counts through global memory. If a look-back spins too long the kernel sets a gave-up flag, and the host re-runs the encode with the old two-pass path. The cost is extra tile-state zeroing, spin-waiting between workgroups, and possible fallback re-encodes.

```diff
diff --git a/include/lfx.h b/include/lfx.h
--- a/include/lfx.h
+++ b/include/lfx.h
@@ -280,6 +280,7 @@
     int n_phases;
 } lfx_timing;
 uint64_t lfx_ctx_match_fallbacks(const lfx_ctx *c);
+uint64_t lfx_ctx_pack_fallbacks(const lfx_ctx *c);
 int lfx_ctx_last_timing(lfx_ctx *c, lfx_timing *t);
 void lfx_ctx_enable_timing(lfx_ctx *c, int on);
 uint32_t lfx_version(void);
diff --git a/libflate_amd/_ffi.py b/libflate_amd/_ffi.py
--- a/libflate_amd/_ffi.py
+++ b/libflate_amd/_ffi.py
@@ -27,7 +27,7 @@
     "lfx_lz77_free", "lfx_ctx_last_timing", "lfx_ctx_enable_timing", "lfx_version",
     "lfx_comm_rccl", "lfx_comm_rccl_free", "lfx_sharded_encode_begin", "lfx_sharded_encode_finish", "lfx_sharded_byte_range",
     "lfx_sharded_decode", "lfx_sharded_layout", "lfx_sharded_gather_tuples", "lfx_sharded_fold", "lfx_sharded_free",
-    "lfx_host_alloc", "lfx_host_free", "lfx_ctx_match_fallbacks", "lfx_decode_members_device", "lfx_decode_members_host",
+    "lfx_host_alloc", "lfx_host_free", "lfx_ctx_match_fallbacks", "lfx_ctx_pack_fallbacks", "lfx_decode_members_device", "lfx_decode_members_host",
     "lfx_decode_index_device", "lfx_index_read_device", "lfx_index_span", "lfx_index_get_info", "lfx_index_get_point",
     "lfx_index_export", "lfx_index_import", "lfx_index_check", "lfx_index_free", "lfx_encode_index_device",
     "lfx_encode_members_bound", "lfx_encode_members_device", "lfx_encode_members_host", "lfx_members_gzi",
@@ -160,6 +160,8 @@
     L.lfx_host_free.argtypes = [vp]
     L.lfx_ctx_match_fallbacks.restype = u64
     L.lfx_ctx_match_fallbacks.argtypes = [vp]
+    L.lfx_ctx_pack_fallbacks.restype = u64
+    L.lfx_ctx_pack_fallbacks.argtypes = [vp]
     L.lfx_decode_device.argtypes = [vp, i32, u32, vp, u64, vp, u64, C.POINTER(u64), C.POINTER(u64)]
     L.lfx_decode_host.argtypes = [vp, i32, u32, vp, u64, vp, u64, C.POINTER(u64), C.POINTER(u64)]
     L.lfx_decode_batch_device.argtypes = [vp, i32, u32, vp, vp, vp, vp, vp, vp, vp, vp]
diff --git a/libflate_amd/context.py b/libflate_amd/context.py
--- a/libflate_amd/context.py
+++ b/libflate_amd/context.py
@@ -60,6 +60,9 @@
 
     def match_fallbacks(self):
         return int(_ffi.lib().lfx_ctx_match_fallbacks(self._h))
+
+    def pack_fallbacks(self):
+        return int(_ffi.lib().lfx_ctx_pack_fallbacks(self._h))
 
     def encode_host_ptr(self, fmt, in_ptr, n, out_ptr, cap, opts=None, schedule=None):
         out_len = C.c_uint64(0)
diff --git a/libflate_amd/csrc/lfx_api.cpp b/libflate_amd/csrc/lfx_api.cpp
--- a/libflate_amd/csrc/lfx_api.cpp
+++ b/libflate_amd/csrc/lfx_api.cpp
@@ -234,6 +234,7 @@
     no_pin_slots = on("LFX_NO_PIN_SLOTS");
     no_small_scan = on("LFX_NO_SMALL_SCAN");
     store_tight = on("LFX_STORE_TIGHT");
+    pack_two_pass = on("LFX_PACK_TWO_PASS");
 }
 
 void Ctx::phase(const char *name) {
@@ -329,6 +330,9 @@
 extern "C" uint64_t lfx_ctx_match_fallbacks(const lfx_ctx *cc) {
     return cc ? reinterpret_cast<const Ctx *>(cc)->match_fallbacks : 0;
 }
+extern "C" uint64_t lfx_ctx_pack_fallbacks(const lfx_ctx *cc) {
+    return cc ? reinterpret_cast<const Ctx *>(cc)->pack_fallbacks : 0;
+}
 extern "C" void lfx_ctx_enable_timing(lfx_ctx *cc, int on) { reinterpret_cast<Ctx *>(cc)->timing_on = on >= 2 && on <= 6 ? on : on != 0; }
 extern "C" int lfx_ctx_last_timing(lfx_ctx *cc, lfx_timing *t) try {
     Ctx *c = reinterpret_cast<Ctx *>(cc);
@@ -424,7 +428,7 @@
     if ((rc = c->d_hist.reserve(4ull * 320 * std::max<size_t>(nblocks, 1)))) return rc;
     if ((rc = c->d_bc.reserve(sizeof(BlockCodes) * std::max<size_t>(nblocks, 1)))) return rc;
     if ((rc = c->d_block_start.reserve(8 * std::max<size_t>(nblocks, 1)))) return rc;
-    if ((rc = c->d_tile_bits.reserve(4 * std::max<uint64_t>(plan.n_tiles, 1)))) return rc;
+    if ((rc = c->d_tile_bits.reserve(8 * std::max<uint64_t>(plan.n_tiles, 1)))) return rc;
     if ((rc = c->d_tile_start.reserve(8 * std::max<uint64_t>(plan.n_tiles, 1)))) return rc;
     const uint64_t nspans = ck_nspans(n);
     if ((rc = c->d_ck.reserve(12 * nspans))) return rc;
@@ -449,8 +453,10 @@
     c->phase("upload");
     uint32_t *tile_map = (uint32_t *)c->d_chunkmap.p, *seg_map = tile_map + plan.n_tiles;
     c->cur_tile_map = tile_map;
+    const bool fused_pack = !c->pack_two_pass();
+    c->pack_state_fresh = fused_pack && nchunks != 0;
     if (int e_ = launch_chunk_maps(st, (const ChunkDesc *)c->d_chunks.p, nchunks, plan.n_tiles, plan.n_segs, tile_map, seg_map, z_hist,
-                                   z_res, z_ucount)) {
+                                   z_res, z_ucount, fused_pack ? (uint64_t *)c->d_tile_bits.p : nullptr)) {
         c->set_error(hipGetErrorString((hipError_t)e_));
         return LFX_E_DEVICE;
     }
@@ -626,6 +632,25 @@
     return LFX_OK;
 }
 
+static int pack_ticket(Ctx *c, hipStream_t st, uint32_t **ticket) {
+    *ticket = nullptr;
+    if (c->force_pack_two_pass) c->pack_fallbacks++;
+    if (c->pack_two_pass()) return LFX_OK;
+    uint32_t *t = (uint32_t *)c->d_res.p + 32;
+    if (!c->pack_state_fresh) {
+        if (hipMemsetAsync(c->d_tile_bits.p, 0, 8 * std::max<uint64_t>(c->cur_ntiles, 1), st) != hipSuccess ||
+            hipMemsetAsync(t, 0, 4, st) != hipSuccess) { c->set_error("hipMemsetAsync failed"); return LFX_E_DEVICE; }
+    }
+    c->pack_state_fresh = false;
+    *ticket = t;
+    return LFX_OK;
+}
+static bool pack_gave_up(Ctx *c, const EncodeResult &res) {
+    if (!(res.match_flags & PACK_GAVE_UP) || c->pack_two_pass()) return false;
+    c->force_pack_two_pass = true;
+    return true;
+}
+
 int encode_emit(Ctx *c, int format, bool with_trailer, uint32_t trailer_check, bool use_device_check, uint64_t total_n,
                 const uint8_t *prefix, uint32_t prefix_len, uint64_t start_bit, uint8_t *d_out, uint64_t cap,
                 EncodeResult *host_res, EncodeResult *async_slot = nullptr);
@@ -649,12 +674,14 @@
     EncodeResult *dres = (EncodeResult *)c->d_res.p;
     LAUNCH_TRY(launch_offsets(st, (const BlockDesc *)c->d_blocks.p, c->cur_nblocks, (const BlockCodes *)c->d_bc.p,
                               start_bit, cap_bits, (uint64_t *)c->d_block_start.p, dres));
+    uint32_t *ticket;
+    if (int rct = pack_ticket(c, st, &ticket)) return rct;
     LAUNCH_TRY(launch_pack(st, c->cur_in, c->cur_n, (const ChunkDesc *)c->d_chunks.p, c->cur_nchunks,
                            (const BlockDesc *)c->d_blocks.p, c->cur_nblocks, c->cur_ntiles,
                            (const uint32_t *)c->d_codes.p, (const uint32_t *)c->d_ncodes.p,
                            (const BlockCodes *)c->d_bc.p, (const uint64_t *)c->d_block_start.p,
-                           (uint32_t *)c->d_tile_bits.p, (uint64_t *)c->d_tile_start.p, dres, 0,
-                           (uint32_t *)d_out, c->cur_tile_map));
+                           c->d_tile_bits.p, (uint64_t *)c->d_tile_start.p, dres, 0,
+                           (uint32_t *)d_out, c->cur_tile_map, ticket));
     c->phase("pack");
     if (prefix_len) {
         int rcp = c->d_hdr.reserve(prefix_len);
@@ -673,6 +700,8 @@
     HIP_TRY(hipStreamSynchronize(st));
     *host_res = *(EncodeResult *)c->h_res;
     if (host_res->status != 0) { c->set_error("output capacity too small"); return LFX_E_NOSPACE; }
+    if (pack_gave_up(c, *host_res))
+        return encode_emit(c, format, with_trailer, trailer_check, use_device_check, total_n, prefix, prefix_len, start_bit, d_out, cap, host_res);
     return LFX_OK;
 }
 
@@ -801,10 +830,12 @@
         EncodeResult *dres = (EncodeResult *)c->d_res.p;
         LAUNCH_TRY(launch_offsets_batch(st, d_streams, count, (const BlockDesc *)c->d_blocks.p, (const BlockCodes *)c->d_bc.p,
                                         (uint32_t)hdr.size(), trailer, (uint64_t *)c->d_block_start.p, d_end, d_status, dres));
+        uint32_t *ticket;
+        if ((rc = pack_ticket(c, st, &ticket))) return rc;
         LAUNCH_TRY(launch_pack(st, (const uint8_t *)d_in, in_extent, (const ChunkDesc *)c->d_chunks.p, c->cur_nchunks,
                                (const BlockDesc *)c->d_blocks.p, nblocks, c->cur_ntiles, (const uint32_t *)c->d_codes.p,
                                (const uint32_t *)c->d_ncodes.p, (const BlockCodes *)c->d_bc.p, (const uint64_t *)c->d_block_start.p,
-                               (uint32_t *)c->d_tile_bits.p, (uint64_t *)c->d_tile_start.p, dres, 0, (uint32_t *)d_out, c->cur_tile_map));
+                               c->d_tile_bits.p, (uint64_t *)c->d_tile_start.p, dres, 0, (uint32_t *)d_out, c->cur_tile_map, ticket));
         c->phase("pack");
         LAUNCH_TRY(launch_frame_batch(st, format, d_streams, count, d_hdr, (uint32_t)hdr.size(), d_end, d_crc, d_adler, dres,
                                       (uint32_t *)d_out, d_len));
@@ -814,7 +845,7 @@
         c->phase("frame");
         HIP_TRY(hipStreamSynchronize(st));
         res = *(EncodeResult *)c->h_res;
-        if (match_violation(c, res)) continue;
+        if (match_violation(c, res) || pack_gave_up(c, res)) continue;
         break;
     }
     for (uint32_t i = 0; i < count; i++) {
@@ -999,10 +1030,12 @@
             if (prezero) HIP_TRY(hipStreamWaitEvent(st, c->ev_zero, 0));
             else if (fill) HIP_TRY(hipMemsetAsync(d_out, 0, fill, st));
             prezero = false;
+            uint32_t *ticket;
+            if ((rc2 = pack_ticket(c, st, &ticket))) return rc2;
             LAUNCH_TRY(launch_pack(st, (const uint8_t *)d_in, n, (const ChunkDesc *)c->d_chunks.p, c->cur_nchunks,
                                    (const BlockDesc *)c->d_blocks.p, nblocks, c->cur_ntiles, (const uint32_t *)c->d_codes.p,
                                    (const uint32_t *)c->d_ncodes.p, (const BlockCodes *)c->d_bc.p, (const uint64_t *)c->d_block_start.p,
-                                   (uint32_t *)c->d_tile_bits.p, (uint64_t *)c->d_tile_start.p, dres, 0, (uint32_t *)d_out, c->cur_tile_map));
+                                   c->d_tile_bits.p, (uint64_t *)c->d_tile_start.p, dres, 0, (uint32_t *)d_out, c->cur_tile_map, ticket));
             c->phase("pack");
             LAUNCH_TRY(launch_members_frame(st, g, d_hdr, d_members, d_crc, dres, (uint32_t *)d_out));
             HIP_TRY(hipMemcpyAsync(c->h_res, dres, sizeof(EncodeResult), hipMemcpyDeviceToHost, st));
@@ -1010,7 +1043,7 @@
             c->phase("frame");
             HIP_TRY(hipStreamSynchronize(st));
             res = *(EncodeResult *)c->h_res;
-            if (match_violation(c, res)) continue;
+            if (match_violation(c, res) || pack_gave_up(c, res)) continue;
             return LFX_OK;
         }
     };
@@ -1238,7 +1271,7 @@
     EncodeResult res = *(const EncodeResult *)e->h_res.data();
     const uint64_t n = e->inflight_n;
     int rc = LFX_OK;
-    if (match_violation(c, res)) {
+    if (match_violation(c, res) || pack_gave_up(c, res)) {
         const uint8_t prefix[1] = {e->carry};
         if ((rc = encode_prepare(c, e->inflight_plan, e->po, (const uint8_t *)e->d_in.p, n, e->format == LFX_GZIP ? 1 : e->format == LFX_ZLIB ? 2 : 0))) { e->err = c->err; return rc; }
         rc = encode_emit(c, LFX_DEFLATE, false, 0, true, 0, prefix, e->carry_bits ? 1 : 0, e->carry_bits, (uint8_t *)e->d_out.p,
diff --git a/libflate_amd/csrc/lfx_ctx.h b/libflate_amd/csrc/lfx_ctx.h
--- a/libflate_amd/csrc/lfx_ctx.h
+++ b/libflate_amd/csrc/lfx_ctx.h
@@ -41,6 +41,7 @@
     bool hist_separate = false;
     bool store_tight = false;
     int enc_batch_mb = 0;
+    bool pack_two_pass = false;
     int pocr_max = 100;
     void read();
 };
@@ -125,6 +126,10 @@
     const uint8_t *cur_in = nullptr;
     bool force_match_v1 = false;
     uint64_t match_fallbacks = 0;
+    bool force_pack_two_pass = false;
+    uint64_t pack_fallbacks = 0;
+    bool pack_state_fresh = false;
+    bool pack_two_pass() const { return force_pack_two_pass || diag.pack_two_pass; }
     HostIo hostio;
     static constexpr size_t POOL_MAX = 8;
     std::vector<PinVec> pin_pool;
diff --git a/libflate_amd/csrc/lfx_device.h b/libflate_amd/csrc/lfx_device.h
--- a/libflate_amd/csrc/lfx_device.h
+++ b/libflate_amd/csrc/lfx_device.h
@@ -62,7 +62,7 @@
 struct ZeroSpan { uint32_t *p; uint32_t n; };
 int launch_chunk_maps(hipStream_t st, const ChunkDesc *chunks, uint32_t nchunks, uint64_t ntiles, uint32_t nsegs,
                       uint32_t *tile_map, uint32_t *seg_map, ZeroSpan z0 = ZeroSpan{nullptr, 0}, ZeroSpan z1 = ZeroSpan{nullptr, 0},
-                      ZeroSpan z2 = ZeroSpan{nullptr, 0});
+                      ZeroSpan z2 = ZeroSpan{nullptr, 0}, uint64_t *tile_state = nullptr );
 int launch_histogram(hipStream_t st, const ChunkDesc *chunks, uint32_t nchunks, uint32_t split,
                      const uint32_t *codes, const uint32_t *ncodes, uint32_t *hist);
 int launch_huffman(hipStream_t st, const BlockDesc *blocks, uint32_t nblocks, const uint32_t *hist,
@@ -87,11 +87,12 @@
                           EncodeResult *res);
 int launch_members_frame(hipStream_t st, const MembersGeom &g, const uint8_t *hdr, const lfx_member *members, const uint32_t *crc,
                          const EncodeResult *res, uint32_t *out);
+constexpr uint32_t PACK_GAVE_UP = 4;
 int launch_pack(hipStream_t st, const uint8_t *in, uint64_t in_bytes, const ChunkDesc *chunks,
                 uint32_t nchunks, const BlockDesc *blocks, uint32_t nblocks, uint64_t ntiles,
                 const uint32_t *codes, const uint32_t *ncodes, const BlockCodes *bc,
-                const uint64_t *block_start, uint32_t *tile_bits, uint64_t *tile_start,
-                const EncodeResult *res, uint64_t out_base_bit, uint32_t *out, const uint32_t *tile_map);
+                const uint64_t *block_start, void *tile_scratch, uint64_t *tile_start,
+                EncodeResult *res, uint64_t out_base_bit, uint32_t *out, const uint32_t *tile_map, uint32_t *ticket);
 inline uint32_t ck_span(uint64_t n) { return n <= (64ull << 20) ? 8192u : 65536u; }
 inline uint64_t ck_nspans(uint64_t n) { return div_up(n ? n : 1, ck_span(n)); }
 int launch_checksum(hipStream_t st, const uint8_t *in, uint64_t n, uint32_t *crc_part,
diff --git a/libflate_amd/csrc/lfx_encode_kernels.hip b/libflate_amd/csrc/lfx_encode_kernels.hip
--- a/libflate_amd/csrc/lfx_encode_kernels.hip
+++ b/libflate_amd/csrc/lfx_encode_kernels.hip
@@ -297,7 +297,7 @@
 __global__ __launch_bounds__(256) void chunk_maps_kernel(const ChunkDesc *__restrict__ chunks, uint32_t nchunks,
                                                          uint64_t ntiles, uint32_t nsegs,
                                                          uint32_t *__restrict__ tile_map, uint32_t *__restrict__ seg_map,
-                                                         ZeroSpan z0, ZeroSpan z1, ZeroSpan z2) {
+                                                         ZeroSpan z0, ZeroSpan z1, ZeroSpan z2, uint64_t *__restrict__ tile_state) {
     {
         const uint32_t nthreads = 256u * gridDim.x * gridDim.y, me = (blockIdx.y * gridDim.x + blockIdx.x) * 256u + threadIdx.x;
         for (uint32_t i = me; i < z0.n; i += nthreads) z0.p[i] = 0;
@@ -308,7 +308,10 @@
     const ChunkDesc ch = chunks[c];
     const uint64_t t1 = c + 1 < nchunks ? chunks[c + 1].tile_base : ntiles;
     const uint32_t s1 = c + 1 < nchunks ? chunks[c + 1].seg_base : nsegs;
-    for (uint64_t t = ch.tile_base + blockIdx.y * 256 + threadIdx.x; t < t1; t += 256ull * gridDim.y) tile_map[t] = c;
+    for (uint64_t t = ch.tile_base + blockIdx.y * 256 + threadIdx.x; t < t1; t += 256ull * gridDim.y) {
+        tile_map[t] = c;
+        if (tile_state) tile_state[t] = 0;
+    }
     for (uint32_t q = ch.seg_base + blockIdx.y * 256 + threadIdx.x; q < s1; q += 256u * gridDim.y) seg_map[q] = c;
 }
 
@@ -692,6 +695,185 @@
     }
 }
 
+constexpr uint64_t PF_AGG = 1ull << 62, PF_PREFIX = 2ull << 62, PF_VALUE = PF_AGG - 1;
+constexpr uint64_t PF_FAIL = ~0ull;
+constexpr uint32_t PF_SPIN_CAP = 1u << 16;
+
+__device__ __forceinline__ uint64_t pf_wave_sum(uint64_t v) {
+    for (int o = 32; o > 0; o >>= 1) v += __shfl_xor(v, o);
+    return (uint64_t)__builtin_amdgcn_readfirstlane((uint32_t)(v >> 32)) << 32 | __builtin_amdgcn_readfirstlane((uint32_t)v);
+}
+
+__device__ __forceinline__ uint64_t pf_look_back(const uint64_t *tile_state, uint64_t t, uint64_t t0, uint64_t base,
+                                                 const uint32_t *flags, uint32_t lane) {
+    uint64_t acc = 0, hi = t;
+    for (uint32_t spins = 0;;) {
+        const bool below = hi < t0 + lane + 1;
+        uint64_t w = __hip_atomic_load(&tile_state[below ? t0 : hi - 1 - lane], __ATOMIC_RELAXED, __HIP_MEMORY_SCOPE_AGENT);
+        if (below) w = PF_PREFIX | base;
+        const uint32_t flag = (uint32_t)(w >> 62);
+        const uint64_t none = __ballot(flag == 0), pfx = __ballot(flag == 2);
+        const uint32_t first_none = none ? (uint32_t)__ffsll((unsigned long long)none) - 1 : 64u;
+        const uint32_t first_pfx = pfx ? (uint32_t)__ffsll((unsigned long long)pfx) - 1 : 64u;
+        if (first_pfx < first_none) return acc + pf_wave_sum(lane <= first_pfx ? w & PF_VALUE : 0ull);
+        if (first_none == 64u) {
+            acc += pf_wave_sum(w & PF_VALUE);
+            hi -= 64;
+            continue;
+        }
+        if (++spins >= PF_SPIN_CAP) return PF_FAIL;
+        if ((spins & 63u) == 0 && (__hip_atomic_load(flags, __ATOMIC_RELAXED, __HIP_MEMORY_SCOPE_AGENT) & PACK_GAVE_UP)) return PF_FAIL;
+        __builtin_amdgcn_s_sleep(8);
+    }
+}
+
+__global__ __launch_bounds__(PACK_THREADS) void pack_fused_kernel(
+    const ChunkDesc *__restrict__ chunks, uint32_t nchunks, const BlockDesc *__restrict__ blocks,
+    const uint32_t *__restrict__ codes, const uint32_t *__restrict__ ncodes,
+    const BlockCodes *__restrict__ bc, const uint64_t *__restrict__ block_start, uint64_t *tile_state,
+    uint64_t *__restrict__ tile_start, EncodeResult *res, uint32_t *ticket, uint64_t out_base_bit,
+    uint32_t *__restrict__ out, const uint32_t *__restrict__ tile_map, uint64_t ntiles) {
+    __shared__ uint32_t lit[288], dst[32];
+    __shared__ uint32_t wsum[PACK_THREADS / 64];
+    __shared__ unsigned long long stage[STAGE_WORDS64];
+    __shared__ uint32_t s_ticket;
+    __shared__ uint64_t s_start;
+    if (res->status != 0) return;
+    if (threadIdx.x == 0) s_ticket = atomicAdd(ticket, 1u);
+    __syncthreads();
+    const uint64_t g0 = (uint64_t)s_ticket * PACK_TPW;
+    if (g0 >= ntiles) return;
+    uint32_t cm[PACK_TPW];
+#pragma unroll
+    for (uint32_t q = 0; q < PACK_TPW; ++q) cm[q] = tile_map[min(g0 + q, ntiles - 1)];
+    uint32_t cur_c = 0xFFFFFFFFu, cur_block = 0xFFFFFFFFu, n = 0;
+    ChunkDesc ch{};
+    BlockDesc bd{};
+    bool raw = false;
+    uint32_t run_block = 0xFFFFFFFFu;
+    uint64_t run = 0;
+    uint32_t cv[PACK_PER_THREAD], cvn[PACK_PER_THREAD];
+    bool have_next = false;
+    const uint32_t lane = threadIdx.x & 63, wave = threadIdx.x >> 6;
+#pragma unroll
+    for (uint32_t q = 0; q < PACK_TPW; ++q) {
+        const uint64_t gt = g0 + q;
+        if (gt >= ntiles) break;
+        const uint32_t c = cm[q];
+        if (c != cur_c) {
+            cur_c = c;
+            ch = chunks[c];
+            n = ncodes[c];
+            bd = blocks[ch.block];
+            raw = bd.type == BT_RAW;
+            have_next = false;
+        }
+        if (raw) { have_next = false; continue; }
+        const uint32_t lo = (uint32_t)(gt - ch.tile_base) * PACK_TILE;
+        const bool live = lo < n;
+        const uint32_t hi = min(n, lo + PACK_TILE);
+        const uint32_t first = lo + threadIdx.x * PACK_PER_THREAD;
+        uint64_t cb[PACK_PER_THREAD];
+        uint32_t mine = 0, x = 0, pre = 0, total = 0;
+        if (live) {
+            const uint32_t *p = codes + ch.code_off;
+            if (have_next) {
+#pragma unroll
+                for (int k = 0; k < PACK_PER_THREAD; ++k) cv[k] = cvn[k];
+            } else {
+#pragma unroll
+                for (int k = 0; k < PACK_PER_THREAD; ++k) cv[k] = p[min(first + k, hi - 1)];
+            }
+            have_next = q + 1 < PACK_TPW && gt + 1 < ntiles && cm[q + 1 < PACK_TPW ? q + 1 : q] == c;
+            if (have_next) {
+#pragma unroll
+                for (int k = 0; k < PACK_PER_THREAD; ++k) cvn[k] = p[min(first + PACK_TILE + k, n - 1)];
+            }
+            __syncthreads();
+            if (ch.block != cur_block) {
+                cur_block = ch.block;
+                const BlockCodes *B = &bc[ch.block];
+                for (uint32_t i = threadIdx.x; i < 288; i += PACK_THREADS) lit[i] = B->lit[i];
+                if (threadIdx.x < 32) dst[threadIdx.x] = B->dist[threadIdx.x];
+            }
+            for (uint32_t i = threadIdx.x; i < STAGE_WORDS64; i += PACK_THREADS) stage[i] = 0;
+            __syncthreads();
+#pragma unroll
+            for (int k = 0; k < PACK_PER_THREAD; ++k) {
+                const uint32_t i = first + k;
+                const uint32_t nb = code_bits(cv[k], lit, dst, cb[k]);
+                cb[k] = i < hi ? cb[k] | (uint64_t)nb << 56 : 0ull;
+                mine += i < hi ? nb : 0u;
+            }
+            x = mine;
+            for (int o = 1; o < 64; o <<= 1) {
+                const uint32_t y = __shfl_up(x, o);
+                if ((int)lane >= o) x += y;
+            }
+            if (lane == 63) wsum[wave] = x;
+            __syncthreads();
+            for (uint32_t w = 0; w < wave; ++w) pre += wsum[w];
+            total = wsum[0] + wsum[1] + wsum[2] + wsum[3];
+        } else {
+            have_next = false;
+        }
+        uint64_t excl;
+        if (run_block == ch.block) {
+            excl = run;
+        } else {
+            const uint64_t t0 = c == bd.first_chunk ? ch.tile_base : chunks[bd.first_chunk].tile_base;
+            const uint64_t base = block_start[ch.block] + 3 + bc[ch.block].hdr_bits;
+            if (gt == t0) {
+                excl = base;
+            } else if (q == 0) {
+                if (wave == 0) {
+                    if (lane == 0) __hip_atomic_store(&tile_state[gt], PF_AGG | total, __ATOMIC_RELAXED, __HIP_MEMORY_SCOPE_AGENT);
+                    const uint64_t e = pf_look_back(tile_state, gt, t0, base, &res->match_flags, lane);
+                    if (lane == 0) s_start = e;
+                }
+                __syncthreads();
+                excl = s_start;
+            } else {
+                excl = PF_FAIL;
+            }
+        }
+        if (excl == PF_FAIL) {
+            if (threadIdx.x == 0) atomicOr(&res->match_flags, PACK_GAVE_UP);
+            return;
+        }
+        run = excl + total;
+        run_block = ch.block;
+        if (threadIdx.x == 0) {
+            __hip_atomic_store(&tile_state[gt], PF_PREFIX | run, __ATOMIC_RELAXED, __HIP_MEMORY_SCOPE_AGENT);
+            tile_start[gt] = excl;
+        }
+        if (!live) continue;
+        const uint64_t start = excl - out_base_bit;
+        const uint32_t phase = (uint32_t)start & 31;
+        uint32_t bit = phase + pre + x - mine;
+#pragma unroll
+        for (int k = 0; k < PACK_PER_THREAD; ++k) {
+            const uint32_t nb = (uint32_t)(cb[k] >> 56);
+            if (nb) {
+                const uint64_t b = cb[k] & ((1ull << 56) - 1);
+                const uint32_t w = bit >> 6, sh = bit & 63;
+                atomicOr(&stage[w], b << sh);
+                if (sh + nb > 64) atomicOr(&stage[w + 1], b >> (64 - sh));
+                bit += nb;
+            }
+        }
+        __syncthreads();
+        const uint32_t nwords = (phase + total + 31) >> 5;
+        const uint32_t *s32 = (const uint32_t *)stage;
+        uint32_t *o = out + (start >> 5);
+        for (uint32_t i = threadIdx.x; i < nwords; i += PACK_THREADS) {
+            const uint32_t v = s32[i];
+            if (i == 0 || i == nwords - 1) { if (v) atomicOr(&o[i], v); }
+            else o[i] = v;
+        }
+    }
+}
+
 __global__ __launch_bounds__(256) void block_header_kernel(
     const uint8_t *__restrict__ in, uint64_t in_bytes, const BlockDesc *__restrict__ blocks,
     const BlockCodes *__restrict__ bc, const uint64_t *__restrict__ block_start,
@@ -1061,7 +1243,7 @@
     return 0;
 }
 int launch_chunk_maps(hipStream_t st, const ChunkDesc *chunks, uint32_t nchunks, uint64_t ntiles, uint32_t nsegs,
-                      uint32_t *tile_map, uint32_t *seg_map, ZeroSpan z0, ZeroSpan z1, ZeroSpan z2) {
+                      uint32_t *tile_map, uint32_t *seg_map, ZeroSpan z0, ZeroSpan z1, ZeroSpan z2, uint64_t *tile_state) {
     if (nchunks == 0) {
         for (const ZeroSpan &z : {z0, z1, z2})
             if (z.n && hipMemsetAsync(z.p, 0, 4ull * z.n, st) != hipSuccess) return (int)hipGetLastError();
@@ -1069,7 +1251,7 @@
     }
     uint32_t split = nchunks >= 256 ? 1 : 256 / nchunks + 1;
     if (split > 64) split = 64;
-    hipLaunchKernelGGL(chunk_maps_kernel, dim3(nchunks, split), dim3(256), 0, st, chunks, nchunks, ntiles, nsegs, tile_map, seg_map, z0, z1, z2);
+    hipLaunchKernelGGL(chunk_maps_kernel, dim3(nchunks, split), dim3(256), 0, st, chunks, nchunks, ntiles, nsegs, tile_map, seg_map, z0, z1, z2, tile_state);
     LFX_LAUNCH_CHECK();
     return 0;
 }
@@ -1115,9 +1297,15 @@
 int launch_pack(hipStream_t st, const uint8_t *in, uint64_t in_bytes, const ChunkDesc *chunks,
                 uint32_t nchunks, const BlockDesc *blocks, uint32_t nblocks, uint64_t ntiles,
                 const uint32_t *codes, const uint32_t *ncodes, const BlockCodes *bc,
-                const uint64_t *block_start, uint32_t *tile_bits, uint64_t *tile_start,
-                const EncodeResult *res, uint64_t out_base_bit, uint32_t *out, const uint32_t *tile_map) {
-    if (ntiles) {
+                const uint64_t *block_start, void *tile_scratch, uint64_t *tile_start,
+                EncodeResult *res, uint64_t out_base_bit, uint32_t *out, const uint32_t *tile_map, uint32_t *ticket) {
+    if (ntiles && ticket) {
+        const uint32_t ngroups = (uint32_t)div_up(ntiles, PACK_TPW);
+        hipLaunchKernelGGL(pack_fused_kernel, dim3(ngroups), dim3(PACK_THREADS), 0, st, chunks, nchunks, blocks, codes, ncodes, bc,
+                           block_start, (uint64_t *)tile_scratch, tile_start, res, ticket, out_base_bit, out, tile_map, ntiles);
+        LFX_LAUNCH_CHECK();
+    } else if (ntiles) {
+        uint32_t *tile_bits = (uint32_t *)tile_scratch;
         const uint32_t ngroups = (uint32_t)div_up(ntiles, PACK_TPW);
         hipLaunchKernelGGL(tile_bits_kernel, dim3(ngroups), dim3(PACK_THREADS), 0, st, chunks,
                            nchunks, blocks, codes, ncodes, bc, tile_bits, tile_map, ntiles);
```

Result: slower. 23.22 GB/s (median of 2 runs) (-60.7%).
